# borgwang/tinynn-autograd

Measured on AMD Instinct MI355X. Metric: training samples/sec, MNIST 3-layer MLP (784-256-128-10), bs=128, at 1/2/4/8 GPUs, higher is better.
Workload: dtype f32; 1 GPU; configs[1]: Dense/ReLU MLP 784-256-128-10, 128 rows per GPU (global batch 128), whole-batch softmax NLL, Adam lr=1e-3; parallelism=dp1, global_batch=128, rows_per_rank=128, data_resident_in_hbm=True

## Files before the change

tinynn-autograd_amd/csrc/tnn_gemm.hip:

```cpp
#include <math.h>
#include <stdlib.h>

#include <algorithm>

#include "tnn_internal.h"
#include "tnn_dispatch.h"
#include "tnn_tile_order.h"
#include "tnn_p2p.h"
#include "tnn_head_stats.h"

namespace {

#include "tnn_gemm_args.h"
#include "tnn_gemm_tiled.h"
#include "tnn_gemm_adam.h"
#include "tnn_gemm_small.h"
#include "tnn_gemm_mid.h"
#include "tnn_gemm_step.h"
#include "tnn_gemm_f64.h"

GemmArgs gemm_args(const void* A, int64_t lda, const void* B, int64_t ldb, void* C, int64_t ldc, int64_t M, int64_t N, int64_t K,
                   int epi, float alpha = 1.f, float beta = 0.f) {
    GemmArgs g = {};
    g.A = (const float*)A; g.B = (const float*)B; g.C = (float*)C;
    g.M = M; g.N = N; g.K = K; g.lda = lda; g.ldb = ldb; g.ldc = ldc;
    g.alpha = alpha; g.beta = beta; g.epi = epi;
    return g;
}
void set_bias_act(GemmArgs& g, const void* bias, int act, int relu_sign) {
    g.bias = (const float*)bias; g.act = act; g.relu_sign = relu_sign;
}
void set_mask(GemmArgs& g, const void* Y, int64_t ldy) {
    g.Y = (const float*)Y; g.ldy = ldy;
}

bool vec_ok(const void* p, int64_t ld, int64_t contiguous, int64_t bytes = 0) {
    return tnn::aligned16(p) && ld % 4 == 0 && contiguous % 4 == 0 && bytes < (int64_t(1) << 32);
}

template <typename F>
auto with_layout(int transA, int transB, F&& f) {
    return tnn::with_flag(!transA, [&](auto akc) { return tnn::with_flag(transB != 0, [&](auto bkc) { return f(akc, bkc); }); });
}

GemmArgs dense_fwd_args(int64_t M, int64_t N, int64_t K, const void* A, int64_t lda, const void* B, int64_t ldb, const void* bias,
                        int act, int relu_sign, void* C, int64_t ldc) {
    GemmArgs g = gemm_args(A, lda, B, ldb, C, ldc, M, N, K, EPI_BIAS_ACT);
    set_bias_act(g, bias, act, relu_sign);
    g.vecA = vec_ok(A, lda, K);
    g.vecB = vec_ok(B, ldb, N);
    return g;
}
void set_head(GemmArgs& g, const void* head_w, void* head_z, int64_t head_c) {
    g.head_w = (const float*)head_w; g.head_z = (float*)head_z; g.head_c = (int)head_c;
}

void small_geometry(GemmArgs& g) {
    g.tiles_m = (int)((g.M + 15) / 16);
    g.tiles_n = (int)((g.N + 15) / 16);
    g.splits = 1;
    g.ws = nullptr;
    g.ord = tnn::tile_order(g.tiles_m, g.tiles_n, 0, 0);
}

inline bool tn_extents_ok(const GemmArgs& g) {
    return g.K * g.lda * 4 < (int64_t(1) << 31) && g.K * g.ldb * 4 < (int64_t(1) << 31);
}

void pick_xcd_cut(GemmArgs& g) {
    int xg_m = 0, xg_n = 0, best = 0;
    for (int xm = 1; xm <= 8; xm *= 2) {
        const int xn = 8 / xm;
        if (g.tiles_m % xm || g.tiles_n % xn) continue;
        const int cost = g.tiles_m / xm + g.tiles_n / xn;
        if (!best || cost < best) { best = cost; xg_m = xm; xg_n = xn; }
    }
    g.ord = tnn::tile_order(g.tiles_m, g.tiles_n, xg_m, xg_n);
}

bool mid_ok(const GemmArgs& g, int transA, int transB) {
    const bool akc = !transA, bkc = transB != 0;
    if (akc && !vec_ok(g.A, g.lda, g.K)) return false;
    if (bkc && !vec_ok(g.B, g.ldb, g.K)) return false;
    const int64_t a_bytes = ((akc ? g.M : g.K) * g.lda) * 4, b_bytes = ((bkc ? g.N : g.K) * g.ldb) * 4;
    return a_bytes < (int64_t(1) << 31) && b_bytes < (int64_t(1) << 31);
}

bool small_fast_ok(const GemmArgs& g, int transA, int transB) {
    const int64_t lim = int64_t(1) << 31;
    if (((g.M - 1) * g.ldc + g.N) * 4 >= lim || (g.epi == EPI_MASK && ((g.M - 1) * g.ldy + g.N) * 4 >= lim)) return false;
    return (!transA || transB) && mid_ok(g, transA, transB);
}

void fill_small_fast(GemmArgs& g, bool akc, bool bkc) {
    SmallFast& f = g.f;
    f.A = g.A; f.B = g.B;
    f.a_bytes = (uint32_t)(((akc ? g.M : g.K) - 1) * g.lda + (akc ? g.K : g.M)) * 4u;
    f.b_bytes = (uint32_t)(((bkc ? g.N : g.K) - 1) * g.ldb + (bkc ? g.K : g.N)) * 4u;
    f.lda4 = (uint32_t)g.lda * 4u; f.ldb4 = (uint32_t)g.ldb * 4u;
    f.M = (uint32_t)g.M; f.N = (uint32_t)g.N; f.K = (uint32_t)g.K;
    f.nchunks = (int)((g.K + 15) / 16);
    f.e_ptr = nullptr; f.e_bytes = 0u; f.e_ld4 = 0u;
    if (g.epi == EPI_BIAS_ACT) {
        f.e_ptr = g.bias; f.e_bytes = (uint32_t)g.N * 4u;
    } else if (g.epi == EPI_MASK) {
        f.e_ptr = g.Y; f.e_bytes = (uint32_t)((g.M - 1) * g.ldy + g.N) * 4u; f.e_ld4 = (uint32_t)g.ldy * 4u;
    } else if (g.beta != 0.f) {
        f.e_ptr = g.C; f.e_bytes = (uint32_t)((g.M - 1) * g.ldc + g.N) * 4u; f.e_ld4 = (uint32_t)g.ldc * 4u;
    }
    if (f.e_ptr == nullptr) f.e_bytes = 0u;
    const bool head = g.head_z != nullptr && g.head_w != nullptr;
    f.head_w = head ? g.head_w : nullptr;
    f.h_bytes = head ? (uint32_t)g.N * (uint32_t)g.head_c * 4u : 0u;
    f.hc4 = (uint32_t)g.head_c * 4u;
}

template <int WAVES>
int launch_small(GemmArgs& g, int transA, int transB, float* colsum) {
    small_geometry(g);
    dim3 grid((unsigned)(g.tiles_m * g.tiles_n));
    hipStream_t s = tnn::stream();
    const bool fast = small_fast_ok(g, transA, transB);
    pick_xcd_cut(g);
    if (fast) fill_small_fast(g, !transA, transB != 0);
    with_layout(transA, transB, [&](auto akc, auto bkc) {
        tnn::with_flag(fast, [&](auto f) {
            hipLaunchKernelGGL((gemm_small_f32_kernel<decltype(akc)::value, decltype(bkc)::value, WAVES, decltype(f)::value>), grid,
                               WAVES * 64, 0, s, g, colsum);
        });
    });
    TNN_LAUNCH_OK();
    return 0;
}

bool use_small_path(const GemmArgs& g) {
    int64_t tiles = ((g.M + 15) / 16) * ((g.N + 15) / 16);
    if (const char* e = getenv("TNN_GEMM_SMALL")) return atoi(e) != 0 && tiles <= tnn::kTileOrderMaxTiles;
    if (getenv("TNN_GEMM_CFG")) return false;
    double flop = 2.0 * (double)g.M * (double)g.N * (double)g.K;
    return flop <= 4.2e8 && tiles <= 8192;
}

int gemm_small(GemmArgs& g, int transA, int transB, float* colsum) {
    int nchunks = (int)((g.K + 15) / 16);
    if (nchunks <= 16) return launch_small<4>(g, transA, transB, colsum);
    if (nchunks <= 48) return launch_small<8>(g, transA, transB, colsum);
    return launch_small<16>(g, transA, transB, colsum);
}

bool use_mid_path(const GemmArgs& g, int transA, int transB) {
    const double flop = 2.0 * (double)g.M * (double)g.N * (double)g.K;
    const int64_t tiles = ((g.M + 31) / 32) * ((g.N + 31) / 32);
    return flop >= 1.5e8 && tiles >= 192 && mid_ok(g, transA, transB);
}

void mid_geometry(GemmArgs& g) {
    g.tiles_m = (int)((g.M + 31) / 32);
    g.tiles_n = (int)((g.N + 31) / 32);
    g.splits = 1;
    g.ws = nullptr;
    pick_xcd_cut(g);
}

int gemm_mid(GemmArgs& g, int transA, int transB, float* colsum) {
    mid_geometry(g);
    const int tiles = g.tiles_m * g.tiles_n;
    hipStream_t s = tnn::stream();
    AdamEpi none = {};
    with_layout(transA, transB, [&](auto akc, auto bkc) {
        hipLaunchKernelGGL((gemm_mid_f32_kernel<decltype(akc)::value, decltype(bkc)::value, false>), tiles, 512, 0, s, g, colsum,
                           none, tiles);
    });
    TNN_LAUNCH_OK();
    return 0;
}

template <int BM, int BN, int BK, int WM, int WN>
int launch_cfg(GemmArgs& g, int transA, int transB, int splits) {
    g.tiles_m = (int)((g.M + BM - 1) / BM);
    g.tiles_n = (int)((g.N + BN - 1) / BN);
    int64_t ktiles = (g.K + BK - 1) / BK;
    if (splits > ktiles) splits = (int)ktiles;
    if (splits < 1) splits = 1;
    int64_t tiles_per_split = (ktiles + splits - 1) / splits;
    if (tiles_per_split < 1) tiles_per_split = 1;
    splits = ktiles > 0 ? (int)((ktiles + tiles_per_split - 1) / tiles_per_split) : 1;
    g.k_per_split = tiles_per_split * BK;
    g.splits = splits;
    g.ws = nullptr;
    g.group_m = 8;
    if (const char* e = getenv("TNN_GEMM_GROUP_M")) g.group_m = atoi(e) > 0 ? atoi(e) : 8;
#ifdef TNN_GEMM_TRACE
    g.trace = nullptr;
    if (const char* e = getenv("TNN_GEMM_TRACE_PTR"))
        if (splits == 1) g.trace = reinterpret_cast<unsigned long long*>(strtoull(e, nullptr, 0));
#endif
    void* ws = nullptr;
    if (splits > 1) {
        if (tnn_malloc((size_t)splits * g.M * g.N * sizeof(float), &ws)) return 1;
        g.ws = (float*)ws;
    }
    dim3 grid((unsigned)(g.tiles_m * g.tiles_n), 1, (unsigned)splits);
    constexpr int NT = WM * WN * 64;
    hipStream_t s = tnn::stream();
    with_layout(transA, transB, [&](auto akc, auto bkc) {
        tnn::with_flag(g.vecA && g.vecB, [&](auto vec) {
            hipLaunchKernelGGL((gemm_f32_mfma_kernel<BM, BN, BK, WM, WN, decltype(akc)::value, decltype(bkc)::value, decltype(vec)::value>),
                               grid, NT, 0, s, g);
        });
    });
    if (splits > 1) {
        hipLaunchKernelGGL(splitk_reduce_kernel, tnn::stream_grid(g.M * g.N, 256), 256, 0, s, g);
        tnn_free(ws);
    }
    TNN_LAUNCH_OK();
    return 0;
}

int gemm_f32(GemmArgs& g, int transA, int transB, float* colsum = nullptr) {
    g.vecA = vec_ok(g.A, g.lda, transA ? g.M : g.K, (transA ? g.K : g.M) * g.lda * 4);
    g.vecB = vec_ok(g.B, g.ldb, transB ? g.K : g.N, (transB ? g.N : g.K) * g.ldb * 4);
    if (use_small_path(g)) return use_mid_path(g, transA, transB) ? gemm_mid(g, transA, transB, colsum)
                                                                    : gemm_small(g, transA, transB, colsum);
    if (colsum != nullptr) {
        if (int rc = tnn_reduce(TNN_RSUM, g.B, colsum, 1, g.K, g.N, TNN_F32)) return rc;
    }

    const int cus = tnn::num_cus();
    g.staged_c = 1;
    int cfg = -1, splits = 0;
    if (const char* e = getenv("TNN_GEMM_CFG")) cfg = atoi(e);
    if (const char* e = getenv("TNN_GEMM_SPLITK")) splits = atoi(e);
    int64_t t128x64 = ((g.M + 127) / 128) * ((g.N + 63) / 64);
    int64_t t64 = ((g.M + 63) / 64) * ((g.N + 63) / 64);
    if (cfg < 0) cfg = (t128x64 >= cus / 2) ? 3 : 2;
    const int64_t t64x128 = ((g.M + 63) / 64) * ((g.N + 127) / 128);
    if (cfg == 3 && !getenv("TNN_GEMM_CFG") && !transA && g.M <= 1024 && t64x128 >= cus / 2 && t64x128 <= 2 * cus) cfg = 1;
    if (splits <= 0) {
        splits = 1;
        int64_t tiles = cfg == 3 ? t128x64 : cfg == 2 ? t64 : cfg == 0 ? ((g.M + 127) / 128) * ((g.N + 127) / 128)
                                                              : ((g.M + 63) / 64) * ((g.N + 127) / 128);
        if (tiles < cus) {
            splits = (int)((cus + tiles - 1) / tiles);
            int64_t max_splits = g.K / 256;
            if (splits > max_splits) splits = (int)max_splits;
            if (splits < 1) splits = 1;
            if (splits > 16) splits = 16;
        }
    }
    switch (cfg) {
        case 0: return launch_cfg<128, 128, 32, 2, 2>(g, transA, transB, splits);
        case 1: return launch_cfg<64, 128, 32, 2, 2>(g, transA, transB, splits);
        case 2: return launch_cfg<64, 64, 32, 2, 2>(g, transA, transB, splits);
        case 3: return launch_cfg<128, 64, 32, 2, 2>(g, transA, transB, splits);
    }
    tnn::set_error("tnn_gemm: unknown tile configuration %d", cfg);
    return 2;
}

int gemm_f64(int transA, int transB, int64_t M, int64_t N, int64_t K, const void* A, int64_t lda,
             const void* B, int64_t ldb, void* C, int64_t ldc, double alpha, double beta, int epi,
             const void* bias, int act, int relu_sign, const void* Y, int64_t ldy) {
    GemmArgsD g;
    g.relu_sign = relu_sign;
    g.A = (const double*)A; g.B = (const double*)B; g.C = (double*)C;
    g.M = M; g.N = N; g.K = K;
    g.sam = transA ? 1 : lda; g.sak = transA ? lda : 1;
    g.sbk = transB ? 1 : ldb; g.sbn = transB ? ldb : 1;
    g.ldc = ldc; g.alpha = alpha; g.beta = beta; g.epi = epi;
    g.bias = (const double*)bias; g.act = act; g.Y = (const double*)Y; g.ldy = ldy;
    dim3 grid((unsigned)((N + 63) / 64), (unsigned)std::min<int64_t>((M + 63) / 64, 65535));
    hipLaunchKernelGGL(gemm_f64_kernel, grid, 256, 0, tnn::stream(), g);
    TNN_LAUNCH_OK();
    return 0;
}

int check_shapes(const char* fn, int transA, int transB, int64_t M, int64_t N, int64_t K,
                 int64_t lda, int64_t ldb, int64_t ldc) {
    TNN_REQUIRE(M >= 0 && N >= 0 && K >= 0, "%s: negative extent", fn);
    TNN_REQUIRE(lda >= (transA ? M : K), "%s: lda %lld too small", fn, (long long)lda);
    TNN_REQUIRE(ldb >= (transB ? K : N), "%s: ldb %lld too small", fn, (long long)ldb);
    TNN_REQUIRE(ldc >= N, "%s: ldc %lld too small", fn, (long long)ldc);
    TNN_REQUIRE(M < (1LL << 31) && N < (1LL << 31), "%s: extent exceeds 2^31", fn);
    return 0;
}

int rowpanel_args(const char* fn, bool merged, int64_t M, int64_t N, int64_t K, const void* A, int64_t lda, const void* B, int64_t ldb,
                  const void* bias, int act, int relu_sign, void* C, int64_t ldc, const void* head_w, int64_t head_c,
                  void* head_z_full, const void* head_b, void* pairs_f32, const void* ticket, const void* out_pair, int dtype,
                  RowPanelArgs& g) {
    TNN_NEED_INIT();
    if (int rc = check_shapes(fn, 0, 0, M, N, K, lda, ldb, ldc)) return rc;
    TNN_REQUIRE(dtype == TNN_F32 && M >= 1 && M <= 1024 && N == 128 && head_c == 10 && K >= 1,
                "%s: f32, 1 <= rows <= 1024, 128 hidden units, 10 classes", fn);
    TNN_REQUIRE(A && B && C && head_w && head_z_full && head_b && pairs_f32 && (!merged || (ticket && out_pair)),
                "%s: A, B, C, head_w, head_z_full, head_b%s are required", fn, merged ? ", pairs, ticket and out_pair" : " and pairs");
    TNN_REQUIRE(act == TNN_ACT_RELU, "%s: the hidden layer in front of the head is a ReLU layer (activation %d)", fn, act);
    TNN_REQUIRE(vec_ok(A, lda, K) && (M - 1) * lda + K < (int64_t)1 << 30 && (K - 1) * ldb + 128 < (int64_t)1 << 30,
                "%s: A must be 16-B aligned with lda and K multiples of 4, operands below 4 GiB", fn);
    g.A = (const float*)A; g.B = (const float*)B; g.bias = (const float*)bias; g.C = (float*)C;
    g.lda = lda; g.ldb = ldb; g.ldc = ldc;
    g.M = (int)M; g.K = (int)K; g.relu_sign = relu_sign;
    g.head_w = (const float*)head_w; g.head_b = (const float*)head_b;
    g.zfull = (float*)head_z_full; g.pairs = (float*)pairs_f32; g.bump = nullptr;
    return 0;
}
int launch_rowpanel_plain(const RowPanelArgs& g) {
    hipLaunchKernelGGL(dense_fwd_rowpanel_head_kernel<false>, dim3((unsigned)((g.M + 15) / 16)), 512, 0, tnn::stream(), g, HeadTail{},
                       tnn::p2p::LaunchCtx{});
    TNN_LAUNCH_OK();
    return 0;
}

}

extern "C" {

int tnn_gemm(int transA, int transB, int64_t M, int64_t N, int64_t K, double alpha, const void* A,
             int64_t lda, const void* B, int64_t ldb, double beta, void* C, int64_t ldc, int dtype) {
    TNN_NEED_INIT();
    if (int rc = check_shapes("tnn_gemm", transA, transB, M, N, K, lda, ldb, ldc)) return rc;
    if (M == 0 || N == 0) return 0;
    if (dtype == TNN_F64)
        return gemm_f64(transA, transB, M, N, K, A, lda, B, ldb, C, ldc, alpha, beta, EPI_AXPBY,
                        nullptr, 0, 0, nullptr, 0);
    TNN_REQUIRE(dtype == TNN_F32, "tnn_gemm: dtype %d is not a float type", dtype);
    GemmArgs g = gemm_args(A, lda, B, ldb, C, ldc, M, N, K, EPI_AXPBY, (float)alpha, (float)beta);
    return gemm_f32(g, transA, transB);
}

int tnn_gemm_tn_colsum(int64_t M, int64_t N, int64_t K, const void* A, int64_t lda, const void* G,
                       int64_t ldg, void* dW, int64_t ldc, void* db, int dtype) {
    TNN_NEED_INIT();
    if (int rc = check_shapes("tnn_gemm_tn_colsum", 1, 0, M, N, K, lda, ldg, ldc)) return rc;
    TNN_REQUIRE(ldg == N || db == nullptr, "tnn_gemm_tn_colsum: the column sum needs a dense G (ldg == N)");
    if (N == 0) return 0;
    if (dtype == TNN_F64) {
        if (M > 0)
            if (int rc = gemm_f64(1, 0, M, N, K, A, lda, G, ldg, dW, ldc, 1.0, 0.0, EPI_AXPBY, nullptr, 0, 0,
                                  nullptr, 0))
                return rc;
        return db ? tnn_reduce(TNN_RSUM, G, db, 1, K, N, TNN_F64) : 0;
    }
    TNN_REQUIRE(dtype == TNN_F32, "tnn_gemm_tn_colsum: dtype %d is not a float type", dtype);
    if (M == 0) return db ? tnn_reduce(TNN_RSUM, G, db, 1, K, N, TNN_F32) : 0;
    GemmArgs g = gemm_args(A, lda, G, ldg, dW, ldc, M, N, K, EPI_AXPBY);
    return gemm_f32(g, 1, 0, (float*)db);
}

int tnn_gemm_tn_adam(int64_t M, int64_t N, int64_t K, const void* A, int64_t lda, const void* G, int64_t ldg, void* g_out,
                     void* p, void* m, void* v, double lr, double b1, double b2, double eps, const void* pows_f64,
                     int dtype) {
    return tnn_gemm_tn_adam_bias(M, N, K, A, lda, G, ldg, g_out, p, m, v, nullptr, nullptr, nullptr, nullptr, lr, b1, b2, eps,
                                 pows_f64, dtype);
}

int tnn_gemm_tn_adam_bias(int64_t M, int64_t N, int64_t K, const void* A, int64_t lda, const void* G, int64_t ldg, void* g_out,
                          void* p, void* m, void* v, void* db, void* pb, void* mb, void* vb, double lr, double b1, double b2,
                          double eps, const void* pows_f64, int dtype) {
    TNN_NEED_INIT();
    if (int rc = check_shapes("tnn_gemm_tn_adam", 1, 0, M, N, K, lda, ldg, N)) return rc;
    TNN_REQUIRE((pb == nullptr) == (mb == nullptr) && (pb == nullptr) == (vb == nullptr) && (pb == nullptr || db != nullptr),
                "tnn_gemm_tn_adam_bias: pb / mb / vb go together and need db");
    TNN_REQUIRE(db == nullptr || ldg == N, "tnn_gemm_tn_adam_bias: the column sum needs a dense G (ldg == N)");
    TNN_REQUIRE(p && m && v && pows_f64, "tnn_gemm_tn_adam: p, m, v and pows are required");
    TNN_REQUIRE(dtype == TNN_F32 || dtype == TNN_F64, "tnn_gemm_tn_adam: dtype %d is not a float type", dtype);
    if (M == 0 || N == 0) return 0;
    using tnn::aligned16;
    GemmArgs g = gemm_args(A, lda, G, ldg, g_out, N, M, N, K, EPI_ADAM);
    const bool tiled = dtype == TNN_F32 && !use_small_path(g) && N % 4 == 0 && aligned16(p) && aligned16(m) && aligned16(v) && aligned16(g_out) &&
                       ((M + 127) / 128) * ((N + 63) / 64) >= tnn::num_cus() / 2 && getenv("TNN_GEMM_CFG") == nullptr &&
                       getenv("TNN_GEMM_SPLITK") == nullptr;
    if (tiled) {
        g.ad_p = (float*)p; g.ad_m = (float*)m; g.ad_v = (float*)v;
        g.ad_lr = (float)lr; g.ad_b1 = (float)b1; g.ad_b2 = (float)b2; g.ad_eps = (float)eps;
        g.ad_pows = (const double*)pows_f64;
        g.ad_guard = tnn::update_guard();
        const bool cs = db != nullptr;
        if (cs) { g.cs_db = (float*)db; g.cs_p = (float*)pb; g.cs_m = (float*)mb; g.cs_v = (float*)vb; }
        if (int rc = gemm_f32(g, 1, 0)) return rc;
        if (db != nullptr && !cs) {
            if (int rc = tnn_reduce(TNN_RSUM, G, db, 1, K, N, dtype)) return rc;
            if (pb) return tnn_adam_ex(pb, db, mb, vb, N, lr, b1, b2, eps, const_cast<void*>(pows_f64), nullptr, dtype, 0, nullptr, nullptr);
        }
        return 0;
    }
    void* scratch = nullptr;
    void* gw = g_out;
    const size_t esz = dtype == TNN_F64 ? 8 : 4;
    if (gw == nullptr) {
        if (tnn_malloc((size_t)(M * N) * esz, &scratch)) return 1;
        gw = scratch;
    }
    int rc = tnn_gemm_tn_colsum(M, N, K, A, lda, G, ldg, gw, N, db, dtype);
    if (!rc) rc = tnn_adam_ex(p, gw, m, v, M * N, lr, b1, b2, eps, const_cast<void*>(pows_f64), nullptr, dtype, 0, nullptr, nullptr);
    if (!rc && pb) rc = tnn_adam_ex(pb, db, mb, vb, N, lr, b1, b2, eps, const_cast<void*>(pows_f64), nullptr, dtype, 0, nullptr, nullptr);
    if (scratch) tnn_free(scratch);
    return rc;
}

int tnn_dense_bwd(int64_t rows, int64_t n_in, int64_t n_out, const void* x, const void* dz, const void* w,
                  void* dw, void* db, void* dx, const void* mask_src, int dtype) {
    TNN_NEED_INIT();
    TNN_REQUIRE(rows > 0 && n_in > 0 && n_out > 0, "tnn_dense_bwd: empty layer");
    TNN_REQUIRE(dx == nullptr || mask_src != nullptr, "tnn_dense_bwd: dx needs mask_src");
    if (dtype == TNN_F32 && dx != nullptr) {
        GemmArgs gw = gemm_args(x, n_in, dz, n_out, dw, n_out, n_in, n_out, rows, EPI_AXPBY);
        gw.vecA = vec_ok(x, n_in, n_in); gw.vecB = vec_ok(dz, n_out, n_out);
        GemmArgs gx = gemm_args(dz, n_out, w, n_out, dx, n_in, rows, n_in, n_out, EPI_MASK);
        set_mask(gx, mask_src, n_in);
        gx.vecA = vec_ok(dz, n_out, n_out); gx.vecB = vec_ok(w, n_out, n_out);
        if (use_small_path(gw) && use_small_path(gx)) {
            small_geometry(gw);
            small_geometry(gx);
            int n_dw = gw.tiles_m * gw.tiles_n, n_dx = gx.tiles_m * gx.tiles_n;
            if (n_dw % 8 == 0) {
                pick_xcd_cut(gw);
                pick_xcd_cut(gx);
            }
            int nchunks = (int)((std::max(gw.K, gx.K) + 15) / 16);
            hipStream_t s = tnn::stream();
            const bool fast = small_fast_ok(gw, 1, 0) && small_fast_ok(gx, 0, 1);
            if (fast) { fill_small_fast(gw, false, false); fill_small_fast(gx, true, true); }
#define TNN_BWD_SMALL(W)                                                                                             \
    do {                                                                                                             \
        if (fast) hipLaunchKernelGGL((dense_bwd_small_kernel<W, true>), n_dw + n_dx, W * 64, 0, s, gw, (float*)db, gx, n_dw); \
        else hipLaunchKernelGGL((dense_bwd_small_kernel<W, false>), n_dw + n_dx, W * 64, 0, s, gw, (float*)db, gx, n_dw);    \
    } while (0)
            if (nchunks <= 16)
                TNN_BWD_SMALL(4);
            else if (nchunks <= 48)
                TNN_BWD_SMALL(8);
            else
                TNN_BWD_SMALL(16);
#undef TNN_BWD_SMALL
            TNN_LAUNCH_OK();
            return 0;
        }
    }
    if (int rc = tnn_gemm_tn_colsum(n_in, n_out, rows, x, n_in, dz, n_out, dw, n_out, db, dtype)) return rc;
    if (dx != nullptr)
        return tnn_gemm_mask(0, 1, rows, n_in, n_out, dz, n_out, w, n_out, mask_src, n_in, dx, n_in, dtype);
    return 0;
}

static bool dw0_wide_ok(const GemmArgs& g) {
    static const bool off = getenv("TNN_DW0_WIDE") && atoi(getenv("TNN_DW0_WIDE")) == 0;
    return !off && g.N % 32 == 0 && ((g.M + 15) / 16) * (g.N / 32) >= 256 && g.epi == EPI_AXPBY && g.beta == 0.f;
}

int tnn_dense_bwd_first_adam(int64_t rows, int64_t n_in, int64_t n_out, const void* x, const void* dz, void* dw, void* db,
                             void* p_w, void* m_w, void* v_w, void* p_b, void* m_b, void* v_b, void* flat_p,
                             const void* flat_g, void* flat_m, void* flat_v, int64_t flat_n, double lr, double b1,
                             double b2, double eps, const void* pows_f64, int dtype) {
    TNN_NEED_INIT();
    TNN_REQUIRE(rows > 0 && n_in > 0 && n_out > 0, "tnn_dense_bwd_first_adam: empty layer");
    TNN_REQUIRE(pows_f64 && p_w && m_w && v_w && p_b && m_b && v_b, "tnn_dense_bwd_first_adam: optimizer state is required");
    if (dtype == TNN_F32) {
        GemmArgs gw = gemm_args(x, n_in, dz, n_out, dw, n_out, n_in, n_out, rows, EPI_AXPBY);
        if (use_small_path(gw) && tn_extents_ok(gw)) {
            const bool mid = use_mid_path(gw, 1, 0);
            if (mid) mid_geometry(gw);
            else { small_geometry(gw); pick_xcd_cut(gw); }
            const int n_dw = gw.tiles_m * gw.tiles_n;
            AdamEpi ad;
            ad.pw = (float*)p_w; ad.mw = (float*)m_w; ad.vw = (float*)v_w;
            ad.pb = (float*)p_b; ad.mb = (float*)m_b; ad.vb = (float*)v_b;
            ad.fp = (float*)flat_p; ad.fg = (const float*)flat_g; ad.fm = (float*)flat_m; ad.fv = (float*)flat_v;
            ad.fn = flat_n > 0 ? flat_n : 0;
            ad.lr = (float)lr; ad.b1 = (float)b1; ad.b2 = (float)b2; ad.eps = (float)eps;
            ad.pows = (const double*)pows_f64;
            const int nchunks = (int)((gw.K + 15) / 16);
            hipStream_t s = tnn::stream();
            if (mid) {
                const int extra = adam_flat_blocks(ad.fp, ad.fg, ad.fm, ad.fv, ad.fn, 512);
                hipLaunchKernelGGL((gemm_mid_f32_kernel<false, false, true>), n_dw + extra, 512, 0, s, gw, (float*)db, ad, n_dw);
                TNN_LAUNCH_OK();
                return 0;
            }
#define TNN_BWD0(W)                                                                                         \
    do {                                                                                                    \
        const int extra = adam_flat_blocks(ad.fp, ad.fg, ad.fm, ad.fv, ad.fn, W * 64);                      \
        hipLaunchKernelGGL((dense_bwd0_adam_kernel<W>), n_dw + extra, W * 64, 0, s, gw, (float*)db, ad, n_dw); \
    } while (0)
            if (nchunks <= 16 && dw0_wide_ok(gw)) {
                gw.tiles_n = (int)(gw.N / 32);
                pick_xcd_cut(gw);
                const int n_wide = gw.tiles_m * gw.tiles_n;
                const int extra = adam_flat_blocks(ad.fp, ad.fg, ad.fm, ad.fv, ad.fn, 256);
                hipLaunchKernelGGL((dense_bwd0_adam_kernel<4, true>), n_wide + extra, 256, 0, s, gw, (float*)db, ad, n_wide);
                TNN_LAUNCH_OK();
                return 0;
            }
            const int waves = nchunks <= 16 ? 4 : nchunks <= 48 ? 8 : 16;
            if (waves == 4) TNN_BWD0(4);
            else if (waves == 8) TNN_BWD0(8);
            else TNN_BWD0(16);
#undef TNN_BWD0
            TNN_LAUNCH_OK();
            return 0;
        }
    }
    void* pows = const_cast<void*>(pows_f64);
    if (int rc = tnn_gemm_tn_adam_bias(n_in, n_out, rows, x, n_in, dz, n_out, dw, p_w, m_w, v_w, db, p_b, m_b, v_b, lr, b1, b2, eps,
                                       pows, dtype))
        return rc;
    if (flat_n > 0)
        return tnn_adam_ex(flat_p, flat_g, flat_m, flat_v, flat_n, lr, b1, b2, eps, pows, nullptr, dtype, 0, nullptr, nullptr);
    return 0;
}

#ifdef TNN_STEP_TRACE
extern "C" __attribute__((visibility("default"))) int tnn_debug_step_trace(unsigned long long* out, int n) {
    TNN_CHECK_HIP(hipDeviceSynchronize());
    TNN_CHECK_HIP(hipMemcpyFromSymbol(out, HIP_SYMBOL(g_step_trace), (size_t)std::min(n, 4 * 1024 * 4) * 8));
    return 0;
}
extern "C" __attribute__((visibility("default"))) int tnn_debug_step_trace_first(unsigned long long* out, int n) {
    TNN_CHECK_HIP(hipDeviceSynchronize());
    TNN_CHECK_HIP(hipMemcpyFromSymbol(out, HIP_SYMBOL(g_step_trace_first), (size_t)std::min(n, 4 * 1024) * 8));
    return 0;
}
#endif
#ifdef TNN_AR_TRACE
__attribute__((visibility("default"))) int tnn_debug_fh_trace(unsigned long long* out, int n) {
    TNN_CHECK_HIP(hipDeviceSynchronize());
    TNN_CHECK_HIP(hipMemcpyFromSymbol(out, HIP_SYMBOL(g_fh_trace), (size_t)std::min(n, 1024) * 8));
    return 0;
}
__attribute__((visibility("default"))) int tnn_debug_ar_trace(unsigned long long* out, int n) {
    TNN_CHECK_HIP(hipDeviceSynchronize());
    TNN_CHECK_HIP(hipMemcpyFromSymbol(out, HIP_SYMBOL(g_ar_trace), (size_t)std::min(n, 4096) * 8));
    return 0;
}
#endif

int tnn_dense_bwd_first_allreduce_adam(int64_t rows, int64_t n_in, int64_t n_out, const void* x, const void* dz, void* grads,
                                       int64_t n_reduce, int64_t w_off, int64_t b_off, void* p, void* m, void* v,
                                       int64_t n_params, double lr, double b1, double b2, double eps, const void* pows_f64,
                                       int64_t scalar_index, void* scalar_dst, int dtype) {
    TNN_NEED_INIT();
    TNN_REQUIRE(rows > 0 && n_in > 0 && n_out > 0, "tnn_dense_bwd_first_allreduce_adam: empty layer");
    TNN_REQUIRE(grads && p && m && v && pows_f64, "tnn_dense_bwd_first_allreduce_adam: NULL argument");
    TNN_REQUIRE(n_params > 0 && n_reduce >= n_params && w_off >= 0 && b_off >= 0 && w_off + n_in * n_out <= n_params &&
                    b_off + n_out <= n_params,
                "tnn_dense_bwd_first_allreduce_adam: the layer's blocks do not lie inside the arena");
    TNN_REQUIRE(!scalar_dst || (scalar_index >= 0 && scalar_index < n_reduce), "tnn_dense_bwd_first_allreduce_adam: scalar_index");
    const size_t esz = dtype == TNN_F64 ? 8 : 4;
    if (dtype == TNN_F32) {
        GemmArgs gw = gemm_args(x, n_in, dz, n_out, nullptr, n_out, n_in, n_out, rows, EPI_AXPBY);
        using tnn::aligned16;
        const bool mid = use_mid_path(gw, 1, 0);
        tnn::p2p::LaunchCtx ctx;
        if (aligned16(grads) && aligned16(p) && aligned16(m) && aligned16(v) && use_small_path(gw) &&
            (mid || (tn_extents_ok(gw) && rows <= 256)) && n_out % 4 == 0 && w_off % 4 == 0 && b_off % 4 == 0 &&
            (!scalar_dst || scalar_index >= n_params) && tnn::p2p_can_allreduce(n_reduce, dtype, TNN_RSUM) && tnn::p2p_launch_ctx(&ctx)) {
            if (int rc = tnn::p2p_refuse_if_failed("tnn_dense_bwd_first_allreduce_adam")) return rc;
            if (mid) mid_geometry(gw);
            else { small_geometry(gw); pick_xcd_cut(gw); }
            const int W = ctx.peers.world;
            ArTileArgs f;
            f.buf = (float*)grads; f.n = n_reduce;
            f.slice = ((n_reduce + W - 1) / W + 3) / 4 * 4;
            f.w_off = w_off; f.b_off = b_off;
            f.n_dw = gw.tiles_m * gw.tiles_n;
            tnn::p2p::AdamTail t;
            t.p = (float*)p; t.m = (float*)m; t.v = (float*)v; t.n_params = n_params;
            t.lr = (float)lr; t.b1 = (float)b1; t.b2 = (float)b2; t.eps = (float)eps;
            t.pows = (const double*)pows_f64;
            t.scalar_index = scalar_dst ? scalar_index : -1;
            t.scalar_dst = (float*)scalar_dst;
            if (mid) {
                hipLaunchKernelGGL(dense_bwd0_mid_allreduce_adam_kernel, f.n_dw + ctx.ar_grid, 512, 0, tnn::stream(), gw, f, ctx, t);
            } else if (dw0_wide_ok(gw)) {
                gw.tiles_n = (int)(gw.N / 32);
                pick_xcd_cut(gw);
                f.n_dw = gw.tiles_m * gw.tiles_n;
                hipLaunchKernelGGL((dense_bwd0_allreduce_adam_kernel<4, true>), f.n_dw + ctx.ar_grid, 256, 0, tnn::stream(), gw, f, ctx, t);
            } else {
                hipLaunchKernelGGL((dense_bwd0_allreduce_adam_kernel<4>), f.n_dw + ctx.ar_grid, 256, 0, tnn::stream(), gw, f, ctx, t);
            }
            TNN_LAUNCH_OK();
            return 0;
        }
    }
    if (int rc = tnn_dense_bwd(rows, n_in, n_out, x, dz, nullptr, (char*)grads + (size_t)w_off * esz,
                               (char*)grads + (size_t)b_off * esz, nullptr, nullptr, dtype))
        return rc;
    return tnn_allreduce_adam(grads, n_reduce, p, m, v, n_params, lr, b1, b2, eps, const_cast<void*>(pows_f64), 0, dtype,
                              scalar_index, scalar_dst);
}

int tnn_gemm_bias_act(int transA, int transB, int64_t M, int64_t N, int64_t K, const void* A,
                      int64_t lda, const void* B, int64_t ldb, const void* bias, int act,
                      int relu_sign, void* C, int64_t ldc, int dtype) {
    TNN_NEED_INIT();
    if (int rc = check_shapes("tnn_gemm_bias_act", transA, transB, M, N, K, lda, ldb, ldc)) return rc;
    TNN_REQUIRE(act == TNN_ACT_NONE || act == TNN_ACT_RELU, "tnn_gemm_bias_act: activation %d", act);
    if (M == 0 || N == 0) return 0;
    if (dtype == TNN_F64)
        return gemm_f64(transA, transB, M, N, K, A, lda, B, ldb, C, ldc, 1.0, 0.0, EPI_BIAS_ACT, bias,
                        act, relu_sign, nullptr, 0);
    TNN_REQUIRE(dtype == TNN_F32, "tnn_gemm_bias_act: dtype %d is not a float type", dtype);
    GemmArgs g = gemm_args(A, lda, B, ldb, C, ldc, M, N, K, EPI_BIAS_ACT);
    set_bias_act(g, bias, act, relu_sign);
    return gemm_f32(g, transA, transB);
}

int tnn_dense_fwd_head_partials(int64_t M, int64_t N, int64_t K, const void* A, int64_t lda, const void* B,
                                           int64_t ldb, const void* bias, int act, int relu_sign, void* C, int64_t ldc,
                                           const void* head_w, int64_t head_c, void* head_z, int dtype) {
    TNN_NEED_INIT();
    if (int rc = check_shapes("tnn_dense_fwd_head_partials", 0, 0, M, N, K, lda, ldb, ldc)) return rc;
    TNN_REQUIRE(dtype == TNN_F32, "tnn_dense_fwd_head_partials: f32 only (dtype %d)", dtype);
    TNN_REQUIRE(head_w && head_z && head_c >= 1 && head_c <= 16, "tnn_dense_fwd_head_partials: head_w, head_z and 1 <= head_c <= 16");
    TNN_REQUIRE(act == TNN_ACT_NONE || act == TNN_ACT_RELU, "tnn_dense_fwd_head_partials: activation %d", act);
    if (M == 0 || N == 0) return 0;
    GemmArgs g = dense_fwd_args(M, N, K, A, lda, B, ldb, bias, act, relu_sign, C, ldc);
    if (use_small_path(g) && small_fast_ok(g, 0, 0)) {
        set_head(g, head_w, head_z, head_c);
        return gemm_small(g, 0, 0, nullptr);
    }
    if (int rc = gemm_f32(g, 0, 0)) return rc;
    const int64_t total = ((N + 15) / 16) * M * head_c;
    hipLaunchKernelGGL(head_partials_kernel, tnn::stream_grid(total, 256), 256, 0, tnn::stream(), (const float*)C, M, N, ldc,
                       (const float*)head_w, (int)head_c, (float*)head_z);
    TNN_LAUNCH_OK();
    return 0;
}

int tnn_dense_fwd_head_partials_stats(int64_t M, int64_t N, int64_t K, const void* A, int64_t lda, const void* B, int64_t ldb,
                                      const void* bias, int act, int relu_sign, void* C, int64_t ldc, const void* head_w,
                                      int64_t head_c, void* head_z, const void* head_b, const void* y, void* ticket_u32,
                                      void* out_pair_f32, int exchange, int dtype) {
    TNN_NEED_INIT();
    if (int rc = check_shapes("tnn_dense_fwd_head_partials_stats", 0, 0, M, N, K, lda, ldb, ldc)) return rc;
    TNN_REQUIRE(dtype == TNN_F32 && M >= 1 && M <= 1024 && N >= 16 && N <= 256 && N % 16 == 0 && head_c >= 1 && head_c <= 16,
                "tnn_dense_fwd_head_partials_stats: f32, rows <= 1024, hidden width a multiple of 16 up to 256, <= 16 classes");
    TNN_REQUIRE(head_w && head_z && head_b && y && ticket_u32 && out_pair_f32,
                "tnn_dense_fwd_head_partials_stats: head_w, head_z, head_b, y, ticket and out_pair are required");
    TNN_REQUIRE(act == TNN_ACT_NONE || act == TNN_ACT_RELU, "tnn_dense_fwd_head_partials_stats: activation %d", act);
    GemmArgs g = dense_fwd_args(M, N, K, A, lda, B, ldb, bias, act, relu_sign, C, ldc);
    TNN_REQUIRE(small_fast_ok(g, 0, 0), "tnn_dense_fwd_head_partials_stats: operands must be 16-B aligned with K %% 4 == 0");
    set_head(g, head_w, head_z, head_c);
    small_geometry(g);
    pick_xcd_cut(g);
    fill_small_fast(g, true, false);
    tnn::p2p::LaunchCtx ctx = {};
    if (exchange == 2) {
        TNN_REQUIRE(M <= 128, "tnn_dense_fwd_head_partials_stats: exchange = 2 is the <= 128-row form (rows %lld)", (long long)M);
        if (int rc = tnn::p2p_refuse_if_failed("tnn_dense_fwd_head_partials_stats")) return rc;
        TNN_REQUIRE(tnn::p2p_launch_ctx(&ctx), "tnn_dense_fwd_head_partials_stats: the peer-to-peer transport is not enabled");
        g.bump = ctx.xchg_seq;
        return gemm_small(g, 0, 0, nullptr);
    }
    HeadTail ta;
    ta.ticket = (unsigned int*)ticket_u32;
    ta.zpart = (const float*)head_z; ta.bias = (const float*)head_b; ta.y = (const float*)y;
    ta.out_pair = (float*)out_pair_f32; ta.m = (int)M; ta.exchange = exchange ? 1 : 0;
    if (exchange) {
        if (int rc = tnn::p2p_refuse_if_failed("tnn_dense_fwd_head_partials_stats")) return rc;
        TNN_REQUIRE(tnn::p2p_launch_ctx(&ctx), "tnn_dense_fwd_head_partials_stats: the peer-to-peer transport is not enabled");
    }
    if (N == 128 && head_c == 10)
        hipLaunchKernelGGL(dense_fwd_head_kernel<8>, dim3((unsigned)(g.tiles_m * g.tiles_n)), 512, 0, tnn::stream(), g, ta, ctx);
    else
        hipLaunchKernelGGL(dense_fwd_head_generic_kernel<8>, dim3((unsigned)(g.tiles_m * g.tiles_n)), 512, 0, tnn::stream(), g, ta, ctx);
    TNN_LAUNCH_OK();
    return 0;
}

int tnn_dense_fwd_rows_head_stats(int64_t M, int64_t N, int64_t K, const void* A, int64_t lda, const void* B, int64_t ldb,
                                  const void* bias, int act, int relu_sign, void* C, int64_t ldc, const void* head_w,
                                  int64_t head_c, void* head_z_full, const void* head_b, void* pairs_f32, int dtype) {
    RowPanelArgs g;
    if (int rc = rowpanel_args("tnn_dense_fwd_rows_head_stats", false, M, N, K, A, lda, B, ldb, bias, act, relu_sign, C, ldc, head_w, head_c,
                               head_z_full, head_b, pairs_f32, nullptr, nullptr, dtype, g))
        return rc;
    return launch_rowpanel_plain(g);
}

int tnn_dense_fwd_rows_head_stats_merged(int64_t M, int64_t N, int64_t K, const void* A, int64_t lda, const void* B, int64_t ldb,
                                         const void* bias, int act, int relu_sign, void* C, int64_t ldc, const void* head_w,
                                         int64_t head_c, void* head_z_full, const void* head_b, void* pairs_f32, void* ticket_u32,
                                         void* out_pair_f32, int exchange, int dtype) {
    RowPanelArgs g;
    if (int rc = rowpanel_args("tnn_dense_fwd_rows_head_stats_merged", true, M, N, K, A, lda, B, ldb, bias, act, relu_sign, C, ldc, head_w,
                               head_c, head_z_full, head_b, pairs_f32, ticket_u32, out_pair_f32, dtype, g))
        return rc;
    HeadTail ta = {};
    ta.ticket = (unsigned int*)ticket_u32;
    ta.out_pair = (float*)out_pair_f32; ta.m = (int)M; ta.exchange = exchange ? 1 : 0;
    tnn::p2p::LaunchCtx ctx = {};
    if (exchange) {
        if (int rc = tnn::p2p_refuse_if_failed("tnn_dense_fwd_rows_head_stats_merged")) return rc;
        TNN_REQUIRE(tnn::p2p_launch_ctx(&ctx), "tnn_dense_fwd_rows_head_stats_merged: the peer-to-peer transport is not enabled");
    }
    if (exchange == 2) {
        g.bump = ctx.xchg_seq;
        return launch_rowpanel_plain(g);
    }
    hipLaunchKernelGGL(dense_fwd_rowpanel_head_kernel<true>, dim3((unsigned)((M + 15) / 16)), 512, 0, tnn::stream(), g, ta, ctx);
    TNN_LAUNCH_OK();
    return 0;
}

int tnn_gemm_mask(int transA, int transB, int64_t M, int64_t N, int64_t K, const void* A, int64_t lda,
                  const void* B, int64_t ldb, const void* Y, int64_t ldy, void* C, int64_t ldc,
                  int dtype) {
    TNN_NEED_INIT();
    if (int rc = check_shapes("tnn_gemm_mask", transA, transB, M, N, K, lda, ldb, ldc)) return rc;
    TNN_REQUIRE(Y != nullptr && ldy >= N, "tnn_gemm_mask: bad mask operand");
    if (M == 0 || N == 0) return 0;
    if (dtype == TNN_F64)
        return gemm_f64(transA, transB, M, N, K, A, lda, B, ldb, C, ldc, 1.0, 0.0, EPI_MASK, nullptr, 0,
                        0, Y, ldy);
    TNN_REQUIRE(dtype == TNN_F32, "tnn_gemm_mask: dtype %d is not a float type", dtype);
    GemmArgs g = gemm_args(A, lda, B, ldb, C, ldc, M, N, K, EPI_MASK);
    set_mask(g, Y, ldy);
    return gemm_f32(g, transA, transB);
}

}
```

tinynn-autograd_amd/csrc/tnn_gemm_args.h:

```cpp
#pragma once

typedef float f32x16 __attribute__((ext_vector_type(16)));
typedef float f32x4 __attribute__((ext_vector_type(4)));

enum { EPI_AXPBY = 0, EPI_BIAS_ACT = 1, EPI_MASK = 2, EPI_ADAM = 3 };

struct SmallFast {
    uint32_t a_bytes, b_bytes;
    uint32_t lda4, ldb4;
    uint32_t M, N, K;
    int nchunks;
    uint32_t e_bytes, e_ld4;
    uint32_t h_bytes, hc4;
    const float *A, *B, *e_ptr, *head_w;
};

struct GemmArgs {
    const float* A;
    const float* B;
    float* C;
    int64_t M, N, K, lda, ldb, ldc;
    float alpha, beta;
    int epi;
    const float* bias;
    int act, relu_sign;
    const float* Y;
    int64_t ldy;
    int vecA, vecB;
    int64_t k_per_split;
    int splits;
    float* ws;
    int tiles_m, tiles_n;
    tnn::TileOrder ord;
    SmallFast f;
    const float* head_w;
    float* head_z;
    int head_c;
    unsigned int* bump;
    float *ad_p, *ad_m, *ad_v;
    float ad_lr, ad_b1, ad_b2, ad_eps;
    const double* ad_pows;
    const int* ad_guard;
    int staged_c;
    int group_m;
    float *cs_db, *cs_p, *cs_m, *cs_v;
#ifdef TNN_GEMM_TRACE
    unsigned long long* trace;
#endif
};

__device__ __forceinline__ float apply_epilogue(const GemmArgs& g, float acc, int64_t row,
                                                int64_t col) {
    if (g.epi == EPI_AXPBY) {
        float r = g.alpha * acc;
        if (g.beta != 0.f) r += g.beta * g.C[row * g.ldc + col];
        return r;
    } else if (g.epi == EPI_BIAS_ACT) {
        float v = acc + (g.bias ? g.bias[col] : 0.f);
        if (g.act == TNN_ACT_RELU) {
            if (g.relu_sign) v = v < 0.f ? -0.0f : fabsf(v);
            else v = v < 0.f ? 0.f : v;
        }
        return v;
    } else {
        float y = g.Y[row * g.ldy + col];
        return (__float_as_uint(y) >> 31) ? 0.f : acc;
    }
}

__device__ __forceinline__ int xcd_remap(int b, int nb) {
    const int nx = 8;
    if (nb < 2 * nx) return b;
    int q = nb / nx, r = nb % nx;
    int xcd = b % nx, local = b / nx;
    int base = xcd < r ? xcd * (q + 1) : r * (q + 1) + (xcd - r) * q;
    return base + local;
}

__device__ __forceinline__ float finish_epilogue(const GemmArgs& g, float acc, float pre) {
    if (g.epi == EPI_AXPBY) {
        float r = g.alpha * acc;
        if (g.beta != 0.f) r += g.beta * pre;
        return r;
    } else if (g.epi == EPI_BIAS_ACT) {
        float v = acc + pre;
        if (g.act == TNN_ACT_RELU) {
            if (g.relu_sign) v = v < 0.f ? -0.0f : fabsf(v);
            else v = v < 0.f ? 0.f : v;
        }
        return v;
    } else {
        return (__float_as_uint(pre) >> 31) ? 0.f : acc;
    }
}

__device__ __forceinline__ void small_tile_coords(const GemmArgs& g, const int block, int& tm, int& tn) {
    tnn::tile_coords(g.ord, block, tm, tn);
}

#ifdef TNN_STEP_TRACE
__device__ unsigned long long g_step_trace[4 * 1024 * 4];
__device__ unsigned long long g_step_trace_first[4 * 1024];
#endif
```

tinynn-autograd_amd/csrc/tnn_gemm_small.h:

```cpp
#pragma once


struct TnFrag {
    __amdgpu_buffer_rsrc_t rsrc;
    uint32_t K, ld4, lane, k0;
    bool ok;
    __device__ __forceinline__ TnFrag(const float* p, int64_t K_, int64_t ld, int64_t extent, int grp, int64_t col, bool ok_)
        : rsrc(__builtin_amdgcn_make_buffer_rsrc(const_cast<float*>(p), 0, (uint32_t)((K_ - 1) * ld + extent) * 4u, 0x00020000)),
          K((uint32_t)K_), ld4((uint32_t)ld * 4u), lane((uint32_t)grp * 4u * (uint32_t)ld * 4u + (uint32_t)col * 4u),
          k0((uint32_t)grp * 4u), ok(ok_) {}
    __device__ __forceinline__ float load(const uint32_t row, const uint32_t byte_off) const {
        uint32_t off = (ok & (row + k0 < K)) ? lane + row * ld4 + byte_off : 0xffffffffu;
        asm("" : "+v"(off));
        return __uint_as_float(__builtin_amdgcn_raw_buffer_load_b32(rsrc, off, 0, 0));
    }
};

template <int V> struct IntC { static constexpr int value = V; };
constexpr int TN_MAXC = 4;
__device__ __forceinline__ void tn_pin(float (&b)[4]) { asm volatile("" : "+v"(b[0]), "+v"(b[1]), "+v"(b[2]), "+v"(b[3])); }
template <int LIVE, int WAVES, class L, class K, class M>
__device__ __forceinline__ void tn_batch_body(const int c0, L&& load, K&& mma_mark, M&& mma) {
#pragma unroll
    for (int u = 0; u < LIVE; ++u) {
        load(u, c0 + u * WAVES);
        __builtin_amdgcn_sched_barrier(0);
    }
#pragma unroll
    for (int u = 0; u < LIVE; ++u) {
        mma_mark(u, LIVE);
        mma(u);
        __builtin_amdgcn_sched_barrier(0);
    }
}
template <int WAVES, bool SINGLE, class L, class K, class M>
__device__ __forceinline__ void tn_batches(const int wid, const int nchunks, L&& load, K&& mma_mark, M&& mma) {
    for (int c0 = wid; c0 < nchunks; c0 += WAVES * TN_MAXC) {
        const int live = (nchunks - c0 + WAVES - 1) / WAVES;
        auto mark = [&](const int u, const int n) { if (c0 == wid) mma_mark(u, n); };
        switch (live < TN_MAXC ? live : TN_MAXC) {
            case 1: tn_batch_body<1, WAVES>(c0, load, mark, mma); break;
            case 2: tn_batch_body<2, WAVES>(c0, load, mark, mma); break;
            case 3: tn_batch_body<3, WAVES>(c0, load, mark, mma); break;
            default: tn_batch_body<4, WAVES>(c0, load, mark, mma); break;
        }
        if constexpr (SINGLE) break;
    }
}

template <bool AKC, bool BKC, int WAVES, bool ADAM = false, bool TO_LDS = false>
__device__ __forceinline__ void small_tile(const GemmArgs& g, float* __restrict__ colsum, int block,
                                           float (*red)[4][64], float (*bsum)[64], const AdamEpi* ad = nullptr,
                                           float* out_lds = nullptr) {
    if constexpr (ADAM) TNN_STEP_STAMP(g_step_trace, 3, 0);
    const int tid = threadIdx.x, lane = tid & 63, wid = tid >> 6;
    const int i16 = lane & 15, grp = lane >> 4;
    int tm, tn;
    small_tile_coords(g, block, tm, tn);
    const int64_t m0 = (int64_t)tm * 16, n0 = (int64_t)tn * 16;
    const int64_t am = m0 + i16, bn = n0 + i16;
    const bool a_ok = am < g.M, b_ok = bn < g.N;
    const int nchunks = (int)((g.K + 15) / 16);
    f32x4 acc = {0.f, 0.f, 0.f, 0.f};
    float bs = 0.f;
    [[maybe_unused]] unsigned long long t_first = 0, t_last = 0;
    float a_p = 0.f, a_m = 0.f, a_v = 0.f, ab_p = 0.f, ab_m = 0.f, ab_v = 0.f, ic1 = 0.f, ic2 = 0.f;
    if constexpr (ADAM) {
        ic1 = (float)(1.0 / (1.0 - ad->pows[0]));
        ic2 = (float)(1.0 / (1.0 - ad->pows[1]));
        if (tid < 256) {
            const int64_t row = m0 + ((tid & 63) >> 4) * 4 + (tid >> 6), col = n0 + (tid & 15);
            if (row < g.M && col < g.N) {
                const int64_t i = row * g.ldc + col;
                a_p = ad->pw[i]; a_m = ad->mw[i]; a_v = ad->vw[i];
            }
        }
        if (tm == 0 && tid < 16 && n0 + tid < g.N) {
            ab_p = ad->pb[n0 + tid]; ab_m = ad->mb[n0 + tid]; ab_v = ad->vb[n0 + tid];
        }
    }
    if constexpr (ADAM) {
        static_assert(!AKC && !BKC, "the Adam epilogue belongs to dW = X^T dZ");
        const TnFrag fa(g.A, g.K, g.lda, g.M, grp, am, a_ok), fb(g.B, g.K, g.ldb, g.N, grp, bn, b_ok);
        const int swid = __builtin_amdgcn_readfirstlane(wid);
        float a[TN_MAXC][4], b[TN_MAXC][4];
        tn_batches<WAVES, false>(
            swid, nchunks,
            [&](const int u, const int c) {
#pragma unroll
                for (int j = 0; j < 4; ++j) {
                    a[u][j] = fa.load((uint32_t)c * 16u + (uint32_t)j, 0u);
                    b[u][j] = fb.load((uint32_t)c * 16u + (uint32_t)j, 0u);
                }
            },
            [&](const int u, const int n) {
                if (u == 0) TNN_STEP_CLOCK_HOME(t_first, a[0][3], b[0][3]);
                if (u == n - 1) TNN_STEP_CLOCK_HOME(t_last, a[u][3], b[u][3]);
            },
            [&](const int u) {
#pragma unroll
                for (int j = 0; j < 4; ++j) acc = __builtin_amdgcn_mfma_f32_16x16x4f32(a[u][j], b[u][j], acc, 0, 0, 0);
                tn_pin(b[u]);
                bs += (b[u][0] + b[u][1]) + (b[u][2] + b[u][3]);
            });
    } else {
        for (int c = wid; c < nchunks; c += WAVES) {
            const int64_t k = (int64_t)c * 16 + grp * 4;
            float a[4] = {0.f, 0.f, 0.f, 0.f}, b[4] = {0.f, 0.f, 0.f, 0.f};
            if constexpr (AKC) {
                const float* p = g.A + am * g.lda + k;
                if (a_ok) {
                    if (g.vecA && k + 3 < g.K) {
                        float4 v = *reinterpret_cast<const float4*>(p);
                        a[0] = v.x; a[1] = v.y; a[2] = v.z; a[3] = v.w;
                    } else {
#pragma unroll
                        for (int j = 0; j < 4; ++j) if (k + j < g.K) a[j] = p[j];
                    }
                }
            } else {
                if (a_ok) {
#pragma unroll
                    for (int j = 0; j < 4; ++j) if (k + j < g.K) a[j] = g.A[(k + j) * g.lda + am];
                }
            }
            if constexpr (BKC) {
                const float* p = g.B + bn * g.ldb + k;
                if (b_ok) {
                    if (g.vecB && k + 3 < g.K) {
                        float4 v = *reinterpret_cast<const float4*>(p);
                        b[0] = v.x; b[1] = v.y; b[2] = v.z; b[3] = v.w;
                    } else {
#pragma unroll
                        for (int j = 0; j < 4; ++j) if (k + j < g.K) b[j] = p[j];
                    }
                }
            } else {
                if (b_ok) {
#pragma unroll
                    for (int j = 0; j < 4; ++j) if (k + j < g.K) b[j] = g.B[(k + j) * g.ldb + bn];
                }
            }
#pragma unroll
            for (int j = 0; j < 4; ++j) acc = __builtin_amdgcn_mfma_f32_16x16x4f32(a[j], b[j], acc, 0, 0, 0);
            bs += (b[0] + b[1]) + (b[2] + b[3]);
        }
    }
#pragma unroll
    for (int r = 0; r < 4; ++r) red[wid][r][lane] = acc[r];
    bsum[wid][lane] = bs;
    __syncthreads();
    if constexpr (ADAM) TNN_STEP_STAMP(g_step_trace, 3, 2);
    if constexpr (ADAM) {
        TNN_STEP_STAMP_VALUE(g_step_trace_first, 3, 1, 0, t_first);
        TNN_STEP_STAMP_VALUE(g_step_trace, 3, 4, 1, t_last);
    }
    if (tid < 256) {
        const int r = tid >> 6, ln = tid & 63;
        float s = 0.f;
#pragma unroll
        for (int w = 0; w < WAVES; ++w) s += red[w][r][ln];
        const int64_t row = m0 + (ln >> 4) * 4 + r, col = n0 + (ln & 15);
        if (row < g.M && col < g.N) {
            const float gval = apply_epilogue(g, s, row, col);
            if constexpr (TO_LDS) out_lds[((ln >> 4) * 4 + r) * 16 + (ln & 15)] = gval;
            else if (!ADAM || g.C != nullptr) g.C[row * g.ldc + col] = gval;
            if constexpr (ADAM) {
                const int64_t i = row * g.ldc + col;
                ad->pw[i] = adam_apply(*ad, ic1, ic2, gval, a_m, a_v, a_p);
                ad->mw[i] = a_m;
                ad->vw[i] = a_v;
            }
        }
    }
    if ((TO_LDS || colsum != nullptr) && tm == 0 && tid < 16 && n0 + tid < g.N) {
        float s = 0.f;
#pragma unroll
        for (int w = 0; w < WAVES; ++w) s += (bsum[w][tid] + bsum[w][16 + tid]) + (bsum[w][32 + tid] + bsum[w][48 + tid]);
        if constexpr (TO_LDS) out_lds[256 + tid] = s;
        else colsum[n0 + tid] = s;
        if constexpr (ADAM) {
            ad->pb[n0 + tid] = adam_apply(*ad, ic1, ic2, s, ab_m, ab_v, ab_p);
            ad->mb[n0 + tid] = ab_m;
            ad->vb[n0 + tid] = ab_v;
        }
    }
    if constexpr (ADAM) TNN_STEP_STAMP_ACKED(g_step_trace, 3, 3);
}

template <int WAVES, bool ADAM, bool TO_LDS>
__device__ __forceinline__ void dw_tile_wide(const GemmArgs& g, float* __restrict__ colsum, const int block, float (*red)[8][64],
                                             float (*bsum)[2][64], const AdamEpi* ad = nullptr, float* out_lds = nullptr) {
    if constexpr (ADAM) TNN_STEP_STAMP(g_step_trace, 3, 0);
    const int tid = threadIdx.x, lane = tid & 63, wid = tid >> 6;
    const int i16 = lane & 15, grp = lane >> 4;
    int tm, tn;
    small_tile_coords(g, block, tm, tn);
    const int64_t m0 = (int64_t)tm * 16, n0 = (int64_t)tn * 32;
    const int64_t am = m0 + i16, bn = n0 + i16;
    const bool a_ok = am < g.M;
    const int nchunks = (int)((g.K + 15) / 16);
    const int e_r = tid >> 6, e_ln = tid & 63;
    const int64_t e_row = m0 + (e_ln >> 4) * 4 + e_r, e_col = n0 + (e_ln & 15);
    const bool e_live = tid < 256 && e_row < g.M;
    float a_p[2] = {0.f, 0.f}, a_m[2] = {0.f, 0.f}, a_v[2] = {0.f, 0.f}, ab_p = 0.f, ab_m = 0.f, ab_v = 0.f, ic1 = 0.f, ic2 = 0.f;
    if constexpr (ADAM) {
        ic1 = (float)(1.0 / (1.0 - ad->pows[0]));
        ic2 = (float)(1.0 / (1.0 - ad->pows[1]));
        if (e_live) {
#pragma unroll
            for (int u = 0; u < 2; ++u) {
                const int64_t i = e_row * g.ldc + e_col + 16 * u;
                a_p[u] = ad->pw[i]; a_m[u] = ad->mw[i]; a_v[u] = ad->vw[i];
            }
        }
        if (tm == 0 && tid < 32) { ab_p = ad->pb[n0 + tid]; ab_m = ad->mb[n0 + tid]; ab_v = ad->vb[n0 + tid]; }
    }
    f32x4 acc0 = {0.f, 0.f, 0.f, 0.f}, acc1 = {0.f, 0.f, 0.f, 0.f};
    float bs0 = 0.f, bs1 = 0.f;
    const TnFrag fa(g.A, g.K, g.lda, g.M, grp, am, a_ok), fb(g.B, g.K, g.ldb, g.N, grp, bn, true);
    const int swid = __builtin_amdgcn_readfirstlane(wid);
    float a[TN_MAXC][4], b0[TN_MAXC][4], b1[TN_MAXC][4];
    [[maybe_unused]] unsigned long long t_first = 0, t_last = 0;
    tn_batches<WAVES, true>(
        swid, nchunks,
        [&](const int u, const int c) {
#pragma unroll
            for (int j = 0; j < 4; ++j) {
                const uint32_t row = (uint32_t)c * 16u + (uint32_t)j;
                a[u][j] = fa.load(row, 0u);
                b0[u][j] = fb.load(row, 0u);
                b1[u][j] = fb.load(row, 64u);
            }
        },
        [&](const int u, const int n) {
            if constexpr (ADAM) {
                if (u == 0) TNN_STEP_CLOCK_HOME(t_first, a[0][3], b1[0][3]);
                if (u == n - 1) TNN_STEP_CLOCK_HOME(t_last, a[u][3], b1[u][3]);
            }
        },
        [&](const int u) {
#pragma unroll
            for (int j = 0; j < 4; ++j) {
                acc0 = __builtin_amdgcn_mfma_f32_16x16x4f32(a[u][j], b0[u][j], acc0, 0, 0, 0);
                acc1 = __builtin_amdgcn_mfma_f32_16x16x4f32(a[u][j], b1[u][j], acc1, 0, 0, 0);
            }
            tn_pin(b0[u]);
            tn_pin(b1[u]);
            bs0 += (b0[u][0] + b0[u][1]) + (b0[u][2] + b0[u][3]);
            bs1 += (b1[u][0] + b1[u][1]) + (b1[u][2] + b1[u][3]);
        });
#pragma unroll
    for (int r = 0; r < 4; ++r) { red[wid][r][lane] = acc0[r]; red[wid][4 + r][lane] = acc1[r]; }
    bsum[wid][0][lane] = bs0;
    bsum[wid][1][lane] = bs1;
    __syncthreads();
    if constexpr (ADAM) TNN_STEP_STAMP(g_step_trace, 3, 2);
    if constexpr (ADAM) {
        TNN_STEP_STAMP_VALUE(g_step_trace_first, 3, 1, 0, t_first);
        TNN_STEP_STAMP_VALUE(g_step_trace, 3, 4, 1, t_last);
    }
    if (e_live) {
#pragma unroll
        for (int u = 0; u < 2; ++u) {
            float sres = 0.f;
#pragma unroll
            for (int w = 0; w < WAVES; ++w) sres += red[w][4 * u + e_r][e_ln];
            const float gval = g.alpha * sres;
            const int64_t i = e_row * g.ldc + e_col + 16 * u;
            if constexpr (TO_LDS) out_lds[(int)(e_row - m0) * 32 + (int)(e_col - n0) + 16 * u] = gval;
            else if (!ADAM || g.C != nullptr) g.C[i] = gval;
            if constexpr (ADAM) {
                ad->pw[i] = adam_apply(*ad, ic1, ic2, gval, a_m[u], a_v[u], a_p[u]);
                ad->mw[i] = a_m[u];
                ad->vw[i] = a_v[u];
            }
        }
    }
    if ((TO_LDS || colsum != nullptr) && tm == 0 && tid < 32) {
        const int u = tid >> 4, t = tid & 15;
        float sres = 0.f;
#pragma unroll
        for (int w = 0; w < WAVES; ++w) sres += (bsum[w][u][t] + bsum[w][u][16 + t]) + (bsum[w][u][32 + t] + bsum[w][u][48 + t]);
        if constexpr (TO_LDS) out_lds[512 + tid] = sres;
        else colsum[n0 + tid] = sres;
        if constexpr (ADAM) {
            ad->pb[n0 + tid] = adam_apply(*ad, ic1, ic2, sres, ab_m, ab_v, ab_p);
            ad->mb[n0 + tid] = ab_m;
            ad->vb[n0 + tid] = ab_v;
        }
    }
    if constexpr (ADAM) TNN_STEP_STAMP_ACKED(g_step_trace, 3, 3);
}

template <bool AKC, bool BKC, int WAVES, bool SYS_HEADZ = false, bool HEAD = true>
__device__ __forceinline__ void small_tile_fast(const GemmArgs& g, float* __restrict__ colsum, int block,
                                                float (*red)[4][64], float (*bsum)[64], float* head_lds = nullptr) {
    typedef unsigned int u32x4_t __attribute__((ext_vector_type(4)));
    constexpr uint32_t OOB = 0xffffffffu;
    constexpr int KID = WAVES == 16 ? 0 : 1;
    TNN_STEP_STAMP(g_step_trace, KID, 0);
    const int tid = threadIdx.x, lane = tid & 63, wid = tid >> 6;
    const int i16 = lane & 15, grp = lane >> 4;
    const SmallFast& f = g.f;
    int tm, tn;
    small_tile_coords(g, block, tm, tn);
    const uint32_t m0 = (uint32_t)tm * 16u, n0 = (uint32_t)tn * 16u;
    const uint32_t am = m0 + (uint32_t)i16, bn = n0 + (uint32_t)i16;
    const bool a_ok = am < f.M, b_ok = bn < f.N;
    const int nchunks = f.nchunks;
    const uint32_t K = f.K, lda4 = f.lda4, ldb4 = f.ldb4;
    const __amdgpu_buffer_rsrc_t a_rsrc = __builtin_amdgcn_make_buffer_rsrc(const_cast<float*>(f.A), 0, f.a_bytes, 0x00020000);
    const __amdgpu_buffer_rsrc_t b_rsrc = __builtin_amdgcn_make_buffer_rsrc(const_cast<float*>(f.B), 0, f.b_bytes, 0x00020000);
    const uint32_t a_lane = AKC ? am * lda4 + (uint32_t)grp * 16u : (uint32_t)grp * 4u * lda4 + am * 4u;
    const uint32_t b_lane = BKC ? bn * ldb4 + (uint32_t)grp * 16u : (uint32_t)grp * 4u * ldb4 + bn * 4u;
    const uint32_t a_chunk = AKC ? 64u : 16u * lda4;
    const uint32_t b_chunk = BKC ? 64u : 16u * ldb4;

    const int e_r = tid >> 6, e_ln = tid & 63;
    const uint32_t e_row = m0 + (uint32_t)((e_ln >> 4) * 4 + e_r), e_col = n0 + (uint32_t)(e_ln & 15);
    const bool e_live = tid < 256 && e_row < f.M && e_col < f.N;
    const uint32_t e_off = e_row * f.e_ld4 + e_col * 4u;
    const __amdgpu_buffer_rsrc_t e_rsrc = __builtin_amdgcn_make_buffer_rsrc(const_cast<float*>(f.e_ptr), 0, f.e_bytes, 0x00020000);
    const bool head_on = f.h_bytes != 0u;
    const __amdgpu_buffer_rsrc_t h_rsrc = __builtin_amdgcn_make_buffer_rsrc(const_cast<float*>(f.head_w), 0, f.h_bytes, 0x00020000);
    const int swid = __builtin_amdgcn_readfirstlane(wid);
    float e_pre = 0.f;
    float head_pre[4] = {0.f, 0.f, 0.f, 0.f};
    auto request_epilogue = [&](auto role_c) {
        constexpr int ROLE = decltype(role_c)::value;
        if constexpr (ROLE >= 1) {
            uint32_t off = e_live ? e_off : OOB;
            asm("" : "+v"(off));
            e_pre = __uint_as_float(__builtin_amdgcn_raw_buffer_load_b32(e_rsrc, off, 0, 0));
        }
        if constexpr (ROLE == 2) {
            const uint32_t unit0 = n0 + 4u * (uint32_t)grp, hc4 = f.hc4;
            uint32_t unit_b = unit0 * hc4;
            asm("" : "+v"(unit_b));
            const uint32_t off0 = unit_b + (uint32_t)i16 * 4u;
            const bool cls_ok = (uint32_t)i16 * 4u < hc4;
#pragma unroll
            for (int j = 0; j < 4; ++j) {
                const bool ok = cls_ok & (unit0 + (uint32_t)j < f.N);
                uint32_t off = ok ? off0 + (uint32_t)j * hc4 : OOB;
                asm("" : "+v"(off));
                head_pre[j] = __uint_as_float(__builtin_amdgcn_raw_buffer_load_b32(h_rsrc, off, 0, 0));
            }
        }
    };

    f32x4 acc = {0.f, 0.f, 0.f, 0.f};
    float bs = 0.f;
    [[maybe_unused]] unsigned long long t_first = 0, t_last = 0;
    constexpr int MAXC = 4;
    auto load_chunk = [&](float (&a)[4], float (&b)[4], const uint32_t c) {
        const uint32_t k = c * 16u + (uint32_t)grp * 4u;
        if constexpr (AKC) {
            uint32_t off = (a_ok && k < K) ? a_lane + c * a_chunk : OOB;
            asm("" : "+v"(off));
            const u32x4_t v = __builtin_amdgcn_raw_buffer_load_b128(a_rsrc, off, 0, 0);
#pragma unroll
            for (int j = 0; j < 4; ++j) a[j] = __uint_as_float(v[j]);
        } else {
#pragma unroll
            for (int j = 0; j < 4; ++j) {
                uint32_t off = (a_ok && k + j < K) ? a_lane + c * a_chunk + (uint32_t)j * lda4 : OOB;
                asm("" : "+v"(off));
                a[j] = __uint_as_float(__builtin_amdgcn_raw_buffer_load_b32(a_rsrc, off, 0, 0));
            }
        }
        if constexpr (BKC) {
            uint32_t off = (b_ok && k < K) ? b_lane + c * b_chunk : OOB;
            asm("" : "+v"(off));
            const u32x4_t v = __builtin_amdgcn_raw_buffer_load_b128(b_rsrc, off, 0, 0);
#pragma unroll
            for (int j = 0; j < 4; ++j) b[j] = __uint_as_float(v[j]);
        } else {
#pragma unroll
            for (int j = 0; j < 4; ++j) {
                uint32_t off = (b_ok && k + j < K) ? b_lane + c * b_chunk + (uint32_t)j * ldb4 : OOB;
                asm("" : "+v"(off));
                b[j] = __uint_as_float(__builtin_amdgcn_raw_buffer_load_b32(b_rsrc, off, 0, 0));
            }
        }
    };
    auto mma_chunk = [&](const float (&a)[4], float (&b)[4]) {
#pragma unroll
        for (int j = 0; j < 4; ++j) acc = __builtin_amdgcn_mfma_f32_16x16x4f32(a[j], b[j], acc, 0, 0, 0);
        tn_pin(b);
        bs += (b[0] + b[1]) + (b[2] + b[3]);
    };
    auto first_batch = [&](auto live_c, auto role_c) {
        constexpr int LIVE = decltype(live_c)::value;
        float a[LIVE > 0 ? LIVE : 1][4], b[LIVE > 0 ? LIVE : 1][4];
#pragma unroll
        for (int u = 0; u < LIVE; ++u) {
            load_chunk(a[u], b[u], (uint32_t)(swid + u * WAVES));
            __builtin_amdgcn_sched_barrier(0);
        }
        request_epilogue(role_c);
        __builtin_amdgcn_sched_barrier(0);
#pragma unroll
        for (int u = 0; u < LIVE; ++u) {
            if (u == 0) TNN_STEP_CLOCK_HOME(t_first, a[0][3], b[0][3]);
            if (u == LIVE - 1) TNN_STEP_CLOCK_HOME(t_last, a[u][3], b[u][3]);
            mma_chunk(a[u], b[u]);
            __builtin_amdgcn_sched_barrier(0);
        }
    };
    auto by_live = [&](auto role_c) {
        const int live = swid < nchunks ? (nchunks - swid + WAVES - 1) / WAVES : 0;
        switch (live < MAXC ? live : MAXC) {
            case 0: first_batch(IntC<0>{}, role_c); break;
            case 1: first_batch(IntC<1>{}, role_c); break;
            case 2: first_batch(IntC<2>{}, role_c); break;
            case 3: first_batch(IntC<3>{}, role_c); break;
            default: first_batch(IntC<4>{}, role_c); break;
        }
    };
    if (HEAD && head_on && swid == 0) by_live(IntC<2>{});
    else if (WAVES <= 4 || swid < 4) by_live(IntC<1>{});
    else by_live(IntC<0>{});
    for (int c0 = swid + WAVES * MAXC; c0 < nchunks; c0 += WAVES * MAXC) {
        float a[MAXC][4], b[MAXC][4];
#pragma unroll
        for (int u = 0; u < MAXC; ++u) {
            const uint32_t c = (uint32_t)(c0 + u * WAVES);
            if ((int)c >= nchunks) {
#pragma unroll
                for (int j = 0; j < 4; ++j) { a[u][j] = 0.f; b[u][j] = 0.f; }
                continue;
            }
            load_chunk(a[u], b[u], c);
        }
#pragma unroll
        for (int u = 0; u < MAXC; ++u) mma_chunk(a[u], b[u]);
    }
#pragma unroll
    for (int r = 0; r < 4; ++r) red[wid][r][lane] = acc[r];
    bsum[wid][lane] = bs;
    __syncthreads();
    TNN_STEP_STAMP(g_step_trace, KID, 2);
    TNN_STEP_STAMP_VALUE(g_step_trace_first, KID, 1, 0, t_first);
    TNN_STEP_STAMP_VALUE(g_step_trace, KID, 4, 1, t_last);
    float e_val = 0.f;
    if (tid < 256) {
        float s = 0.f;
#pragma unroll
        for (int w = 0; w < WAVES; ++w) s += red[w][e_r][e_ln];
        if (e_live) {
            e_val = finish_epilogue(g, s, e_pre);
            g.C[(int64_t)e_row * g.ldc + e_col] = e_val;
        }
    }
    if (colsum != nullptr && tm == 0 && tid < 16 && n0 + (uint32_t)tid < f.N) {
        float s = 0.f;
#pragma unroll
        for (int w = 0; w < WAVES; ++w) s += (bsum[w][tid] + bsum[w][16 + tid]) + (bsum[w][32 + tid] + bsum[w][48 + tid]);
        colsum[n0 + tid] = s;
    }
    if (head_lds != nullptr && g.head_z != nullptr) {
        float* tile_s = head_lds;
        if (tid < 256) tile_s[((e_ln >> 4) * 4 + e_r) * 20 + (e_ln & 15)] = e_val;
        __syncthreads();
        if (wid == 0) {
            const f32x4 a4 = *reinterpret_cast<const f32x4*>(tile_s + i16 * 20 + 4 * grp);
            f32x4 hacc = {0.f, 0.f, 0.f, 0.f};
#pragma unroll
            for (int j = 0; j < 4; ++j) hacc = __builtin_amdgcn_mfma_f32_16x16x4f32(a4[j], head_pre[j], hacc, 0, 0, 0);
            if (i16 < g.head_c) {
#pragma unroll
                for (int q = 0; q < 4; ++q) {
                    const int64_t row = (int64_t)m0 + 4 * grp + q;
                    if (row < g.M) {
                        float* dst = g.head_z + ((int64_t)tn * g.M + row) * g.head_c + i16;
                        if constexpr (SYS_HEADZ) tnn::p2p::store_sys(reinterpret_cast<uint32_t*>(dst), __float_as_uint(hacc[q]));
                        else *dst = hacc[q];
                    }
                }
            }
        }
    }
    TNN_STEP_STAMP_ACKED(g_step_trace, KID, 3);
}

template <bool AKC, bool BKC, int WAVES, bool FAST>
__global__ __launch_bounds__(WAVES * 64) void gemm_small_f32_kernel(GemmArgs g, float* __restrict__ colsum) {
    __shared__ float red[WAVES][4][64];
    __shared__ float bsum[WAVES][64];
    if constexpr (FAST) {
        __shared__ __attribute__((aligned(16))) float head_lds[16 * 20];
        small_tile_fast<AKC, BKC, WAVES>(g, colsum, (int)blockIdx.x, red, bsum, head_lds);
        if (g.bump != nullptr && blockIdx.x == 0 && threadIdx.x == 0) *g.bump += 1u;
    } else {
        small_tile<AKC, BKC, WAVES>(g, colsum, (int)blockIdx.x, red, bsum);
    }
}
```

tinynn-autograd_amd/csrc/tnn_gemm_step.h:

```cpp
#pragma once

#ifdef TNN_AR_TRACE
__device__ unsigned long long g_fh_trace[128 * 8];
#endif
template <int WAVES>
__global__ __launch_bounds__(WAVES * 64) void dense_fwd_head_kernel(GemmArgs g, HeadTail ta, tnn::p2p::LaunchCtx ctx) {
    static_assert(WAVES == 8, "head_tail_stats is written for 512 threads");
    __shared__ float red[WAVES][4][64];
    __shared__ float bsum[WAVES][64];
    __shared__ __attribute__((aligned(16))) float head_lds[16 * 20];
    __shared__ __attribute__((aligned(16))) float zs[128 * 10], ys[128 * 10];
    __shared__ double dred[8][4];
    __shared__ int is_last;
    TNN_AR_STAMP(g_fh_trace, blockIdx.x, 8, 128, 0);
    small_tile_fast<true, false, WAVES, true>(g, nullptr, (int)blockIdx.x, red, bsum, head_lds);
    TNN_AR_STAMP(g_fh_trace, blockIdx.x, 8, 128, 1);
    using namespace tnn::p2p;
    int tm, tn;
    small_tile_coords(g, (int)blockIdx.x, tm, tn);
    const int nb = (ta.m + 127) / 128, rb = nb > 1 ? tm >> 3 : 0;
    const unsigned cnt = nb > 1 ? (unsigned)(min(8, g.tiles_m - 8 * rb) * g.tiles_n) : gridDim.x;
    unsigned int* const ctr = ta.ticket + (nb > 1 ? 1 + rb : 0);
    float* const pairs = reinterpret_cast<float*>(ta.ticket + 16);
    if (threadIdx.x < 64) {
        asm volatile("s_waitcnt vmcnt(0)" ::: "memory");
        TNN_AR_STAMP(g_fh_trace, blockIdx.x, 8, 128, 2);
        if (threadIdx.x == 0) {
            const unsigned prev = __hip_atomic_fetch_add(ctr, 1u, __ATOMIC_RELAXED, __HIP_MEMORY_SCOPE_AGENT);
            const int last = prev == cnt - 1 ? 1 : 0;
            if (last) __hip_atomic_store(ctr, 0u, __ATOMIC_RELAXED, __HIP_MEMORY_SCOPE_AGENT);
            is_last = last;
        }
    }
    __syncthreads();
#ifdef TNN_AR_TRACE
    if (threadIdx.x == 0 && blockIdx.x < 128) { g_fh_trace[blockIdx.x * 8 + 3] = wall_clock64(); g_fh_trace[blockIdx.x * 8 + 6] = is_last; }
#endif
    if (!is_last) return;
    float M, S;
    head_tail_stats<10, 8>(ta, 128 * rb, min(ta.m, 128 * rb + 128), zs, ys, dred, M, S);
    TNN_AR_STAMP(g_fh_trace, blockIdx.x, 8, 128, 4);
    if (nb > 1) {
        __syncthreads();
        if (threadIdx.x == 0) {
            __hip_atomic_store(pairs + 2 * rb, M, __ATOMIC_RELAXED, __HIP_MEMORY_SCOPE_SYSTEM);
            __hip_atomic_store(pairs + 2 * rb + 1, S, __ATOMIC_RELAXED, __HIP_MEMORY_SCOPE_SYSTEM);
            asm volatile("s_waitcnt vmcnt(0)" ::: "memory");
            const unsigned prev = __hip_atomic_fetch_add(ta.ticket, 1u, __ATOMIC_RELAXED, __HIP_MEMORY_SCOPE_AGENT);
            const int last = prev == (unsigned)nb - 1 ? 1 : 0;
            if (last) __hip_atomic_store(ta.ticket, 0u, __ATOMIC_RELAXED, __HIP_MEMORY_SCOPE_AGENT);
            is_last = last;
        }
        __syncthreads();
        if (!is_last) return;
        M = -INFINITY; S = 0.f;
        for (int q = 0; q < nb; ++q) {
            const float mq = __hip_atomic_load(pairs + 2 * q, __ATOMIC_RELAXED, __HIP_MEMORY_SCOPE_SYSTEM);
            const float sq = __hip_atomic_load(pairs + 2 * q + 1, __ATOMIC_RELAXED, __HIP_MEMORY_SCOPE_SYSTEM);
            const float nm = fmaxf(M, mq);
            S = S * expf(M - nm) + sq * expf(mq - nm);
            M = nm;
        }
    }
    head_tail_finish(ta, ctx, M, S);
    TNN_AR_STAMP(g_fh_trace, blockIdx.x, 8, 128, 5);
}

template <int WAVES>
__global__ __launch_bounds__(WAVES * 64) void dense_fwd_head_generic_kernel(GemmArgs g, HeadTail ta, tnn::p2p::LaunchCtx ctx) {
    static_assert(WAVES == 8, "512 threads");
    __shared__ float red[WAVES][4][64];
    __shared__ float bsum[WAVES][64];
    __shared__ __attribute__((aligned(16))) float head_lds[16 * 20];
    __shared__ float wred[WAVES][2];
    __shared__ int is_last;
    small_tile_fast<true, false, WAVES, true>(g, nullptr, (int)blockIdx.x, red, bsum, head_lds);
    using namespace tnn::p2p;
    if (threadIdx.x < 64) {
        asm volatile("s_waitcnt vmcnt(0)" ::: "memory");
        if (threadIdx.x == 0) {
            const unsigned prev = __hip_atomic_fetch_add(ta.ticket, 1u, __ATOMIC_RELAXED, __HIP_MEMORY_SCOPE_AGENT);
            const int last = prev == gridDim.x - 1 ? 1 : 0;
            if (last) __hip_atomic_store(ta.ticket, 0u, __ATOMIC_RELAXED, __HIP_MEMORY_SCOPE_AGENT);
            is_last = last;
        }
    }
    __syncthreads();
    if (!is_last) return;
    const int t = threadIdx.x, lane = t & 63, wid = t >> 6;
    const int C = g.head_c, NP = g.tiles_n, m = ta.m;
    float mx = -INFINITY, sx = 0.f;
    for (int r = t; r < m; r += WAVES * 64) {
        uint32_t u[16][1];
        float z[16];
#pragma unroll
        for (int k = 0; k < 16; ++k) z[k] = k < C ? ta.bias[k] : -INFINITY;
        for (int tn = 0; tn < NP; ++tn) {
            const uint32_t* src = reinterpret_cast<const uint32_t*>(ta.zpart) + ((size_t)tn * m + r) * C;
#pragma unroll
            for (int k = 0; k < 16; ++k) if (k < C) load_sys(u[k][0], src + k);
            asm volatile("s_waitcnt vmcnt(0)" ::: "memory");
#pragma unroll
            for (int k = 0; k < 16; ++k) {
                asm volatile("" : "+v"(u[k][0]));
                if (k < C) z[k] += __uint_as_float(u[k][0]);
            }
        }
        float rm = -INFINITY, rs = 0.f;
#pragma unroll
        for (int k = 0; k < 16; ++k) if (k < C) rm = fmaxf(rm, z[k]);
#pragma unroll
        for (int k = 0; k < 16; ++k) if (k < C) rs += expf(z[k] - rm);
        const float nm = fmaxf(mx, rm);
        sx = sx * expf(mx - nm) + rs * expf(rm - nm);
        mx = nm;
    }
    const float wm = tnn::wave_max_dpp(mx);
    const float ws = tnn::wave_sum_dpp(mx > -INFINITY ? sx * expf(mx - wm) : 0.f);
    if (lane == 0) { wred[wid][0] = wm; wred[wid][1] = ws; }
    __syncthreads();
    float M = -INFINITY, S = 0.f;
#pragma unroll
    for (int w = 0; w < WAVES; ++w) M = fmaxf(M, wred[w][0]);
#pragma unroll
    for (int w = 0; w < WAVES; ++w) S += wred[w][0] > -INFINITY ? wred[w][1] * expf(wred[w][0] - M) : 0.f;
    head_tail_finish(ta, ctx, M, S);
}

struct RowPanelArgs {
    const float *A, *B, *bias;
    float* C;
    int64_t lda, ldb, ldc;
    int M, K, relu_sign;
    const float *head_w, *head_b;
    float *zfull, *pairs;
    unsigned int* bump;
};

template <bool MERGE>
__global__ __launch_bounds__(512) void dense_fwd_rowpanel_head_kernel(RowPanelArgs g, HeadTail ta, tnn::p2p::LaunchCtx ctx) {
    typedef unsigned int u32x4_t __attribute__((ext_vector_type(4)));
    constexpr uint32_t OOB = 0xffffffffu;
    constexpr int C = 10;
    __shared__ __attribute__((aligned(16))) float tile_s[8][16 * 20];
    __shared__ float zred[8][16 * 16];
    __shared__ float wred[4][2];
    const int tid = threadIdx.x, lane = tid & 63, wid = tid >> 6;
    const int i16 = lane & 15, grp = lane >> 4;
    const int m0 = 16 * (int)blockIdx.x, n0 = 16 * wid;
    const uint32_t K = (uint32_t)g.K, lda4 = (uint32_t)g.lda * 4u, ldb4 = (uint32_t)g.ldb * 4u;
    const __amdgpu_buffer_rsrc_t a_rsrc = __builtin_amdgcn_make_buffer_rsrc(
        const_cast<float*>(g.A), 0, (uint32_t)(((int64_t)(g.M - 1) * g.lda + g.K) * 4), 0x00020000);
    const __amdgpu_buffer_rsrc_t b_rsrc = __builtin_amdgcn_make_buffer_rsrc(
        const_cast<float*>(g.B), 0, (uint32_t)(((int64_t)(g.K - 1) * g.ldb + 128) * 4), 0x00020000);
    const uint32_t b_lane = (uint32_t)grp * 4u * ldb4 + (uint32_t)(n0 + i16) * 4u;

    const float e_bias = g.bias ? g.bias[n0 + i16] : 0.f;
    float head_pre[4] = {0.f, 0.f, 0.f, 0.f};
    if (i16 < C) {
#pragma unroll
        for (int j = 0; j < 4; ++j) head_pre[j] = g.head_w[(n0 + 4 * grp + j) * C + i16];
    }
    const int zrow = tid >> 4, zcls = tid & 15;
    const float zb = (tid < 256 && zcls < C) ? g.head_b[zcls] : 0.f;

    constexpr int KB = 256, CH = KB / 16, AS = KB + 4;
    __shared__ __attribute__((aligned(16))) float a_s[16 * AS];
    f32x4 accq[4] = {{0.f, 0.f, 0.f, 0.f}, {0.f, 0.f, 0.f, 0.f}, {0.f, 0.f, 0.f, 0.f}, {0.f, 0.f, 0.f, 0.f}};
    for (int kb = 0; kb < g.K; kb += KB) {
        u32x4_t av[2];
#pragma unroll
        for (int i = 0; i < 2; ++i) {
            const int piece = tid + i * 512, row = piece >> 6, c4 = piece & 63;
            const uint32_t k = (uint32_t)kb + (uint32_t)c4 * 4u;
            const uint32_t aoff = (m0 + row < g.M && k < K) ? (uint32_t)(m0 + row) * lda4 + k * 4u : OOB;
            av[i] = __builtin_amdgcn_raw_buffer_load_b128(a_rsrc, aoff, 0, 0);
        }
        __builtin_amdgcn_sched_barrier(0);
        float b[CH][4];
#pragma unroll
        for (int c = 0; c < CH; ++c) {
            const uint32_t k = (uint32_t)kb + (uint32_t)c * 16u + (uint32_t)grp * 4u;
#pragma unroll
            for (int j = 0; j < 4; ++j) {
                const uint32_t boff = (k + j < K) ? b_lane + (uint32_t)(kb / 16 + c) * 16u * ldb4 + (uint32_t)j * ldb4 : OOB;
                b[c][j] = __uint_as_float(__builtin_amdgcn_raw_buffer_load_b32(b_rsrc, boff, 0, 0));
            }
        }
        if (kb) __syncthreads();
#pragma unroll
        for (int i = 0; i < 2; ++i) {
            const int piece = tid + i * 512, row = piece >> 6, c4 = piece & 63;
            *reinterpret_cast<u32x4_t*>(a_s + row * AS + 4 * c4) = av[i];
        }
        __syncthreads();
#pragma unroll
        for (int c = 0; c < CH; ++c) {
            const f32x4 a4 = *reinterpret_cast<const f32x4*>(a_s + i16 * AS + 16 * c + 4 * grp);
#pragma unroll
            for (int j = 0; j < 4; ++j) accq[j] = __builtin_amdgcn_mfma_f32_16x16x4f32(a4[j], b[c][j], accq[j], 0, 0, 0);
        }
    }
    const f32x4 acc = (accq[0] + accq[1]) + (accq[2] + accq[3]);

    float* ts = tile_s[wid];
#pragma unroll
    for (int r = 0; r < 4; ++r) {
        float v = acc[r] + e_bias;
        if (g.relu_sign) v = v < 0.f ? -0.0f : fabsf(v);
        else v = v < 0.f ? 0.f : v;
        const int row = m0 + 4 * grp + r;
        if (row < g.M) g.C[(int64_t)row * g.ldc + n0 + i16] = v;
        ts[(4 * grp + r) * 20 + i16] = v;
    }
    __builtin_amdgcn_fence(__ATOMIC_RELEASE, "wavefront");
    __builtin_amdgcn_wave_barrier();
    {
        const f32x4 a4 = *reinterpret_cast<const f32x4*>(ts + i16 * 20 + 4 * grp);
        f32x4 hacc = {0.f, 0.f, 0.f, 0.f};
#pragma unroll
        for (int j = 0; j < 4; ++j) hacc = __builtin_amdgcn_mfma_f32_16x16x4f32(a4[j], head_pre[j], hacc, 0, 0, 0);
#pragma unroll
        for (int q = 0; q < 4; ++q) zred[wid][(4 * grp + q) * 16 + i16] = hacc[q];
    }
    __syncthreads();
    if (tid < 256) {
        const float* zr = &zred[0][zrow * 16 + zcls];
        const float z_nb = ((zr[0] + zr[256]) + (zr[512] + zr[768])) + ((zr[1024] + zr[1280]) + (zr[1536] + zr[1792]));
        const int grow = m0 + zrow;
        const bool valid = zcls < C && grow < g.M;
        if (valid) g.zfull[(int64_t)grow * C + zcls] = z_nb;
        const float z = z_nb + zb;
        float mx = valid ? z : -INFINITY, w;
        w = tnn::dpp_move<0xB1, 0xf>(-INFINITY, mx); mx = w > mx ? w : mx;
        w = tnn::dpp_move<0x4E, 0xf>(-INFINITY, mx); mx = w > mx ? w : mx;
        w = tnn::dpp_move<0x141, 0xf>(-INFINITY, mx); mx = w > mx ? w : mx;
        w = tnn::dpp_move<0x140, 0xf>(-INFINITY, mx); mx = w > mx ? w : mx;
        float se = valid ? expf(z - mx) : 0.f;
        se += tnn::dpp_move<0xB1, 0xf>(0.f, se);
        se += tnn::dpp_move<0x4E, 0xf>(0.f, se);
        se += tnn::dpp_move<0x141, 0xf>(0.f, se);
        se += tnn::dpp_move<0x140, 0xf>(0.f, se);
        const bool speaks = zcls == 0 && grow < g.M;
        const float wm = tnn::wave_max_dpp(speaks ? mx : -INFINITY);
        const float ws = tnn::wave_sum_dpp(speaks ? se * expf(mx - wm) : 0.f);
        if (lane == 0) { wred[wid][0] = wm; wred[wid][1] = ws; }
    }
    __syncthreads();
    if (tid == 0) {
        float M = wred[0][0];
#pragma unroll
        for (int q = 1; q < 4; ++q) M = fmaxf(M, wred[q][0]);
        float S = 0.f;
#pragma unroll
        for (int q = 0; q < 4; ++q) S += wred[q][0] > -INFINITY ? wred[q][1] * expf(wred[q][0] - M) : 0.f;
        if constexpr (MERGE) {
            __hip_atomic_store(g.pairs + 2 * blockIdx.x, M, __ATOMIC_RELAXED, __HIP_MEMORY_SCOPE_SYSTEM);
            __hip_atomic_store(g.pairs + 2 * blockIdx.x + 1, S, __ATOMIC_RELAXED, __HIP_MEMORY_SCOPE_SYSTEM);
        } else {
            g.pairs[2 * blockIdx.x] = M;
            g.pairs[2 * blockIdx.x + 1] = S;
            if (g.bump != nullptr && blockIdx.x == 0) *g.bump += 1u;
        }
    }
    if constexpr (MERGE) {
        __shared__ int is_last;
        if (tid == 0) {
            asm volatile("s_waitcnt vmcnt(0)" ::: "memory");
            const unsigned prev = __hip_atomic_fetch_add(ta.ticket, 1u, __ATOMIC_RELAXED, __HIP_MEMORY_SCOPE_AGENT);
            const int last = prev == gridDim.x - 1 ? 1 : 0;
            if (last) __hip_atomic_store(ta.ticket, 0u, __ATOMIC_RELAXED, __HIP_MEMORY_SCOPE_AGENT);
            is_last = last;
        }
        __syncthreads();
        if (!is_last) return;
        const int n = (int)gridDim.x;
        const bool has = lane < n;
        const float mq = has ? __hip_atomic_load(g.pairs + 2 * lane, __ATOMIC_RELAXED, __HIP_MEMORY_SCOPE_SYSTEM) : -INFINITY;
        const float sq = has ? __hip_atomic_load(g.pairs + 2 * lane + 1, __ATOMIC_RELAXED, __HIP_MEMORY_SCOPE_SYSTEM) : 0.f;
        const float Mm = tnn::wave_max_dpp(mq);
        const float Sm = tnn::wave_sum_dpp(has ? sq * expf(mq - Mm) : 0.f);
        head_tail_finish(ta, ctx, Mm, Sm);
    }
}

template <int WAVES, bool FAST>
__global__ __launch_bounds__(WAVES * 64) void dense_bwd_small_kernel(GemmArgs gw, float* __restrict__ db,
                                                                     GemmArgs gx, int n_dw) {
    __shared__ float red[WAVES][4][64];
    __shared__ float bsum[WAVES][64];
    if constexpr (FAST) {
        if ((int)blockIdx.x < n_dw)
            small_tile_fast<false, false, WAVES, false, false>(gw, db, (int)blockIdx.x, red, bsum);
        else
            small_tile_fast<true, true, WAVES, false, false>(gx, nullptr, (int)blockIdx.x - n_dw, red, bsum);
    } else {
        if ((int)blockIdx.x < n_dw)
            small_tile<false, false, WAVES>(gw, db, (int)blockIdx.x, red, bsum);
        else
            small_tile<true, true, WAVES>(gx, nullptr, (int)blockIdx.x - n_dw, red, bsum);
    }
}

template <int WAVES, bool WIDE = false>
__global__ __launch_bounds__(WAVES * 64) void dense_bwd0_adam_kernel(GemmArgs gw, float* __restrict__ db, AdamEpi ad,
                                                                     int n_dw) {
    __shared__ float red[WAVES][WIDE ? 8 : 4][64];
    __shared__ float bsum[WAVES][WIDE ? 2 : 1][64];
    if ((int)blockIdx.x < n_dw) {
        if constexpr (WIDE) dw_tile_wide<WAVES, true, false>(gw, db, (int)blockIdx.x, red, bsum, &ad);
        else small_tile<false, false, WAVES, true>(gw, db, (int)blockIdx.x, red, reinterpret_cast<float(*)[64]>(bsum), &ad);
        return;
    }
    adam_flat_range<WAVES * 64, true>(ad, (int)blockIdx.x - n_dw, (int)gridDim.x - n_dw);
}

struct ArTileArgs {
    float* buf;
    int64_t n, slice;
    int64_t w_off, b_off;
    int n_dw;
};

#ifdef TNN_AR_TRACE
__device__ unsigned long long g_ar_trace[1024 * 4];
#endif

template <int WAVES, bool WIDE = false>
__global__ __launch_bounds__(WAVES * 64) void dense_bwd0_allreduce_adam_kernel(GemmArgs gw, ArTileArgs f,
                                                                               tnn::p2p::LaunchCtx ctx,
                                                                               tnn::p2p::AdamTail t) {
    using namespace tnn::p2p;
    constexpr int TW = WIDE ? 32 : 16;
    __shared__ float red[WAVES][WIDE ? 8 : 4][64];
    __shared__ float bsum[WAVES][WIDE ? 2 : 1][64];
    __shared__ __attribute__((aligned(16))) float tile[16 * TW + TW];
    const Peers& p = ctx.peers;
    const int tid = threadIdx.x, P = ctx.ar_grid;
    TNN_AR_STAMP(g_ar_trace, blockIdx.x, 4, 1024, 0);
    if ((int)blockIdx.x < f.n_dw) {
        const int b = (int)blockIdx.x % P;
        const uint32_t tag = ctx.ar_epoch[b] + 1;
        const int dead_at_entry = __hip_atomic_load(ctx.dead, __ATOMIC_RELAXED, __HIP_MEMORY_SCOPE_AGENT);
        if constexpr (WIDE) dw_tile_wide<WAVES, false, true>(gw, nullptr, (int)blockIdx.x, red, bsum, nullptr, tile);
        else small_tile<false, false, WAVES, false, true>(gw, nullptr, (int)blockIdx.x, red, reinterpret_cast<float(*)[64]>(bsum), nullptr, tile);
        __syncthreads();
        TNN_AR_STAMP(g_ar_trace, blockIdx.x, 4, 1024, 1);
        constexpr int Q = TW / 4;
        if (tid < 16 * Q + Q && dead_at_entry == 0) {
            int tm, tn;
            small_tile_coords(gw, (int)blockIdx.x, tm, tn);
            const int64_t m0 = (int64_t)tm * 16, n0 = (int64_t)tn * TW;
            int64_t e;
            bool live;
            f32x4 v;
            if (tid < 16 * Q) {
                const int row = tid / Q, c4 = tid % Q;
                live = m0 + row < gw.M && n0 + 4 * c4 < gw.N;
                e = f.w_off + (m0 + row) * gw.ldc + n0 + 4 * c4;
                v = *reinterpret_cast<const f32x4*>(tile + row * TW + 4 * c4);
            } else {
                const int c4 = tid - 16 * Q;
                live = tm == 0 && n0 + 4 * c4 < gw.N;
                e = f.b_off + n0 + 4 * c4;
                v = *reinterpret_cast<const f32x4*>(tile + 16 * TW + 4 * c4);
            }
            if (live) {
                const int q = f.n < (int64_t(1) << 31) ? (int)((uint32_t)e / (uint32_t)f.slice) : (int)(e / f.slice);
                ll_send(p.base[q] + ll_recv_off(p, p.rank, (e - (int64_t)q * f.slice) / 4), v, tag);
            }
        }
        __syncthreads();
        if (tid == 0) __hip_atomic_fetch_add(ctx.ar_gate + b * GATE_STRIDE, 1u, __ATOMIC_RELAXED, __HIP_MEMORY_SCOPE_AGENT);
        TNN_AR_STAMP(g_ar_trace, blockIdx.x, 4, 1024, 2);
        return;
    }
    const int b = (int)blockIdx.x - f.n_dw;
    const uint32_t tag = ctx.ar_epoch[b] + 1;
    unsigned* const gate = ctx.ar_gate + b * GATE_STRIDE;
    SkipRanges skip;
    skip.lo0 = f.w_off; skip.hi0 = f.w_off + gw.M * gw.N;
    skip.lo1 = f.b_off; skip.hi1 = f.b_off + gw.N;
#ifdef TNN_AR_TRACE
    if (blockIdx.x < 1024) skip.trace = g_ar_trace + blockIdx.x * 4;
#endif
    allreduce_body<true, 2>(p, f.buf, f.n, f.slice, tag, ctx.dead, ctx.timeout_ticks, t, (int64_t)b * (WAVES * 64) + tid,
                         (int64_t)P * (WAVES * 64), skip, gate, b < f.n_dw ? (unsigned)((f.n_dw - b + P - 1) / P) : 0u);
    __syncthreads();
    if (tid == 0) {
        __hip_atomic_store(gate, 0u, __ATOMIC_RELAXED, __HIP_MEMORY_SCOPE_AGENT);
        ctx.ar_epoch[b] = tag;
    }
}

__global__ __launch_bounds__(512) void dense_bwd0_mid_allreduce_adam_kernel(GemmArgs gw, ArTileArgs f, tnn::p2p::LaunchCtx ctx,
                                                                            tnn::p2p::AdamTail t) {
    using namespace tnn::p2p;
    __shared__ float red[8][16][64];
    __shared__ float bsum[8][64];
    __shared__ __attribute__((aligned(16))) float tile[32 * 32 + 32];
    const Peers& p = ctx.peers;
    const int tid = threadIdx.x, P = ctx.ar_grid;
    if ((int)blockIdx.x < f.n_dw) {
        const int b = (int)blockIdx.x % P;
        const uint32_t tag = ctx.ar_epoch[b] + 1;
        const AdamEpi none = {};
        const int dead_at_entry = __hip_atomic_load(ctx.dead, __ATOMIC_RELAXED, __HIP_MEMORY_SCOPE_AGENT);
        mid_tile<false, false, false, true>(gw, nullptr, none, (int)blockIdx.x, red, bsum, tile);
        __syncthreads();
        if (tid < 264 && dead_at_entry == 0) {
            int tm, tn;
            small_tile_coords(gw, (int)blockIdx.x, tm, tn);
            const int64_t m0 = (int64_t)tm * 32, n0 = (int64_t)tn * 32;
            int64_t e;
            bool live;
            f32x4 v;
            if (tid < 256) {
                const int row = tid >> 3, c4 = tid & 7;
                live = m0 + row < gw.M && n0 + 4 * c4 < gw.N;
                e = f.w_off + (m0 + row) * gw.ldc + n0 + 4 * c4;
                v = *reinterpret_cast<const f32x4*>(tile + row * 32 + 4 * c4);
            } else {
                const int c4 = tid - 256;
                live = tm == 0 && n0 + 4 * c4 < gw.N;
                e = f.b_off + n0 + 4 * c4;
                v = *reinterpret_cast<const f32x4*>(tile + 1024 + 4 * c4);
            }
            if (live) {
                const int q = f.n < (int64_t(1) << 31) ? (int)((uint32_t)e / (uint32_t)f.slice) : (int)(e / f.slice);
                ll_send(p.base[q] + ll_recv_off(p, p.rank, (e - (int64_t)q * f.slice) / 4), v, tag);
            }
        }
        __syncthreads();
        if (tid == 0) __hip_atomic_fetch_add(ctx.ar_gate + b * GATE_STRIDE, 1u, __ATOMIC_RELAXED, __HIP_MEMORY_SCOPE_AGENT);
        return;
    }
    const int b = (int)blockIdx.x - f.n_dw;
    const uint32_t tag = ctx.ar_epoch[b] + 1;
    unsigned* const gate = ctx.ar_gate + b * GATE_STRIDE;
    SkipRanges skip;
    skip.lo0 = f.w_off; skip.hi0 = f.w_off + gw.M * gw.N;
    skip.lo1 = f.b_off; skip.hi1 = f.b_off + gw.N;
    allreduce_body<true, 2>(p, f.buf, f.n, f.slice, tag, ctx.dead, ctx.timeout_ticks, t, (int64_t)b * 512 + tid, (int64_t)P * 512, skip,
                            gate, b < f.n_dw ? (unsigned)((f.n_dw - b + P - 1) / P) : 0u);
    __syncthreads();
    if (tid == 0) {
        __hip_atomic_store(gate, 0u, __ATOMIC_RELAXED, __HIP_MEMORY_SCOPE_AGENT);
        ctx.ar_epoch[b] = tag;
    }
}

__global__ __launch_bounds__(256) void head_partials_kernel(const float* __restrict__ out, int64_t M, int64_t N, int64_t ldc,
                                                            const float* __restrict__ hw, int hc, float* __restrict__ hz) {
    const int64_t tiles_n = (N + 15) / 16, total = tiles_n * M * hc;
    for (int64_t i = (int64_t)blockIdx.x * blockDim.x + threadIdx.x; i < total; i += (int64_t)gridDim.x * blockDim.x) {
        const int c = (int)(i % hc);
        const int64_t row = (i / hc) % M, tn = i / (hc * M);
        float acc = 0.f;
        for (int col = 0; col < 16 && tn * 16 + col < N; ++col)
            acc = fmaf(out[row * ldc + tn * 16 + col], hw[(tn * 16 + col) * hc + c], acc);
        hz[i] = acc;
    }
}
```

tinynn-autograd_amd/csrc/tnn_head.hip:

```cpp
#include <math.h>
#include <stdio.h>
#include <stdlib.h>

#include "tnn_internal.h"
#include "tnn_tile_order.h"
#include "tnn_p2p.h"
#include <mutex>
#include <unordered_map>

#include "tnn_head_stats.h"

namespace {

typedef float f32x4 __attribute__((ext_vector_type(4)));

struct HeadMArgs {
    int m, rpb;
    int vec;
    int nparts;
    int m_global;
    const float* ext_pairs;
    int ext_n;
    const tnn::p2p::XchgCtx* xc;
    int xw;
    const float *a, *w, *b, *y;
    const float* zpart;
    float *logits, *dz, *stats, *loss, *dw, *db, *da;
    double* tick;
    double b1, b2;
};

template <int C, int NP>
struct HeadStage {
    f32x4 v[NP], yv;
};
template <int C, int NP>
__device__ __forceinline__ void head_stage_request(const HeadMArgs& p, const int t, HeadStage<C, NP>& h) {
    const int n = p.m * C;
    if (p.vec && t < (n >> 2)) {
#pragma unroll
        for (int tn = 0; tn < NP; ++tn) h.v[tn] = *reinterpret_cast<const f32x4*>(p.zpart + (size_t)tn * n + 4 * t);
        h.yv = *reinterpret_cast<const f32x4*>(p.y + 4 * t);
    }
}
template <int C, int NP>
__device__ __forceinline__ f32x4 head_stage_bias(const HeadMArgs& p, const int t) {
    f32x4 b = {0.f, 0.f, 0.f, 0.f};
    if (p.vec) {
#pragma unroll
        for (int i = 0; i < 4; ++i) b[i] = p.b[(4 * t + i) % C];
    }
    return b;
}
template <int C, int NP>
__device__ __forceinline__ void head_stage_store(const HeadMArgs& p, const int t, const HeadStage<C, NP>& h, float* zs, float* ys,
                                                 const f32x4 bias4) {
    static_assert(NP == 8, "the partial-sum tree is written for 8 tiles");
    const int n = p.m * C;
    if (p.vec) {
        if (t < (n >> 2)) {
            f32x4 s = ((h.v[0] + h.v[1]) + (h.v[2] + h.v[3])) + ((h.v[4] + h.v[5]) + (h.v[6] + h.v[7]));
            s += bias4;
            *reinterpret_cast<f32x4*>(zs + 4 * t) = s;
            *reinterpret_cast<f32x4*>(ys + 4 * t) = h.yv;
        }
    } else {
        for (int e = t; e < n; e += 512) {
            float u[NP];
#pragma unroll
            for (int tn = 0; tn < NP; ++tn) u[tn] = p.zpart[(size_t)tn * n + e];
            zs[e] = (((u[0] + u[1]) + (u[2] + u[3])) + ((u[4] + u[5]) + (u[6] + u[7]))) + p.b[e % C];
            ys[e] = p.y[e];
        }
    }
}

template <int H, int C, bool PART, int CUT, bool DA, int SH = 0>
__device__ __forceinline__ void head_block(const HeadMArgs& p, const int g) {
    constexpr int ROWS = 128, ZS = C + 1, WS = 12, JPB = 8, G = H / JPB, KC = H / 16, NP = H / 16;
    static_assert(H == ROWS && C <= 12 && (H * C) % 4 == 0, "thread (t & 127) doubles as the hidden-unit index of the da phase");
    constexpr int TS = ROWS + 16;
    __shared__ float zs[ROWS * ZS];
    __shared__ __attribute__((aligned(16))) float ws[H * WS];
    __shared__ __attribute__((aligned(16))) float dzr[ROWS * WS];
    __shared__ __attribute__((aligned(16))) float dzT[C * TS];
    __shared__ __attribute__((aligned(16))) float asT[JPB * TS];
    __shared__ double red[8][4];
    const int t = threadIdx.x, lane = t & 63, wid = t >> 6;
    const int i16 = lane & 15, grp = lane >> 4;
    const int r = t & (ROWS - 1), kq = t >> 7;
    const int srow = t >> 2, sub = t & 3;
    const int m = p.m;
    const bool slive = srow < m;

    const int sr = min(srow, m - 1);
    float zc[3] = {0.f, 0.f, 0.f}, yc[3];
    __shared__ __attribute__((aligned(16))) float zst[PART ? ROWS * C : 4], yst[PART ? ROWS * C : 4];
    HeadStage<C, NP> stg;
    f32x4 av[PART ? 1 : KC];
    f32x4 bias4 = {0.f, 0.f, 0.f, 0.f};
    if constexpr (PART) {
        head_stage_request<C, NP>(p, t, stg);
        bias4 = head_stage_bias<C, NP>(p, t);
    } else {
        const float* arow = p.a + (size_t)min(16 * wid + i16, m - 1) * H + 4 * grp;
#pragma unroll
        for (int c = 0; c < KC; ++c) av[c] = *reinterpret_cast<const f32x4*>(arow + 16 * c);
    }
    if constexpr (!PART) {
#pragma unroll
        for (int i = 0; i < 3; ++i) yc[i] = p.y[(size_t)sr * C + min(sub + 4 * i, C - 1)];
    }
    constexpr int WV = H * C / 4;
    f32x4 w4 = {0.f, 0.f, 0.f, 0.f};
    if (t < WV) w4 = *reinterpret_cast<const f32x4*>(p.w + 4 * t);
    float am[2] = {0.f, 0.f};
    const int r0 = g * p.rpb, rend = min(m, r0 + p.rpb);
    if constexpr (DA) {
#pragma unroll
        for (int i = 0; i < 2; ++i) am[i] = p.a[(size_t)min(r0 + kq + 4 * i, m - 1) * H + r];
    }
    const f32x4 asl = *reinterpret_cast<const f32x4*>(p.a + (size_t)min((t & 255) >> 1, m - 1) * H + g * JPB + 4 * (t & 1));
    double pw0 = 0.0, pw1 = 0.0;
    if (g == 0 && t == 0 && p.tick) { pw0 = p.tick[0]; pw1 = p.tick[1]; }

    if (t < H) { ws[t * WS + 10] = 0.f; ws[t * WS + 11] = 0.f; }
    if (t < WV) {
#pragma unroll
        for (int i = 0; i < 4; ++i) { const int e = 4 * t + i; ws[(e / C) * WS + e % C] = w4[i]; }
    }
    if (t < 2 * ROWS) {
#pragma unroll
        for (int i = 0; i < 4; ++i) asT[(4 * (t & 1) + i) * TS + (t >> 1)] = (t >> 1) < m ? asl[i] : 0.f;
    }

    if constexpr (PART) {
        head_stage_store<C, NP>(p, t, stg, zst, yst, bias4);
        __syncthreads();
#pragma unroll
        for (int i = 0; i < 3; ++i) {
            zc[i] = zst[sr * C + min(sub + 4 * i, C - 1)];
            yc[i] = yst[sr * C + min(sub + 4 * i, C - 1)];
        }
    } else {
        __syncthreads();
        f32x4 acc0 = {0.f, 0.f, 0.f, 0.f}, acc1 = {0.f, 0.f, 0.f, 0.f};
        const float* wl = ws + (4 * grp) * WS + min(i16, WS - 1);
#pragma unroll
        for (int c = 0; c < KC; ++c) {
            acc0 = __builtin_amdgcn_mfma_f32_16x16x4f32(av[c][0], wl[(16 * c + 0) * WS], acc0, 0, 0, 0);
            acc1 = __builtin_amdgcn_mfma_f32_16x16x4f32(av[c][1], wl[(16 * c + 1) * WS], acc1, 0, 0, 0);
            acc0 = __builtin_amdgcn_mfma_f32_16x16x4f32(av[c][2], wl[(16 * c + 2) * WS], acc0, 0, 0, 0);
            acc1 = __builtin_amdgcn_mfma_f32_16x16x4f32(av[c][3], wl[(16 * c + 3) * WS], acc1, 0, 0, 0);
        }
        if (i16 < C) {
            const float bias = p.b[i16];
#pragma unroll
            for (int q = 0; q < 4; ++q) zs[(16 * wid + 4 * grp + q) * ZS + i16] = (acc0[q] + acc1[q]) + bias;
        }
        __syncthreads();
#pragma unroll
        for (int i = 0; i < 3; ++i) zc[i] = zs[srow * ZS + min(sub + 4 * i, C - 1)];
    }
    if constexpr (CUT == 1) {
        p.da[(size_t)g * 512 + t] = zc[0] + zc[1] + zc[2] + am[0] + am[1] + yc[0];
        return;
    }

    HeadStats st;
    if constexpr (SH == 2) head_stats<C, true, true>(zc, yc, slive, sub, lane, wid, red, st, g == 0, p.ext_pairs, p.ext_n);
    else head_stats<C>(zc, yc, slive, sub, lane, wid, red, st, g == 0);
    if constexpr (SH == 3) {
        __shared__ float xm[2];
        float Mx = st.M, Sx = (float)st.S;
        tnn::p2p::xchg_merge<512>(p.xc, p.xw, Mx, Sx, false, xm);
        st.M = Mx; st.S = (double)Sx;
    }
    const bool (&valid)[3] = st.valid;
    const float (&ec)[3] = st.ec, (&eyc)[3] = st.eyc;
    const float mx = st.mx, urow = st.urow;
    const float M = st.M;
    const double S = st.S;
    const double L = st.L;
    double inv_m = 1.0 / (double)m;
    if constexpr (SH != 0) inv_m = 1.0 / (double)p.m_global;
    if constexpr (CUT == 2) {
        p.da[(size_t)g * 512 + t] = (float)(S + L) + M + am[0] + am[1] + ec[0] + ec[1] + ec[2] + eyc[0];
        return;
    }
    float dzc[3];
    {
        const float sf = slive ? expf(mx - M) * __builtin_amdgcn_rcpf((float)S) : 0.f, uf = slive ? (float)inv_m * __builtin_amdgcn_rcpf(urow) : 0.f;
#pragma unroll
        for (int i = 0; i < 3; ++i) {
            dzc[i] = ec[i] * sf - eyc[i] * uf;
            if (valid[i]) {
                dzr[srow * WS + sub + 4 * i] = dzc[i];
                dzT[(sub + 4 * i) * TS + srow] = dzc[i];
            }
        }
        if (sub >= 2) dzr[srow * WS + 8 + sub] = 0.f;
    }
    __syncthreads();
    if constexpr (CUT == 3) {
        p.da[(size_t)g * 512 + t] = dzr[r * WS] + asT[r] + am[0] + am[1];
        return;
    }

    if (DA && p.da) {
        f32x4 wv[WS / 4];
#pragma unroll
        for (int i = 0; i < WS / 4; ++i) wv[i] = *reinterpret_cast<const f32x4*>(ws + r * WS + 4 * i);
#pragma unroll
        for (int i = 0; i < 2; ++i) {
            const int row = r0 + kq + 4 * i;
            if (row < rend) {
                float d = 0.f;
#pragma unroll
                for (int k = 0; k < WS / 4; ++k) {
                    const f32x4 dv = *reinterpret_cast<const f32x4*>(dzr + row * WS + 4 * k);
#pragma unroll
                    for (int e = 0; e < 4; ++e) d = fmaf(dv[e], wv[k][e], d);
                }
                p.da[(size_t)row * H + r] = (__float_as_uint(am[i]) >> 31) ? 0.f : d;
            }
        }
    }
    if constexpr (CUT == 4) return;
    if (t < JPB * C * 4) {
        const int q = t & 3, o = t >> 2, jl = o / C, c = o - jl * C;
        float s0 = 0.f, s1 = 0.f;
#pragma unroll
        for (int i = 0; i < ROWS / 16; ++i) {
            const f32x4 a4 = *reinterpret_cast<const f32x4*>(asT + jl * TS + 16 * i + 4 * q);
            const f32x4 d4 = *reinterpret_cast<const f32x4*>(dzT + c * TS + 16 * i + 4 * q);
            s0 = fmaf(a4[0], d4[0], s0); s1 = fmaf(a4[1], d4[1], s1);
            s0 = fmaf(a4[2], d4[2], s0); s1 = fmaf(a4[3], d4[3], s1);
        }
        float s = s0 + s1;
        s += tnn::dpp_move<0xB1, 0xf>(0.f, s);
        s += tnn::dpp_move<0x4E, 0xf>(0.f, s);
        if (q == 0) p.dw[(size_t)(g * JPB + jl) * C + c] = s;
    }
    if constexpr (CUT == 5) return;
    if (g == 0) {
        if (wid == 7) {
            const int c = min(lane & 15, C - 1), rq = lane >> 4;
            f32x4 acc = {0.f, 0.f, 0.f, 0.f};
#pragma unroll
            for (int i = 0; i < ROWS / 16; ++i) acc += *reinterpret_cast<const f32x4*>(dzT + c * TS + 32 * rq + 4 * i);
            float s = (acc[0] + acc[1]) + (acc[2] + acc[3]);
            s += __shfl_xor(s, 16, 64);
            s += __shfl_xor(s, 32, 64);
            if (lane < C) p.db[lane] = s;
        }
        if (t == 0) {
            if (p.loss) p.loss[0] = SH != 0 ? (float)((((double)logf((float)S) + (double)M) * (double)m - L) * inv_m)
                                       : (float)((double)logf((float)S) + (double)M - L * inv_m);
            if (p.stats) { p.stats[0] = M; p.stats[1] = (float)S; }
            if (p.tick) { p.tick[0] = pw0 * p.b1; p.tick[1] = pw1 * p.b2; }
        }
    }
    if (g == G - 1 && slive) {
#pragma unroll
        for (int i = 0; i < 3; ++i)
            if (valid[i]) {
                if (p.logits) p.logits[(size_t)srow * C + sub + 4 * i] = zc[i];
                if (p.dz) p.dz[(size_t)srow * C + sub + 4 * i] = dzc[i];
            }
    }
}

template <int H, int C, bool PART, int CUT = 0>
__global__ __launch_bounds__(512) void mlp_head_multi_kernel(HeadMArgs p) {
    head_block<H, C, PART, CUT, true>(p, (int)blockIdx.x);
}

struct HeadBwdArgs {
    const float* x;
    const float* w1;
    float *dw1, *db1, *dx;
    int n_in, tiles_in;
    int n_dw;
    tnn::TileOrder ord_dw, ord_dx;
    int dx_wide;
};

#ifdef TNN_STEP_TRACE
__device__ unsigned long long g_step_trace_head[1024 * 4];
#endif

template <int H, int C, int CUT = 0, int SH = 0>
__global__ __launch_bounds__(512) void mlp_head_bwd_kernel(HeadMArgs p, HeadBwdArgs q) {
    constexpr int ROWS = 128, WS = 12, NP = H / 16, G = H / 8, TH = H / 16, PS = H + 4;
    static_assert(H == 128 && NP == 8, "one 16-deep K chunk per wave, 8 waves");
    TNN_STEP_STAMP(g_step_trace_head, 0, 0);
    if ((int)blockIdx.x < G) {
        head_block<H, C, true, 0, false, SH>(p, (int)blockIdx.x);
        TNN_STEP_STAMP_ACKED(g_step_trace_head, 0, 3);
        return;
    }
    __shared__ __attribute__((aligned(16))) float zs[ROWS * C], ys[ROWS * C];
    __shared__ __attribute__((aligned(16))) float dzr[ROWS * WS];
    __shared__ __attribute__((aligned(16))) float pan[16 * PS];
    __shared__ float redm[8][8][64];
    __shared__ float bsum[8][64];
    __shared__ double red[8][4];
    const int t = threadIdx.x, lane = t & 63, wid = t >> 6;
    const int i16 = lane & 15, grp = lane >> 4;
    const int srow = t >> 2, sub = t & 3;
    const int m = p.m;
    const bool slive = srow < m;
    const int sr = min(srow, m - 1);
    const int n_dw = q.n_dw;
    const int blk = (int)blockIdx.x - G;
    const bool is_dw = blk < n_dw;
    const bool wide = q.dx_wide != 0;
    const int n_in = q.n_in;
    int tm, tn;
    tnn::tile_coords(is_dw ? q.ord_dw : q.ord_dx, is_dw ? blk : blk - n_dw, tm, tn);
    const int m0 = tm * 16, n0 = tn * ((!is_dw && wide) ? 32 : 16);

    HeadStage<C, NP> stg;
    head_stage_request<C, NP>(p, t, stg);
    const f32x4 bias4 = head_stage_bias<C, NP>(p, t);
    const int urow = (is_dw ? n0 : 16 * wid) + i16;
    const int prow0 = (is_dw ? 16 * wid : m0) + 4 * grp;
    float w2f[3], a1m[4];
#pragma unroll
    for (int s3 = 0; s3 < 3; ++s3) w2f[s3] = p.w[(size_t)urow * C + min(4 * s3 + grp, C - 1)];
#pragma unroll
    for (int r = 0; r < 4; ++r) a1m[r] = p.a[(size_t)min(prow0 + r, m - 1) * H + urow];
    const int e_r = (t >> 6) & 3, e_ln = t & 63;
    float xq[4];
#pragma unroll
    for (int j = 0; j < 4; ++j) {
        const int xrow = is_dw ? 16 * wid + 4 * grp + j : m0 + 4 * grp + e_r;
        const int xcol = (is_dw ? m0 : n0 + ((j == 1 && wide) ? 16 : 0)) + i16;
        xq[j] = q.x[(size_t)min(xrow, m - 1) * n_in + xcol];
    }
    const int wrow = (is_dw ? 0 : n0) + i16, wrow1 = wrow + ((!is_dw && wide) ? 16 : 0);
    const f32x4 bf = *reinterpret_cast<const f32x4*>(q.w1 + (size_t)wrow * H + 16 * wid + 4 * grp);
    const f32x4 bf1 = *reinterpret_cast<const f32x4*>(q.w1 + (size_t)wrow1 * H + 16 * wid + 4 * grp);
    float af[4] = {xq[0], xq[1], xq[2], xq[3]};
    float e_pre = xq[0], e_pre1 = xq[1];
    if (grp >= 2) w2f[2] = 0.f;
    static_assert(C == 10, "the zero columns of the K = 12 product are written for 10 classes");

    TNN_STEP_STAMP_ACKED(g_step_trace_head, 0, 1);
    head_stage_store<C, NP>(p, t, stg, zs, ys, bias4);
    __syncthreads();
    float zc[3], yc[3];
#pragma unroll
    for (int i = 0; i < 3; ++i) {
        zc[i] = zs[sr * C + min(sub + 4 * i, C - 1)];
        yc[i] = ys[sr * C + min(sub + 4 * i, C - 1)];
    }
    if constexpr (CUT == 1) {
        q.dx[(size_t)(blk % 64) * 512 + t] = zc[0] + zc[1] + zc[2] + yc[0] + w2f[0] + w2f[1] + w2f[2] + a1m[0] + a1m[1] + a1m[2] + a1m[3] + af[0] + af[1] + af[2] + af[3] + bf[0] + e_pre;
        return;
    }
    HeadStats st;
    if constexpr (SH == 2) head_stats<C, false, true>(zc, yc, slive, sub, lane, wid, red, st, false, p.ext_pairs, p.ext_n);
    else head_stats<C, false>(zc, yc, slive, sub, lane, wid, red, st);
    if constexpr (SH == 3) {
        __shared__ float xm[2];
        float Mx = st.M, Sx = (float)st.S;
        tnn::p2p::xchg_merge<512>(p.xc, p.xw, Mx, Sx, blk == 0, xm);
        st.M = Mx; st.S = (double)Sx;
    }
    if constexpr (CUT == 2) {
        q.dx[(size_t)(blk % 64) * 512 + t] = (float)st.S + st.M + st.ec[0] + st.eyc[1] + w2f[0] + w2f[1] + w2f[2] + a1m[0] + a1m[1] + a1m[2] + a1m[3] + af[0] + af[1] + af[2] + af[3] + bf[0] + e_pre;
        return;
    }
    float m_norm = (float)m;
    if constexpr (SH != 0) m_norm = (float)p.m_global;
    {
        const float sf = slive ? expf(st.mx - st.M) * __builtin_amdgcn_rcpf((float)st.S) : 0.f;
        const float uf = slive ? __builtin_amdgcn_rcpf(m_norm * st.urow) : 0.f;
#pragma unroll
        for (int i = 0; i < 3; ++i)
            if (st.valid[i]) dzr[srow * WS + sub + 4 * i] = st.ec[i] * sf - st.eyc[i] * uf;
        if (sub >= 2) dzr[srow * WS + 8 + sub] = 0.f;
    }
    if (is_dw) { __builtin_amdgcn_fence(__ATOMIC_RELEASE, "wavefront"); __builtin_amdgcn_wave_barrier(); }
    else __syncthreads();
    if constexpr (CUT == 3) {
        q.dx[(size_t)(blk % 64) * 512 + t] = dzr[t] + w2f[0] + w2f[1] + w2f[2] + a1m[0] + a1m[1] + a1m[2] + a1m[3] + af[0] + af[1] + af[2] + af[3] + bf[0] + e_pre;
        return;
    }

    f32x4 pz = {0.f, 0.f, 0.f, 0.f};
    {
        const float* drow = dzr + ((is_dw ? 16 * wid : m0) + i16) * WS + grp;
#pragma unroll
        for (int s3 = 0; s3 < 3; ++s3) pz = __builtin_amdgcn_mfma_f32_16x16x4f32(drow[4 * s3], w2f[s3], pz, 0, 0, 0);
#pragma unroll
        for (int r = 0; r < 4; ++r) pz[r] = (__float_as_uint(a1m[r]) >> 31) ? 0.f : pz[r];
    }
    f32x4 acc = {0.f, 0.f, 0.f, 0.f}, acc1 = {0.f, 0.f, 0.f, 0.f};
    float bs = 0.f;
    if (is_dw) {
        if constexpr (CUT == 4) {
            q.dx[(size_t)(blk % 64) * 512 + t] = pz[0] + pz[1] + pz[2] + pz[3] + af[0] + af[1] + af[2] + af[3];
            return;
        }
#pragma unroll
        for (int j = 0; j < 4; ++j) acc = __builtin_amdgcn_mfma_f32_16x16x4f32(af[j], pz[j], acc, 0, 0, 0);
        bs = (pz[0] + pz[1]) + (pz[2] + pz[3]);
    } else {
#pragma unroll
        for (int r = 0; r < 4; ++r) pan[(4 * grp + r) * PS + 16 * wid + i16] = pz[r];
        __syncthreads();
        if constexpr (CUT == 4) {
            q.dx[(size_t)(blk % 64) * 512 + t] = pan[t] + bf[0] + e_pre;
            return;
        }
        const f32x4 a4 = *reinterpret_cast<const f32x4*>(pan + i16 * PS + 16 * wid + 4 * grp);
#pragma unroll
        for (int j = 0; j < 4; ++j) acc = __builtin_amdgcn_mfma_f32_16x16x4f32(a4[j], bf[j], acc, 0, 0, 0);
        if (wide) {
#pragma unroll
            for (int j = 0; j < 4; ++j) acc1 = __builtin_amdgcn_mfma_f32_16x16x4f32(a4[j], bf1[j], acc1, 0, 0, 0);
        }
    }
#pragma unroll
    for (int r = 0; r < 4; ++r) redm[wid][r][lane] = acc[r];
    if (!is_dw && wide) {
#pragma unroll
        for (int r = 0; r < 4; ++r) redm[wid][4 + r][lane] = acc1[r];
    }
    bsum[wid][lane] = bs;
    __syncthreads();
    TNN_STEP_STAMP(g_step_trace_head, 0, 2);
    asm volatile("" : "+v"(e_pre), "+v"(e_pre1));
    if (t < 256) {
        float s = 0.f;
#pragma unroll
        for (int w = 0; w < 8; ++w) s += redm[w][e_r][e_ln];
        const int row = m0 + (e_ln >> 4) * 4 + e_r, col = n0 + (e_ln & 15);
        if (is_dw) q.dw1[(size_t)row * H + col] = s;
        else if (row < m) {
            q.dx[(size_t)row * n_in + col] = (__float_as_uint(e_pre) >> 31) ? 0.f : s;
            if (wide) {
                float s1 = 0.f;
#pragma unroll
                for (int w = 0; w < 8; ++w) s1 += redm[w][4 + e_r][e_ln];
                q.dx[(size_t)row * n_in + col + 16] = (__float_as_uint(e_pre1) >> 31) ? 0.f : s1;
            }
        }
    }
    if (is_dw && tm == 0 && t < 16) {
        float s = 0.f;
#pragma unroll
        for (int w = 0; w < 8; ++w) s += (bsum[w][t] + bsum[w][16 + t]) + (bsum[w][32 + t] + bsum[w][48 + t]);
        q.db1[n0 + t] = s;
    }
    TNN_STEP_STAMP_ACKED(g_step_trace_head, 0, 3);
}

template <int C, int NP>
__device__ __forceinline__ void head_stage_request_rb(const HeadMArgs& p, const int t, HeadStage<C, NP>& h, const int mb, const int row0) {
    const int n = mb * C, stride = p.m * C, base = row0 * C;
    if (p.vec && t < (n >> 2)) {
#pragma unroll
        for (int tn = 0; tn < NP; ++tn) {
            h.v[tn] = f32x4{0.f, 0.f, 0.f, 0.f};
            if (tn < p.nparts) h.v[tn] = *reinterpret_cast<const f32x4*>(p.zpart + (size_t)tn * stride + base + 4 * t);
        }
        h.yv = *reinterpret_cast<const f32x4*>(p.y + base + 4 * t);
    }
}
template <int C, int NP>
__device__ __forceinline__ void head_stage_store_rb(const HeadMArgs& p, const int t, const HeadStage<C, NP>& h, float* zs, float* ys,
                                                 const int mb, const int row0, const f32x4 bias4) {
    static_assert(NP == 8, "the partial-sum tree is written for 8 tiles");
    const int n = mb * C, stride = p.m * C, base = row0 * C;
    if (p.vec) {
        if (t < (n >> 2)) {
            f32x4 s = ((h.v[0] + h.v[1]) + (h.v[2] + h.v[3])) + ((h.v[4] + h.v[5]) + (h.v[6] + h.v[7]));
            s += bias4;
            *reinterpret_cast<f32x4*>(zs + 4 * t) = s;
            *reinterpret_cast<f32x4*>(ys + 4 * t) = h.yv;
        }
    } else {
#pragma unroll 1
        for (int e = t; e < n; e += 512) {
            float u[NP];
#pragma unroll
            for (int tn = 0; tn < NP; ++tn) u[tn] = tn < p.nparts ? p.zpart[(size_t)tn * stride + base + e] : 0.f;
            zs[e] = (((u[0] + u[1]) + (u[2] + u[3])) + ((u[4] + u[5]) + (u[6] + u[7]))) + p.b[e % C];
            ys[e] = p.y[base + e];
        }
    }
}

template <int H, int C, bool PART, int CUT, bool DA, int SH = 0, bool RB = false>
__device__ __forceinline__ void head_block_rb(const HeadMArgs& p, const int g) {
    constexpr int ROWS = 128, ZS = C + 1, WS = 12, JPB = 8, G = H / JPB, KC = H / 16, NP = H / 16;
    static_assert(H == ROWS && C <= 12 && (H * C) % 4 == 0, "thread (t & 127) doubles as the hidden-unit index of the da phase");
    static_assert(!RB || (SH >= 2 && PART && !DA && CUT == 0), "row blocks exist in the form that takes the statistics from memory only");
    constexpr int TS = ROWS + 16;
    __shared__ float zs[ROWS * ZS];
    __shared__ __attribute__((aligned(16))) float ws[H * WS];
    __shared__ __attribute__((aligned(16))) float dzr[ROWS * WS];
    __shared__ __attribute__((aligned(16))) float dzT[C * TS];
    __shared__ __attribute__((aligned(16))) float asT[JPB * TS];
    __shared__ double red[8][4];
    __shared__ __attribute__((aligned(16))) float zst[PART ? ROWS * C : 4], yst[PART ? ROWS * C : 4];
    const int t = threadIdx.x, lane = t & 63, wid = t >> 6;
    const int i16 = lane & 15, grp = lane >> 4;
    const int r = t & (ROWS - 1), kq = t >> 7;
    const int srow = t >> 2, sub = t & 3;
    const int nb = RB ? (p.m + ROWS - 1) / ROWS : 1;

    constexpr int WV = H * C / 4;
    f32x4 w4 = {0.f, 0.f, 0.f, 0.f};
    if (t < WV) w4 = *reinterpret_cast<const f32x4*>(p.w + 4 * t);
    double pw0 = 0.0, pw1 = 0.0;
    if (g == 0 && t == 0 && p.tick) { pw0 = p.tick[0]; pw1 = p.tick[1]; }

    f32x4 bias4 = {0.f, 0.f, 0.f, 0.f};
    if constexpr (PART) bias4 = head_stage_bias<C, NP>(p, t);
    float ext_ms[2] = {0.f, 0.f};
    if constexpr (SH >= 2) head_merge_pairs(p.ext_pairs, p.ext_n, lane, ext_ms[0], ext_ms[1]);
    if constexpr (SH == 3) {
        __shared__ float xm[2];
        tnn::p2p::xchg_merge<512>(p.xc, p.xw, ext_ms[0], ext_ms[1], false, xm);
    }
    float dws0 = 0.f, dws1 = 0.f;
    f32x4 dbacc = {0.f, 0.f, 0.f, 0.f};
    double Lsum = 0.0;
    float M = 0.f;
    double S = 0.0;
    HeadStage<C, NP> stg_nx;
    f32x4 asl_nx = {0.f, 0.f, 0.f, 0.f};
    constexpr bool PF = true;
    if constexpr (RB && PF) {
        const int m0b = min(ROWS, p.m);
        head_stage_request_rb<C, NP>(p, t, stg_nx, m0b, 0);
        asl_nx = *reinterpret_cast<const f32x4*>(p.a + (size_t)min((t & 255) >> 1, m0b - 1) * H + g * JPB + 4 * (t & 1));
    }
    for (int rb = 0; rb < nb; ++rb) {
    int row0 = rb * ROWS;
    if constexpr (RB) asm volatile("" : "+s"(row0));
    const int m = RB ? min(ROWS, p.m - row0) : p.m;
    const float* const a_rb = p.a + (size_t)row0 * H;
    const bool slive = srow < m;
    if (rb) __syncthreads();
    int tt = t;
    if constexpr (RB) asm volatile("" : "+v"(tt));

    const int sr = min(srow, m - 1);
    float zc[3] = {0.f, 0.f, 0.f}, yc[3];
    HeadStage<C, NP> stg;
    f32x4 av[PART ? 1 : KC];
    if constexpr (PART) {
        if constexpr (RB && PF) stg = stg_nx;
        else head_stage_request_rb<C, NP>(p, tt, stg, m, row0);
    } else {
        const float* arow = a_rb + (size_t)min(16 * wid + i16, m - 1) * H + 4 * grp;
#pragma unroll
        for (int c = 0; c < KC; ++c) av[c] = *reinterpret_cast<const f32x4*>(arow + 16 * c);
    }
    if constexpr (!PART) {
#pragma unroll
        for (int i = 0; i < 3; ++i) yc[i] = p.y[(size_t)(row0 + sr) * C + min(sub + 4 * i, C - 1)];
    }
    float am[2] = {0.f, 0.f};
    const int r0 = g * p.rpb, rend = min(m, r0 + p.rpb);
    if constexpr (DA) {
#pragma unroll
        for (int i = 0; i < 2; ++i) am[i] = a_rb[(size_t)min(r0 + kq + 4 * i, m - 1) * H + r];
    }
    f32x4 asl;
    if constexpr (RB && PF) asl = asl_nx;
    else asl = *reinterpret_cast<const f32x4*>(a_rb + (size_t)min((t & 255) >> 1, m - 1) * H + g * JPB + 4 * (t & 1));

    if (rb == 0) {
        if (t < H) { ws[t * WS + 10] = 0.f; ws[t * WS + 11] = 0.f; }
        if (t < WV) {
#pragma unroll
            for (int i = 0; i < 4; ++i) { const int e = 4 * t + i; ws[(e / C) * WS + e % C] = w4[i]; }
        }
    }
    if (t < 2 * ROWS) {
#pragma unroll
        for (int i = 0; i < 4; ++i) asT[(4 * (t & 1) + i) * TS + (t >> 1)] = (t >> 1) < m ? asl[i] : 0.f;
    }

    if constexpr (PART) {
        head_stage_store_rb<C, NP>(p, t, stg, zst, yst, m, row0, bias4);
        if constexpr (RB && PF) {
            if (rb + 1 < nb) {
                const int m1 = min(ROWS, p.m - row0 - ROWS);
                head_stage_request_rb<C, NP>(p, tt, stg_nx, m1, row0 + ROWS);
                asl_nx = *reinterpret_cast<const f32x4*>(a_rb + (size_t)(ROWS + min((tt & 255) >> 1, m1 - 1)) * H + g * JPB + 4 * (tt & 1));
            }
        }
        __syncthreads();
#pragma unroll
        for (int i = 0; i < 3; ++i) {
            zc[i] = zst[sr * C + min(sub + 4 * i, C - 1)];
            yc[i] = yst[sr * C + min(sub + 4 * i, C - 1)];
        }
    } else {
        __syncthreads();
        f32x4 acc0 = {0.f, 0.f, 0.f, 0.f}, acc1 = {0.f, 0.f, 0.f, 0.f};
        const float* wl = ws + (4 * grp) * WS + min(i16, WS - 1);
#pragma unroll
        for (int c = 0; c < KC; ++c) {
            acc0 = __builtin_amdgcn_mfma_f32_16x16x4f32(av[c][0], wl[(16 * c + 0) * WS], acc0, 0, 0, 0);
            acc1 = __builtin_amdgcn_mfma_f32_16x16x4f32(av[c][1], wl[(16 * c + 1) * WS], acc1, 0, 0, 0);
            acc0 = __builtin_amdgcn_mfma_f32_16x16x4f32(av[c][2], wl[(16 * c + 2) * WS], acc0, 0, 0, 0);
            acc1 = __builtin_amdgcn_mfma_f32_16x16x4f32(av[c][3], wl[(16 * c + 3) * WS], acc1, 0, 0, 0);
        }
        if (i16 < C) {
            const float bias = p.b[i16];
#pragma unroll
            for (int q = 0; q < 4; ++q) zs[(16 * wid + 4 * grp + q) * ZS + i16] = (acc0[q] + acc1[q]) + bias;
        }
        __syncthreads();
#pragma unroll
        for (int i = 0; i < 3; ++i) zc[i] = zs[srow * ZS + min(sub + 4 * i, C - 1)];
    }
    if constexpr (CUT == 1) {
        p.da[(size_t)g * 512 + t] = zc[0] + zc[1] + zc[2] + am[0] + am[1] + yc[0];
        return;
    }

    HeadStats st;
    if constexpr (SH >= 2) head_stats<C, true, true>(zc, yc, slive, sub, lane, wid, red, st, !RB && g == 0, ext_ms, 0);
    else head_stats<C>(zc, yc, slive, sub, lane, wid, red, st, g == 0);
    const bool (&valid)[3] = st.valid;
    const float (&ec)[3] = st.ec, (&eyc)[3] = st.eyc;
    const float mx = st.mx, urow = st.urow;
    M = st.M;
    S = st.S;
    if constexpr (RB) { if (g == 0 && slive && sub == 0) Lsum += (double)logf(urow) + (double)mx; }
    else Lsum += st.L;
    double inv_m = 1.0 / (double)m;
    if constexpr (SH != 0) inv_m = 1.0 / (double)p.m_global;
    if constexpr (CUT == 2) {
        p.da[(size_t)g * 512 + t] = (float)(S + st.L) + M + am[0] + am[1] + ec[0] + ec[1] + ec[2] + eyc[0];
        return;
    }
    float dzc[3];
    {
        const float sf = slive ? expf(mx - M) * __builtin_amdgcn_rcpf((float)S) : 0.f, uf = slive ? (float)inv_m * __builtin_amdgcn_rcpf(urow) : 0.f;
#pragma unroll
        for (int i = 0; i < 3; ++i) {
            dzc[i] = ec[i] * sf - eyc[i] * uf;
            if (valid[i]) {
                dzr[srow * WS + sub + 4 * i] = dzc[i];
                dzT[(sub + 4 * i) * TS + srow] = dzc[i];
            }
        }
        if (sub >= 2) dzr[srow * WS + 8 + sub] = 0.f;
    }
    __syncthreads();
    if constexpr (CUT == 3) {
        p.da[(size_t)g * 512 + t] = dzr[r * WS] + asT[r] + am[0] + am[1];
        return;
    }

    if (DA && p.da) {
        f32x4 wv[WS / 4];
#pragma unroll
        for (int i = 0; i < WS / 4; ++i) wv[i] = *reinterpret_cast<const f32x4*>(ws + r * WS + 4 * i);
#pragma unroll
        for (int i = 0; i < 2; ++i) {
            const int row = r0 + kq + 4 * i;
            if (row < rend) {
                float d = 0.f;
#pragma unroll
                for (int k = 0; k < WS / 4; ++k) {
                    const f32x4 dv = *reinterpret_cast<const f32x4*>(dzr + row * WS + 4 * k);
#pragma unroll
                    for (int e = 0; e < 4; ++e) d = fmaf(dv[e], wv[k][e], d);
                }
                p.da[(size_t)row * H + r] = (__float_as_uint(am[i]) >> 31) ? 0.f : d;
            }
        }
    }
    if constexpr (CUT == 4) return;
    if (t < JPB * C * 4) {
        const int q = t & 3, o = t >> 2, jl = o / C, c = o - jl * C;
#pragma unroll
        for (int i = 0; i < ROWS / 16; ++i) {
            const f32x4 a4 = *reinterpret_cast<const f32x4*>(asT + jl * TS + 16 * i + 4 * q);
            const f32x4 d4 = *reinterpret_cast<const f32x4*>(dzT + c * TS + 16 * i + 4 * q);
            dws0 = fmaf(a4[0], d4[0], dws0); dws1 = fmaf(a4[1], d4[1], dws1);
            dws0 = fmaf(a4[2], d4[2], dws0); dws1 = fmaf(a4[3], d4[3], dws1);
        }
    }
    if (g == 0 && wid == 7) {
        const int c = min(lane & 15, C - 1), rq = lane >> 4;
#pragma unroll
        for (int i = 0; i < ROWS / 16; ++i) dbacc += *reinterpret_cast<const f32x4*>(dzT + c * TS + 32 * rq + 4 * i);
    }
    if (g == G - 1 && slive) {
#pragma unroll
        for (int i = 0; i < 3; ++i)
            if (valid[i]) {
                if (p.logits) p.logits[(size_t)(row0 + srow) * C + sub + 4 * i] = zc[i];
                if (p.dz) p.dz[(size_t)(row0 + srow) * C + sub + 4 * i] = dzc[i];
            }
    }
    }

    if (t < JPB * C * 4) {
        const int q = t & 3, o = t >> 2, jl = o / C, c = o - jl * C;
        float s = dws0 + dws1;
        s += tnn::dpp_move<0xB1, 0xf>(0.f, s);
        s += tnn::dpp_move<0x4E, 0xf>(0.f, s);
        if (q == 0) p.dw[(size_t)(g * JPB + jl) * C + c] = s;
    }
    if constexpr (CUT == 5) return;
    if constexpr (RB) {
        if (g == 0) {
            const double wl = tnn::wave_sum_dpp(Lsum);
            __syncthreads();
            if (lane == 0) red[wid][2] = wl;
            __syncthreads();
            Lsum = ((red[0][2] + red[1][2]) + (red[2][2] + red[3][2])) + ((red[4][2] + red[5][2]) + (red[6][2] + red[7][2]));
        }
    }
    if (g == 0) {
        if (wid == 7) {
            float s = (dbacc[0] + dbacc[1]) + (dbacc[2] + dbacc[3]);
            s += __shfl_xor(s, 16, 64);
            s += __shfl_xor(s, 32, 64);
            if (lane < C) p.db[lane] = s;
        }
        if (t == 0) {
            const double inv_all = 1.0 / (double)(SH != 0 ? p.m_global : p.m);
            if (p.loss) p.loss[0] = SH != 0 ? (float)((((double)logf((float)S) + (double)M) * (double)p.m - Lsum) * inv_all)
                                       : (float)((double)logf((float)S) + (double)M - Lsum * inv_all);
            if (p.stats) { p.stats[0] = M; p.stats[1] = (float)S; }
            if (p.tick) { p.tick[0] = pw0 * p.b1; p.tick[1] = pw1 * p.b2; }
        }
    }
}

template <int H, int C, int CUT = 0, int SH = 0, bool RB = false>
__global__ __launch_bounds__(512, RB ? 4 : 2) void mlp_head_bwd_rb_kernel(HeadMArgs p, HeadBwdArgs q) {
    constexpr int ROWS = 128, WS = 12, NP = H / 16, G = H / 8, TH = H / 16, PS = H + 4;
    static_assert(H == 128 && NP == 8, "one 16-deep K chunk per wave, 8 waves");
    TNN_STEP_STAMP(g_step_trace_head, 0, 0);
    if ((int)blockIdx.x < G) {
        head_block_rb<H, C, true, 0, false, SH, RB>(p, (int)blockIdx.x);
        TNN_STEP_STAMP_ACKED(g_step_trace_head, 0, 3);
        return;
    }
    __shared__ __attribute__((aligned(16))) float zs[ROWS * C], ys[ROWS * C];
    __shared__ __attribute__((aligned(16))) float dzr[ROWS * WS];
    __shared__ __attribute__((aligned(16))) float pan[16 * PS];
    __shared__ float redm[8][8][64];
    __shared__ float bsum[8][64];
    __shared__ double red[8][4];
    const int t = threadIdx.x, lane = t & 63, wid = t >> 6;
// ... 287 lines not shown
                tnn::p2p::xchg_merge<256>(p.xc, p.xw, M, Sx, blk == 0, xm);
                S = (double)Sx;
            }
        }
        if (t < n) {
            const float sf = live ? expf(mx - M) / (float)S : 0.f, uf = live ? (float)inv_m / qy : 0.f;
#pragma unroll
            for (int k = 0; k < CMAX; ++k) {
                const float d = live ? e[k] * sf - e[k] * yv[k] * uf : 0.f;
                dzs[t * CS + k] = d;
                if (write_out && p.dz && live && k < C) p.dz[(size_t)r * C + k] = d;
            }
        }
        __syncthreads();
        return live ? mx + logf(qy) : 0.f;
    };
    const int nblk = ext ? (m + ROWS - 1) / ROWS : 1;
    const bool par = p.ws != nullptr && nblk > 1;
    const int units = G + n_dw, role_blocks = par ? units * nblk : units;
    constexpr int SLOT = 288;
    __shared__ int last_flag;
    auto publish = [&](const int unit, const int rb, const float mine, const int n_main, const float bsum, const int n_b,
                       const double lsum_total) -> bool {
        float* slot = p.ws + ((size_t)unit * nblk + rb) * SLOT;
        if (t < n_main) __hip_atomic_store(slot + t, mine, __ATOMIC_RELAXED, __HIP_MEMORY_SCOPE_SYSTEM);
        if (t < n_b) __hip_atomic_store(slot + 256 + t, bsum, __ATOMIC_RELAXED, __HIP_MEMORY_SCOPE_SYSTEM);
        if (t == 0) __hip_atomic_store(reinterpret_cast<double*>(slot + 272), lsum_total, __ATOMIC_RELAXED, __HIP_MEMORY_SCOPE_SYSTEM);
        asm volatile("s_waitcnt vmcnt(0)" ::: "memory");
        __syncthreads();
        if (t == 0) {
            const unsigned prev = __hip_atomic_fetch_add(p.tickets + unit, 1u, __ATOMIC_RELAXED, __HIP_MEMORY_SCOPE_AGENT);
            const int last = prev == (unsigned)nblk - 1 ? 1 : 0;
            if (last) __hip_atomic_store(p.tickets + unit, 0u, __ATOMIC_RELAXED, __HIP_MEMORY_SCOPE_AGENT);
            last_flag = last;
        }
        __syncthreads();
        return last_flag != 0;
    };
    auto gather = [&](const int unit, const int off) -> float {
        float acc = 0.f;
        for (int rb = 0; rb < nblk; ++rb)
            acc += __hip_atomic_load(p.ws + ((size_t)unit * nblk + rb) * SLOT + off, __ATOMIC_RELAXED, __HIP_MEMORY_SCOPE_SYSTEM);
        return acc;
    };

    if (blk < role_blocks && (par ? blk / nblk : blk) < G) {
        const int g = par ? blk / nblk : blk, rb_lo = par ? blk % nblk : 0, rb_hi = par ? rb_lo + 1 : nblk;
        const int j = t / C, c = t - j * C;
        float s0 = 0.f, s1 = 0.f, dbs = 0.f;
        double lsum = 0.0;
        for (int rb = rb_lo; rb < rb_hi; ++rb) {
            const int row0 = rb * ROWS;
            const float lq = block_dz(row0, ROWS, g == G - 1);
            if (ext && g == 0) lsum += (double)lq;
#pragma unroll
            for (int i = t; i < ROWS * 16; i += 256) {
                const int r = i >> 4, jj = i & 15;
                pan[r * CS + jj] = row0 + r < m ? p.a[(size_t)(row0 + r) * H + 16 * g + jj] : 0.f;
            }
            __syncthreads();
            if (t < 16 * C) {
#pragma unroll 8
                for (int r = 0; r < ROWS; r += 2) {
                    s0 = fmaf(pan[r * CS + j], dzs[r * CS + c], s0);
                    s1 = fmaf(pan[(r + 1) * CS + j], dzs[(r + 1) * CS + c], s1);
                }
            }
            if (g == 0 && t < C)
                for (int r = 0; r < ROWS; ++r) dbs += dzs[r * CS + t];
            if (rb + 1 < rb_hi) __syncthreads();
        }
        if (g == 0 && ext) {
            lsum = tnn::wave_sum(lsum);
            __syncthreads();
            if (lane == 0) red[wid] = lsum;
            __syncthreads();
            L = (red[0] + red[1]) + (red[2] + red[3]);
        }
        float dw_v = s0 + s1;
        if (par) {
            if (!publish(g, rb_lo, dw_v, 16 * C, dbs, g == 0 ? C : 0, g == 0 ? L : 0.0)) return;
            if (t < 16 * C) dw_v = gather(g, t);
            if (g == 0) {
                if (t < C) dbs = gather(g, 256 + t);
                L = 0.0;
                for (int rb = 0; rb < nblk; ++rb)
                    L += __hip_atomic_load(reinterpret_cast<const double*>(p.ws + ((size_t)g * nblk + rb) * SLOT + 272), __ATOMIC_RELAXED,
                                           __HIP_MEMORY_SCOPE_SYSTEM);
            }
        }
        if (t < 16 * C) p.dw[(size_t)(16 * g + j) * C + c] = dw_v;
        if (g == 0) {
            if (t < C) p.db[t] = dbs;
            if (t == 0) {
                if (p.loss) p.loss[0] = dp ? (float)((((double)logf((float)S) + (double)M) * (double)m - L) * inv_m)
                                           : (float)((double)logf((float)S) + (double)M - L * inv_m);
                if (p.stats) { p.stats[0] = M; p.stats[1] = (float)S; }
                if (p.tick) {
                    if (par) { pw0 = p.tick[0]; pw1 = p.tick[1]; }
                    p.tick[0] = pw0 * p.b1;
                    p.tick[1] = pw1 * p.b2;
                }
            }
        }
        return;
    }
    if (blk < role_blocks) {
        const int unit = par ? blk / nblk : blk, rb_lo = par ? blk % nblk : 0, rb_hi = par ? rb_lo + 1 : nblk;
        const int b2 = unit - G, tm = b2 % tiles_in, tn = b2 / tiles_in, m0 = tm * 16, n0 = tn * 16;
        const int ti = t >> 4, tj = t & 15;
        float s0 = 0.f, s1 = 0.f, dbs = 0.f;
        for (int rb = rb_lo; rb < rb_hi; ++rb) {
            const int row0 = rb * ROWS;
            block_dz(row0, ROWS, false);
            float av8[8], xv8[8];
#pragma unroll
            for (int u = 0; u < 8; ++u) {
                const int i = t + 256 * u, r = i >> 4, j = i & 15;
                const bool ok = row0 + r < m;
                av8[u] = ok ? p.a[(size_t)(row0 + r) * H + n0 + j] : 0.f;
                xv8[u] = ok ? p.x[(size_t)(row0 + r) * n_in + m0 + j] : 0.f;
            }
#pragma unroll
            for (int u = 0; u < 8; ++u) {
                const int i = t + 256 * u, r = i >> 4, j = i & 15;
                float acc = 0.f;
                for (int c = 0; c < C; ++c) acc = fmaf(dzs[r * CS + c], w2s[(n0 + j) * C + c], acc);
                pan[r * CS + j] = (row0 + r < m && !(__float_as_uint(av8[u]) >> 31)) ? acc : 0.f;
                xs[r * CS + j] = xv8[u];
            }
            __syncthreads();
#pragma unroll 8
            for (int r = 0; r < ROWS; r += 2) {
                s0 = fmaf(xs[r * CS + ti], pan[r * CS + tj], s0);
                s1 = fmaf(xs[(r + 1) * CS + ti], pan[(r + 1) * CS + tj], s1);
            }
            if (tm == 0 && t < 16)
                for (int r = 0; r < ROWS; ++r) dbs += pan[r * CS + t];
            if (rb + 1 < rb_hi) __syncthreads();
        }
        float dw_v = s0 + s1;
        if (par) {
            if (!publish(unit, rb_lo, dw_v, 256, dbs, tm == 0 ? 16 : 0, 0.0)) return;
            dw_v = gather(unit, t);
            if (tm == 0 && t < 16) dbs = gather(unit, 256 + t);
        }
        p.dw1[(size_t)(m0 + ti) * H + n0 + tj] = dw_v;
        if (tm == 0 && t < 16) p.db1[n0 + t] = dbs;
        return;
    }
    {
        const int b3 = blk - role_blocks, tr = (m + 15) / 16, tm = b3 % tr, tn = b3 / tr, m0 = tm * 16, n0 = tn * 16;
        const int HS = H + 1;
        const int dz0 = ext ? m0 : 0;
        block_dz(dz0, ext ? 16 : ROWS, false);
        for (int i = t; i < 16 * H; i += 256) {
            const int rr = i / H, j = i - rr * H, r = m0 + rr;
            float d1 = 0.f;
            if (r < m) {
                const float av = p.a[(size_t)r * H + j];
                float acc = 0.f;
                for (int c = 0; c < C; ++c) acc = fmaf(dzs[(r - dz0) * CS + c], w2s[j * C + c], acc);
                d1 = (__float_as_uint(av) >> 31) ? 0.f : acc;
            }
            pz[rr * HS + j] = d1;
            w1s[rr * HS + j] = p.w1[(size_t)(n0 + rr) * H + j];
        }
        __syncthreads();
        const int rr = t >> 4, i = t & 15, r = m0 + rr;
        float s0 = 0.f, s1 = 0.f;
#pragma unroll 8
        for (int j = 0; j < H; j += 2) {
            s0 = fmaf(pz[rr * HS + j], w1s[i * HS + j], s0);
            s1 = fmaf(pz[rr * HS + j + 1], w1s[i * HS + j + 1], s1);
        }
        if (r < m) {
            const float xv = p.x[(size_t)r * n_in + n0 + i];
            p.dx[(size_t)r * n_in + n0 + i] = (__float_as_uint(xv) >> 31) ? 0.f : s0 + s1;
        }
    }
}

struct HeadWs {
    float* slots = nullptr;
    unsigned* tickets = nullptr;
    size_t slot_floats = 0;
    int units = 0;
};
std::mutex g_head_ws_mu;
std::unordered_map<hipStream_t, HeadWs> g_head_ws;

bool head_workspace(hipStream_t st, int units, int nblk, HeadWs* out) {
    std::lock_guard<std::mutex> lk(g_head_ws_mu);
    HeadWs& w = g_head_ws[st];
    constexpr size_t CAP_FLOATS = ((size_t)16 << 20) / 4;
    constexpr int MAX_UNITS = (int)(CAP_FLOATS / (2 * 288));
    const size_t need = (size_t)units * nblk * 288;
    if (need > CAP_FLOATS || units > MAX_UNITS) return false;
    if (w.slots != nullptr) { *out = w; return true; }
    hipStreamCaptureStatus cs = hipStreamCaptureStatusNone;
    if (hipStreamIsCapturing(st, &cs) != hipSuccess || cs != hipStreamCaptureStatusNone) return false;
    if (hipMalloc(&w.slots, CAP_FLOATS * 4) != hipSuccess) { (void)hipGetLastError(); w = HeadWs(); return false; }
    if (hipMalloc(&w.tickets, (size_t)MAX_UNITS * 4) != hipSuccess || hipMemset(w.tickets, 0, (size_t)MAX_UNITS * 4) != hipSuccess) {
        (void)hipGetLastError();
        (void)hipFree(w.slots);
        w = HeadWs();
        return false;
    }
    w.slot_floats = CAP_FLOATS;
    w.units = MAX_UNITS;
    *out = w;
    return true;
}

bool head_bwd_generic_fits(int64_t rows, int64_t n_in, int64_t n_hidden, int64_t n_classes, int dtype, bool ext = false) {
    return dtype == TNN_F32 && rows >= 1 && rows <= (ext ? 1024 : 128) && n_hidden % 16 == 0 && n_hidden >= 16 &&
           n_hidden <= 256 && n_classes >= 1 && n_classes <= 16 && n_in >= 16 && n_in % 16 == 0;
}

constexpr int kHeadBwdMaxIn = 16 * (tnn::kTileOrderMaxTiles / 64);

bool head_multi_fits(int64_t rows, int64_t n_hidden, int64_t n_classes, int dtype) {
    return dtype == TNN_F32 && n_classes == 10 && n_hidden == 128 && rows >= 1 && rows <= 128;
}

int head_bwd_orders(HeadBwdArgs& q, const int tr) {
    q.n_dw = tnn::head_tile_orders(q.tiles_in, tr, q.dx_wide != 0, q.ord_dw, q.ord_dx);
    return q.n_dw + tr * (q.dx_wide ? q.tiles_in / 2 : q.tiles_in);
}

int head_bwd_launch(const char* fn, const float* ext_pairs, int ext_n, bool whole_logits, int64_t m_global, int64_t rows, int64_t n_in, int64_t n_hidden, int64_t n_classes, const void* x, const void* w1,
                          const tnn::p2p::XchgCtx* xc, const int xw,
                          const void* a, const void* w, const void* b, const void* y, const void* logit_partials,
                          void* logits, void* dz, void* stats, void* loss, void* dw, void* db, void* dw1, void* db1,
                          void* dx, int dtype, void* adam_pows_f64, double b1, double b2) {
    TNN_NEED_INIT();
    TNN_REQUIRE(rows > 0 && n_in > 0 && n_hidden > 0 && n_classes > 0, "%s: empty head", fn);
    TNN_REQUIRE(x && w1 && a && w && b && y && logit_partials && dw && db && dw1 && db1 && dx,
                "%s: x, w1, a, w, b, y, logit_partials, dw, db, dw1, db1 and dx are required", fn);
    auto al = [](const void* ptr) { return (reinterpret_cast<uintptr_t>(ptr) & 15) == 0; };
    if (!head_multi_fits(1, n_hidden, n_classes, dtype) && !whole_logits &&
        head_bwd_generic_fits(rows, n_in, n_hidden, n_classes, dtype, ext_pairs != nullptr)) {
        TNN_REQUIRE(ext_pairs == nullptr || (m_global >= rows && ext_n >= 1 && ext_n <= 64), "%s: m_global < rows or bad pair count", fn);
        HeadGenArgs ga;
        ga.m = (int)rows; ga.H = (int)n_hidden; ga.C = (int)n_classes; ga.n_in = (int)n_in;
        ga.m_global = (int)m_global; ga.ext_n = ext_n; ga.ext_pairs = ext_pairs; ga.xc = xc; ga.xw = xw;
        TNN_REQUIRE(xc == nullptr || (ext_pairs == nullptr && m_global >= rows),
                    "%s: the deferred exchange of a generic head is the <= 128-row form (statistics inside)", fn);
        ga.a = (const float*)a; ga.w = (const float*)w; ga.b = (const float*)b; ga.y = (const float*)y;
        ga.zpart = (const float*)logit_partials; ga.x = (const float*)x; ga.w1 = (const float*)w1;
        ga.logits = (float*)logits; ga.dz = (float*)dz; ga.stats = (float*)stats; ga.loss = (float*)loss;
        ga.dw = (float*)dw; ga.db = (float*)db; ga.dw1 = (float*)dw1; ga.db1 = (float*)db1; ga.dx = (float*)dx;
        ga.tick = (double*)adam_pows_f64; ga.b1 = b1; ga.b2 = b2;
        const int gh = (int)(n_hidden / 16), ti = (int)(n_in / 16);
        const int units = gh + ti * gh, nblk = ext_pairs != nullptr ? (int)((rows + 127) / 128) : 1;
        ga.ws = nullptr; ga.tickets = nullptr;
        HeadWs hw;
        if (nblk > 1 && head_workspace(tnn::stream(), units, nblk, &hw)) { ga.ws = hw.slots; ga.tickets = hw.tickets; }
        const int grid = units * (ga.ws ? nblk : 1) + (int)((rows + 15) / 16) * ti;
        hipLaunchKernelGGL(mlp_head_bwd_generic_kernel, grid, 256, 0, tnn::stream(), ga);
        TNN_LAUNCH_OK();
        return 0;
    }
    TNN_REQUIRE(head_multi_fits(ext_pairs ? (rows <= 1024 ? 1 : rows) : rows, n_hidden, n_classes, dtype) && n_in % 16 == 0 &&
                    n_in <= kHeadBwdMaxIn && al(a) && al(w) && al(w1),
                "%s: this head does not fit the merged form (tnn_mlp_head_fits, n_in %% 16 == 0 up to %d, 16-B aligned a / w / w1)", fn,
                kHeadBwdMaxIn);
    HeadMArgs p;
    p.m = (int)rows;
    p.rpb = (int)((rows + 15) / 16);
    p.a = (const float*)a; p.w = (const float*)w; p.b = (const float*)b; p.y = (const float*)y;
    p.zpart = (const float*)logit_partials;
    p.vec = (rows % 2 == 0 && ((reinterpret_cast<uintptr_t>(y) | reinterpret_cast<uintptr_t>(logit_partials)) & 15) == 0) ? 1 : 0;
    p.m_global = (int)m_global;
    p.ext_pairs = ext_pairs; p.ext_n = ext_n; p.xc = xc; p.xw = xw;
    TNN_REQUIRE(!whole_logits || rows > 128, "%s: whole logits (n_pairs < 0) come from the row-panel forward, i.e. with more than 128 rows", fn);
    p.nparts = whole_logits ? 1 : 8;
    p.logits = (float*)logits; p.dz = (float*)dz; p.stats = (float*)stats; p.loss = (float*)loss;
    p.dw = (float*)dw; p.db = (float*)db; p.da = nullptr;
    p.tick = (double*)adam_pows_f64; p.b1 = b1; p.b2 = b2;
    HeadBwdArgs q;
    q.x = (const float*)x; q.w1 = (const float*)w1;
    q.dw1 = (float*)dw1; q.db1 = (float*)db1; q.dx = (float*)dx;
    q.n_in = (int)n_in; q.tiles_in = (int)(n_in / 16);
    static const bool dx_wide_off = getenv("TNN_HEAD_DX_WIDE") && atoi(getenv("TNN_HEAD_DX_WIDE")) == 0;
    static const bool dx_wide_rb_off = getenv("TNN_HEAD_DX_WIDE_RB") && atoi(getenv("TNN_HEAD_DX_WIDE_RB")) == 0;
    q.dx_wide = (q.tiles_in % 2 == 0 && !dx_wide_off && (rows <= 128 || !dx_wide_rb_off)) ? 1 : 0;
    const int grid = 16 + head_bwd_orders(q, (int)((rows + 15) / 16));
    if (xc != nullptr) {
        TNN_REQUIRE(m_global >= rows && (rows <= 128 ? ext_pairs == nullptr : (ext_pairs != nullptr && ext_n >= 1 && ext_n <= 64)),
                    "%s: m_global < rows, or the pairs do not match the row count", fn);
        if (rows > 128) hipLaunchKernelGGL((mlp_head_bwd_rb_kernel<128, 10, 0, 3, true>), grid, 512, 0, tnn::stream(), p, q);
        else hipLaunchKernelGGL((mlp_head_bwd_kernel<128, 10, 0, 3>), grid, 512, 0, tnn::stream(), p, q);
        TNN_LAUNCH_OK();
        return 0;
    }
    if (ext_pairs != nullptr) {
        TNN_REQUIRE(m_global >= rows && ext_n >= 1 && ext_n <= 64, "%s: m_global < rows or bad pair count", fn);
        if (rows > 128) hipLaunchKernelGGL((mlp_head_bwd_rb_kernel<128, 10, 0, 2, true>), grid, 512, 0, tnn::stream(), p, q);
        else hipLaunchKernelGGL((mlp_head_bwd_kernel<128, 10, 0, 2>), grid, 512, 0, tnn::stream(), p, q);
        TNN_LAUNCH_OK();
        return 0;
    }
    hipLaunchKernelGGL((mlp_head_bwd_kernel<128, 10>), grid, 512, 0, tnn::stream(), p, q);
    TNN_LAUNCH_OK();
    return 0;
}


}

extern "C" {

#ifdef TNN_STEP_TRACE
__attribute__((visibility("default"))) int tnn_debug_step_trace_head(unsigned long long* out, int n) {
    TNN_CHECK_HIP(hipDeviceSynchronize());
    TNN_CHECK_HIP(hipMemcpyFromSymbol(out, HIP_SYMBOL(g_step_trace_head), (size_t)(n < 4096 ? n : 4096) * 8));
    return 0;
}
#endif

int tnn_mlp_head(int64_t rows, int64_t n_hidden, int64_t n_classes, const void* a, const void* w,
                 const void* b, const void* y, void* logits, void* dz, void* stats, void* loss, void* dw,
                 void* db, void* da, int dtype) {
    TNN_NEED_INIT();
    TNN_REQUIRE(rows > 0 && n_hidden > 0 && n_classes > 0, "tnn_mlp_head: empty head");
    TNN_REQUIRE(logits != nullptr && dz != nullptr && dw != nullptr && db != nullptr,
                "tnn_mlp_head: logits, dz, dw and db buffers are required");
    if (int rc = tnn_gemm_bias_act(0, 0, rows, n_classes, n_hidden, a, n_hidden, w, n_classes, b, TNN_ACT_NONE, 0,
                                   logits, n_classes, dtype))
        return rc;
    if (int rc = tnn_softmax_nll_fused(logits, y, rows, n_classes, stats, loss, dz, dtype)) return rc;
    return tnn_dense_bwd(rows, n_hidden, n_classes, a, dz, w, dw, db, da, a, dtype);
}

int tnn_mlp_head_fits(int64_t rows, int64_t n_hidden, int64_t n_classes, int dtype, int* fits) {
    TNN_REQUIRE(fits != nullptr, "tnn_mlp_head_fits: fits is NULL");
    *fits = head_multi_fits(rows, n_hidden, n_classes, dtype) ? 1 : 0;
    return 0;
}

int tnn_mlp_head_bwd_fits(int64_t rows, int64_t n_in, int64_t n_hidden, int64_t n_classes, int dtype, int* fits) {
    TNN_REQUIRE(fits != nullptr, "tnn_mlp_head_bwd_fits: fits is NULL");
    *fits = ((head_multi_fits(rows, n_hidden, n_classes, dtype) && n_in % 16 == 0 && n_in >= 16 && n_in <= kHeadBwdMaxIn) ||
             head_bwd_generic_fits(rows, n_in, n_hidden, n_classes, dtype)) ? 1 : 0;
    return 0;
}

int tnn_mlp_head_bwd_reserve(int64_t max_rows, int64_t n_in, int64_t n_hidden, int64_t n_classes) {
    TNN_NEED_INIT();
    if (head_multi_fits(1, n_hidden, n_classes, TNN_F32) || !head_bwd_generic_fits(max_rows < 1024 ? max_rows : 1024, n_in, n_hidden, n_classes, TNN_F32, true))
        return 0;
    const int nblk = (int)(((max_rows < 1024 ? max_rows : 1024) + 127) / 128);
    HeadWs hw;
    if (nblk > 1) (void)head_workspace(tnn::stream(), (int)(n_hidden / 16 + n_in / 16 * (n_hidden / 16)), nblk, &hw);
    return 0;
}

int tnn_mlp_head_tick(int64_t rows, int64_t n_hidden, int64_t n_classes, const void* a, const void* w,
                      const void* b, const void* y, const void* logit_partials, void* logits, void* dz, void* stats,
                      void* loss, void* dw, void* db, void* da, int dtype, void* adam_pows_f64, double b1, double b2) {
    TNN_NEED_INIT();
    TNN_REQUIRE(rows > 0 && n_hidden > 0 && n_classes > 0, "tnn_mlp_head_tick: empty head");
    TNN_REQUIRE(a && w && b && y && dw && db, "tnn_mlp_head_tick: a, w, b, y, dw and db are required");
    TNN_REQUIRE(head_multi_fits(rows, n_hidden, n_classes, dtype) && (reinterpret_cast<uintptr_t>(a) & 15) == 0,
                "tnn_mlp_head_tick: this head does not fit the one-launch form (ask tnn_mlp_head_fits first)");
    HeadMArgs p;
    p.m = (int)rows;
    p.rpb = (int)((rows + 15) / 16);
    p.a = (const float*)a; p.w = (const float*)w; p.b = (const float*)b; p.y = (const float*)y;
    p.zpart = (const float*)logit_partials;
    p.vec = (rows % 2 == 0 && ((reinterpret_cast<uintptr_t>(y) | reinterpret_cast<uintptr_t>(logit_partials)) & 15) == 0) ? 1 : 0;
    p.m_global = 0;
    p.ext_pairs = nullptr; p.ext_n = 0; p.xc = nullptr; p.xw = 1;
    p.nparts = 8;
    p.logits = (float*)logits; p.dz = (float*)dz; p.stats = (float*)stats; p.loss = (float*)loss;
    p.dw = (float*)dw; p.db = (float*)db; p.da = (float*)da;
    p.tick = (double*)adam_pows_f64; p.b1 = b1; p.b2 = b2;
    hipStream_t st = tnn::stream();
    if (p.zpart) hipLaunchKernelGGL((mlp_head_multi_kernel<128, 10, true>), 16, 512, 0, st, p);
    else hipLaunchKernelGGL((mlp_head_multi_kernel<128, 10, false>), 16, 512, 0, st, p);
    TNN_LAUNCH_OK();
    return 0;
}

int tnn_mlp_head_bwd_tick(int64_t rows, int64_t n_in, int64_t n_hidden, int64_t n_classes, const void* x, const void* w1,
                          const void* a, const void* w, const void* b, const void* y, const void* logit_partials,
                          void* logits, void* dz, void* stats, void* loss, void* dw, void* db, void* dw1, void* db1,
                          void* dx, int dtype, void* adam_pows_f64, double b1, double b2) {
    return head_bwd_launch("tnn_mlp_head_bwd_tick", nullptr, 0, false, 0, rows, n_in, n_hidden, n_classes, x, w1, nullptr, 1, a, w, b, y, logit_partials, logits,
                           dz, stats, loss, dw, db, dw1, db1, dx, dtype, adam_pows_f64, b1, b2);
}

int tnn_mlp_head_bwd_tick_ext(int64_t rows, int64_t m_global, int64_t n_in, int64_t n_hidden, int64_t n_classes,
                              const void* x, const void* w1, const void* a, const void* w, const void* b, const void* y,
                              const void* logit_partials, const void* stats_pairs, int n_pairs, void* logits, void* dz,
                              void* stats, void* loss, void* dw, void* db, void* dw1, void* db1, void* dx, int dtype,
                              void* adam_pows_f64, double b1, double b2) {
    TNN_REQUIRE(stats_pairs != nullptr && m_global >= 1, "tnn_mlp_head_bwd_tick_ext: stats_pairs and m_global are required");
    return head_bwd_launch("tnn_mlp_head_bwd_tick_ext", (const float*)stats_pairs, n_pairs < 0 ? -n_pairs : n_pairs, n_pairs < 0, m_global, rows, n_in, n_hidden,
                           n_classes, x, w1, nullptr, 1, a, w, b, y, logit_partials, logits, dz, stats, loss, dw, db, dw1, db1, dx, dtype,
                           adam_pows_f64, b1, b2);
}

int tnn_mlp_head_bwd_xchg_fits(int64_t rows, int64_t n_in, int64_t n_hidden, int64_t n_classes, int dtype, int* fits) {
    TNN_REQUIRE(fits != nullptr, "tnn_mlp_head_bwd_xchg_fits: fits is NULL");
    *fits = 0;
    if (!tnn::initialised() || tnn::p2p_xchg_ctx() == nullptr || dtype != TNN_F32 || rows < 1 || n_in < 16 || n_in % 16) return 0;
    const bool tuned = head_multi_fits(1, n_hidden, n_classes, dtype);
    int grid = 0, per_cu = 0;
    if (tuned && rows <= 1024) {
        static const bool dx_wide_off = getenv("TNN_HEAD_DX_WIDE") && atoi(getenv("TNN_HEAD_DX_WIDE")) == 0;
        static const bool dx_wide_rb_off = getenv("TNN_HEAD_DX_WIDE_RB") && atoi(getenv("TNN_HEAD_DX_WIDE_RB")) == 0;
        const int ti = (int)(n_in / 16), dx_cols = (ti % 2 == 0 && !dx_wide_off && (rows <= 128 || !dx_wide_rb_off)) ? ti / 2 : ti;
        grid = 16 + ti * 8 + (int)((rows + 15) / 16) * dx_cols;
        static int per_cu_small = -1, per_cu_rb = -1;
        if (per_cu_small < 0) {
            if (hipOccupancyMaxActiveBlocksPerMultiprocessor(&per_cu_small, mlp_head_bwd_kernel<128, 10, 0, 3>, 512, 0) != hipSuccess) per_cu_small = 0;
            if (hipOccupancyMaxActiveBlocksPerMultiprocessor(&per_cu_rb, mlp_head_bwd_rb_kernel<128, 10, 0, 3, true>, 512, 0) != hipSuccess) per_cu_rb = 0;
            (void)hipGetLastError();
        }
        per_cu = rows <= 128 ? per_cu_small : per_cu_rb;
    } else if (!tuned && head_bwd_generic_fits(rows, n_in, n_hidden, n_classes, dtype, false)) {
        const int gh = (int)(n_hidden / 16), ti = (int)(n_in / 16);
        grid = gh + ti * gh + (int)((rows + 15) / 16) * ti;
        static int per_cu_gen = -1;
        if (per_cu_gen < 0) {
            if (hipOccupancyMaxActiveBlocksPerMultiprocessor(&per_cu_gen, mlp_head_bwd_generic_kernel, 256, 0) != hipSuccess) per_cu_gen = 0;
            (void)hipGetLastError();
        }
        per_cu = per_cu_gen;
    } else {
        return 0;
    }
    const int shared = tnn::p2p_ranks_on_my_device();
    static const bool force = getenv("TNN_DP_XCHG") && atoi(getenv("TNN_DP_XCHG")) == 2;
    if (shared <= 1 || force || (int64_t)shared * grid <= (int64_t)per_cu * tnn::num_cus()) *fits = 1;
    return 0;
}

int tnn_mlp_head_bwd_tick_xchg(int64_t rows, int64_t m_global, int64_t n_in, int64_t n_hidden, int64_t n_classes,
                               const void* x, const void* w1, const void* a, const void* w, const void* b, const void* y,
                               const void* logit_partials, const void* shard_pairs, int n_pairs, void* logits, void* dz,
                               void* stats, void* loss, void* dw, void* db, void* dw1, void* db1, void* dx, int dtype,
                               void* adam_pows_f64, double b1, double b2) {
    TNN_NEED_INIT();
    TNN_REQUIRE(m_global >= 1 && n_pairs <= 0 && (n_pairs == 0 || shard_pairs != nullptr),
                "tnn_mlp_head_bwd_tick_xchg: m_global >= 1, n_pairs = 0 (statistics inside) or < 0 (row-panel pairs of this shard)");
    if (int rc = tnn::p2p_refuse_if_failed("tnn_mlp_head_bwd_tick_xchg")) return rc;
    const tnn::p2p::XchgCtx* xc = tnn::p2p_xchg_ctx();
    TNN_REQUIRE(xc != nullptr, "tnn_mlp_head_bwd_tick_xchg: the peer-to-peer transport is not enabled");
    int rank = 0, world = 1;
    (void)tnn::p2p_world(&rank, &world);
    return head_bwd_launch("tnn_mlp_head_bwd_tick_xchg", n_pairs < 0 ? (const float*)shard_pairs : nullptr, -n_pairs, n_pairs < 0, m_global,
                           rows, n_in, n_hidden, n_classes, x, w1, xc, world, a, w, b, y, logit_partials, logits, dz, stats, loss, dw, db, dw1,
                           db1, dx, dtype, adam_pows_f64, b1, b2);
}

}
```

tinynn-autograd_amd/csrc/tnn_tile_order.h:

```cpp
#pragma once
#include <stdint.h>

#if defined(__HIPCC__) || defined(__CUDACC__)
#define TNN_TILE_ORDER_HD __host__ __device__ __forceinline__
#else
#define TNN_TILE_ORDER_HD inline
#endif

namespace tnn {

constexpr int kTileOrderMaxTiles = 65535;

struct TileOrder {
    uint64_t magic;
    uint32_t pm, pn;
    uint32_t xcd_mask, xcd_shift;
    uint32_t xm_mask, xm_shift;
};

inline TileOrder tile_order(int tiles_m, int tiles_n, int xg_m, int xg_n) {
    TileOrder o = {};
    const bool cut = xg_m != 0;
    o.pm = (uint32_t)(cut ? tiles_m / xg_m : tiles_m);
    o.pn = (uint32_t)(cut ? tiles_n / xg_n : 0);
    if (o.pm == 0) o.pm = 1;
    o.magic = (uint64_t(1) << 32) / o.pm + 1;
    o.xcd_mask = cut ? 7u : 0u;
    o.xcd_shift = cut ? 3u : 0u;
    o.xm_mask = cut ? (uint32_t)xg_m - 1u : 0u;
    for (int x = xg_m; x > 1; x >>= 1) ++o.xm_shift;
    return o;
}

inline int head_tile_orders(int tiles_in, int tr, bool dx_wide, TileOrder& ord_dw, TileOrder& ord_dx) {
    constexpr int TH = 8;
    const int tcols = dx_wide ? tiles_in / 2 : tiles_in, n_dw = tiles_in * TH;
    const bool cut_dw = tiles_in % 2 == 0, cut_dx = tr % 2 == 0 && tcols % 4 == 0 && n_dw % 8 == 0;
    ord_dw = tile_order(tiles_in, TH, cut_dw ? 2 : 0, cut_dw ? 4 : 0);
    ord_dx = tile_order(tr, tcols, cut_dx ? 2 : 0, cut_dx ? 4 : 0);
    return n_dw;
}

TNN_TILE_ORDER_HD uint32_t tile_div(uint32_t n, uint64_t magic) {
    return (uint32_t)(((uint64_t)n * magic) >> 32);
}

TNN_TILE_ORDER_HD void tile_coords(const TileOrder& o, const int block, int& tm, int& tn) {
    const uint32_t b = (uint32_t)block, xcd = b & o.xcd_mask, idx = b >> o.xcd_shift;
    const uint32_t q = tile_div(idx, o.magic), r = idx - q * o.pm;
    tm = (int)((xcd & o.xm_mask) * o.pm + r);
    tn = (int)((xcd >> o.xm_shift) * o.pn + q);
}

}
```

Before: 7.615 million samples/s.

## Pass first-needed kernel args as leading scalars and move late loads after GEMM start

```diff
diff --git a/tinynn-autograd_amd/csrc/tnn_gemm.hip b/tinynn-autograd_amd/csrc/tnn_gemm.hip
--- a/tinynn-autograd_amd/csrc/tnn_gemm.hip
+++ b/tinynn-autograd_amd/csrc/tnn_gemm.hip
@@ -1,5 +1,6 @@
 #include <math.h>
 #include <stdlib.h>
+#include <string.h>
 
 #include <algorithm>
 
@@ -115,6 +116,17 @@
     f.hc4 = (uint32_t)g.head_c * 4u;
 }
 
+int g_small_args_form = -1;
+int g_bwd0_args_form = -1;
+
+bool step_args_struct_forced(const char* part) {
+    const char* e = getenv("TNN_STEP_ARGS");
+    if (e == nullptr || strncmp(e, "struct", 6) != 0) return false;
+    return e[6] == 0 || (e[6] == ':' && strstr(e + 7, part) != nullptr);
+}
+
+bool placed_at_once(int64_t workgroups) { return workgroups <= tnn::num_cus(); }
+
 template <int WAVES>
 int launch_small(GemmArgs& g, int transA, int transB, float* colsum) {
     small_geometry(g);
@@ -123,6 +135,20 @@
     const bool fast = small_fast_ok(g, transA, transB);
     pick_xcd_cut(g);
     if (fast) fill_small_fast(g, !transA, transB != 0);
+    tnn::PackedTileOrder po;
+    const char* part = WAVES == 4 ? "fwd4" : WAVES == 8 ? "fwd8" : "fwd16";
+    if (fast && placed_at_once(grid.x) && !step_args_struct_forced(part) && tnn::pack_tile_order(g.ord, po)) {
+        const SmallFast& f = g.f;
+        po.w[2] |= (f.h_bytes != 0u ? FAST_FLAG_HEAD : 0u) << tnn::kPackedOrderFlagShift;
+        with_layout(transA, transB, [&](auto akc, auto bkc) {
+            hipLaunchKernelGGL((gemm_small_pre_f32_kernel<decltype(akc)::value, decltype(bkc)::value, WAVES>), grid, WAVES * 64, 0, s,
+                               f.A, f.B, f.a_bytes, f.b_bytes, f.lda4, f.ldb4, f.M, f.N, f.K, po.w[0], po.w[1], po.w[2], g, colsum);
+        });
+        g_small_args_form = 1;
+        TNN_LAUNCH_OK();
+        return 0;
+    }
+    g_small_args_form = 0;
     with_layout(transA, transB, [&](auto akc, auto bkc) {
         tnn::with_flag(fast, [&](auto f) {
             hipLaunchKernelGGL((gemm_small_f32_kernel<decltype(akc)::value, decltype(bkc)::value, WAVES, decltype(f)::value>), grid,
@@ -449,6 +475,13 @@
     return !off && g.N % 32 == 0 && ((g.M + 15) / 16) * (g.N / 32) >= 256 && g.epi == EPI_AXPBY && g.beta == 0.f;
 }
 
+static bool pack_dw_dims(const GemmArgs& g, uint32_t& dims) {
+    if (g.M < 1 || g.M > 0xffff || g.N < 32 || g.N % 32 != 0 || g.N / 32 > 0xff || g.K < 1 || g.K > 256) return false;
+    if (g.lda != g.M || g.ldb != g.N || g.ldc != g.N) return false;
+    dims = (uint32_t)g.M | (uint32_t)(g.N / 32) << 16 | (uint32_t)(g.K - 1) << 24;
+    return true;
+}
+
 int tnn_dense_bwd_first_adam(int64_t rows, int64_t n_in, int64_t n_out, const void* x, const void* dz, void* dw, void* db,
                              void* p_w, void* m_w, void* v_w, void* p_b, void* m_b, void* v_b, void* flat_p,
                              const void* flat_g, void* flat_m, void* flat_v, int64_t flat_n, double lr, double b1,
@@ -456,6 +489,7 @@
     TNN_NEED_INIT();
     TNN_REQUIRE(rows > 0 && n_in > 0 && n_out > 0, "tnn_dense_bwd_first_adam: empty layer");
     TNN_REQUIRE(pows_f64 && p_w && m_w && v_w && p_b && m_b && v_b, "tnn_dense_bwd_first_adam: optimizer state is required");
+    g_bwd0_args_form = 0;
     if (dtype == TNN_F32) {
         GemmArgs gw = gemm_args(x, n_in, dz, n_out, dw, n_out, n_in, n_out, rows, EPI_AXPBY);
         if (use_small_path(gw) && tn_extents_ok(gw)) {
@@ -488,6 +522,16 @@
                 pick_xcd_cut(gw);
                 const int n_wide = gw.tiles_m * gw.tiles_n;
                 const int extra = adam_flat_blocks(ad.fp, ad.fg, ad.fm, ad.fv, ad.fn, 256);
+                tnn::PackedTileOrder po;
+                uint32_t dims;
+                if (!step_args_struct_forced("bwd0") && tnn::pack_tile_order(gw.ord, po) && n_wide <= 0xffff && pack_dw_dims(gw, dims)) {
+                    po.w[2] |= (uint32_t)n_wide << tnn::kPackedOrderFlagShift;
+                    hipLaunchKernelGGL((dense_bwd0_adam_pre_kernel<4>), n_wide + extra, 256, 0, s, ad.pw, ad.mw, ad.vw, gw.A, gw.B, po.w[0],
+                                       po.w[1], po.w[2], dims, gw, (float*)db, ad, ad);
+                    g_bwd0_args_form = 1;
+                    TNN_LAUNCH_OK();
+                    return 0;
+                }
                 hipLaunchKernelGGL((dense_bwd0_adam_kernel<4, true>), n_wide + extra, 256, 0, s, gw, (float*)db, ad, n_wide);
                 TNN_LAUNCH_OK();
                 return 0;
@@ -509,6 +553,8 @@
         return tnn_adam_ex(flat_p, flat_g, flat_m, flat_v, flat_n, lr, b1, b2, eps, pows, nullptr, dtype, 0, nullptr, nullptr);
     return 0;
 }
+
+__attribute__((visibility("default"))) int tnn_step_args_form(int which) { return which == 1 ? g_bwd0_args_form : g_small_args_form; }
 
 #ifdef TNN_STEP_TRACE
 extern "C" __attribute__((visibility("default"))) int tnn_debug_step_trace(unsigned long long* out, int n) {
@@ -623,8 +669,8 @@
     }
     if (int rc = gemm_f32(g, 0, 0)) return rc;
     const int64_t total = ((N + 15) / 16) * M * head_c;
-    hipLaunchKernelGGL(head_partials_kernel, tnn::stream_grid(total, 256), 256, 0, tnn::stream(), (const float*)C, M, N, ldc,
-                       (const float*)head_w, (int)head_c, (float*)head_z);
+    hipLaunchKernelGGL(head_partials_kernel, tnn::stream_grid(total, 256), 256, 0, tnn::stream(),
+                       HeadPartialsArgs{(const float*)C, M, N, ldc, (const float*)head_w, (int)head_c, (float*)head_z});
     TNN_LAUNCH_OK();
     return 0;
 }
diff --git a/tinynn-autograd_amd/csrc/tnn_gemm_args.h b/tinynn-autograd_amd/csrc/tnn_gemm_args.h
--- a/tinynn-autograd_amd/csrc/tnn_gemm_args.h
+++ b/tinynn-autograd_amd/csrc/tnn_gemm_args.h
@@ -22,6 +22,7 @@
     int64_t M, N, K, lda, ldb, ldc;
     float alpha, beta;
     int epi;
+    int epi_hole;
     const float* bias;
     int act, relu_sign;
     const float* Y;
@@ -48,6 +49,26 @@
     unsigned long long* trace;
 #endif
 };
+
+struct FastFirst {
+    const float *A, *B;
+    uint32_t a_bytes, b_bytes, lda4, ldb4, M, N, K;
+    int nchunks;
+    tnn::TileOrder ord;
+    bool head_on;
+};
+constexpr uint32_t FAST_FLAG_HEAD = 1u << 15;
+
+__device__ __forceinline__ FastFirst fast_first(const GemmArgs& g) {
+    const SmallFast& f = g.f;
+    return FastFirst{f.A, f.B, f.a_bytes, f.b_bytes, f.lda4, f.ldb4, f.M, f.N, f.K, f.nchunks, g.ord, f.h_bytes != 0u};
+}
+__device__ __forceinline__ FastFirst fast_first_sgprs(const float* A, const float* B, uint32_t a_bytes, uint32_t b_bytes, uint32_t lda4,
+                                                      uint32_t ldb4, uint32_t M, uint32_t N, uint32_t K, uint32_t o0, uint32_t o1,
+                                                      uint32_t o2) {
+    return FastFirst{A, B, a_bytes, b_bytes, lda4, ldb4, M, N, K, (int)((K + 15u) >> 4), tnn::unpack_tile_order(o0, o1, o2),
+                     (o2 >> tnn::kPackedOrderFlagShift & FAST_FLAG_HEAD) != 0u};
+}
 
 __device__ __forceinline__ float apply_epilogue(const GemmArgs& g, float acc, int64_t row,
                                                 int64_t col) {
diff --git a/tinynn-autograd_amd/csrc/tnn_gemm_small.h b/tinynn-autograd_amd/csrc/tnn_gemm_small.h
--- a/tinynn-autograd_amd/csrc/tnn_gemm_small.h
+++ b/tinynn-autograd_amd/csrc/tnn_gemm_small.h
@@ -188,37 +188,63 @@
     if constexpr (ADAM) TNN_STEP_STAMP_ACKED(g_step_trace, 3, 3);
 }
 
+struct DwFirst {
+    const float *A, *B;
+    float *pw, *mw, *vw;
+    int64_t M, N, K, lda, ldb, ldc;
+    tnn::TileOrder ord;
+};
+__device__ __forceinline__ DwFirst dw_first(const GemmArgs& g, const AdamEpi* ad) {
+    return DwFirst{g.A, g.B, ad ? ad->pw : nullptr, ad ? ad->mw : nullptr, ad ? ad->vw : nullptr, g.M, g.N, g.K, g.lda, g.ldb, g.ldc, g.ord};
+}
+__device__ __forceinline__ DwFirst dw_first_sgprs(float* pw, float* mw, float* vw, const float* A, const float* B, uint32_t o0, uint32_t o1,
+                                                  uint32_t o2, uint32_t dims) {
+    const int64_t M = dims & 0xffffu, N = (dims >> 16 & 0xffu) * 32u, K = (dims >> 24) + 1u;
+    return DwFirst{A, B, pw, mw, vw, M, N, K, M, N, N, tnn::unpack_tile_order(o0, o1, o2)};
+}
+
 template <int WAVES, bool ADAM, bool TO_LDS>
-__device__ __forceinline__ void dw_tile_wide(const GemmArgs& g, float* __restrict__ colsum, const int block, float (*red)[8][64],
-                                             float (*bsum)[2][64], const AdamEpi* ad = nullptr, float* out_lds = nullptr) {
+__device__ __forceinline__ void dw_tile_wide(const DwFirst& q, const GemmArgs& g, float* __restrict__ colsum, const int block,
+                                             float (*red)[8][64], float (*bsum)[2][64], const AdamEpi* ad = nullptr,
+                                             float* out_lds = nullptr) {
     if constexpr (ADAM) TNN_STEP_STAMP(g_step_trace, 3, 0);
     const int tid = threadIdx.x, lane = tid & 63, wid = tid >> 6;
     const int i16 = lane & 15, grp = lane >> 4;
     int tm, tn;
-    small_tile_coords(g, block, tm, tn);
+    tnn::tile_coords(q.ord, block, tm, tn);
     const int64_t m0 = (int64_t)tm * 16, n0 = (int64_t)tn * 32;
     const int64_t am = m0 + i16, bn = n0 + i16;
-    const bool a_ok = am < g.M;
-    const int nchunks = (int)((g.K + 15) / 16);
+    const bool a_ok = am < q.M;
+    const int nchunks = (int)((q.K + 15) / 16);
     const int e_r = tid >> 6, e_ln = tid & 63;
     const int64_t e_row = m0 + (e_ln >> 4) * 4 + e_r, e_col = n0 + (e_ln & 15);
-    const bool e_live = tid < 256 && e_row < g.M;
-    float a_p[2] = {0.f, 0.f}, a_m[2] = {0.f, 0.f}, a_v[2] = {0.f, 0.f}, ab_p = 0.f, ab_m = 0.f, ab_v = 0.f, ic1 = 0.f, ic2 = 0.f;
-    if constexpr (ADAM) {
-        ic1 = (float)(1.0 / (1.0 - ad->pows[0]));
-        ic2 = (float)(1.0 / (1.0 - ad->pows[1]));
+    const bool e_live = tid < 256 && e_row < q.M;
+    float a_p[2] = {0.f, 0.f}, a_m[2] = {0.f, 0.f}, a_v[2] = {0.f, 0.f}, ab_p = 0.f, ab_m = 0.f, ab_v = 0.f;
+    double pow1 = 0.0, pow2 = 0.0;
+    if constexpr (ADAM) {
         if (e_live) {
 #pragma unroll
             for (int u = 0; u < 2; ++u) {
-                const int64_t i = e_row * g.ldc + e_col + 16 * u;
-                a_p[u] = ad->pw[i]; a_m[u] = ad->mw[i]; a_v[u] = ad->vw[i];
-            }
-        }
-        if (tm == 0 && tid < 32) { ab_p = ad->pb[n0 + tid]; ab_m = ad->mb[n0 + tid]; ab_v = ad->vb[n0 + tid]; }
-    }
+                const int64_t i = e_row * q.ldc + e_col + 16 * u;
+                a_p[u] = q.pw[i]; a_m[u] = q.mw[i]; a_v[u] = q.vw[i];
+            }
+        }
+    }
+    [[maybe_unused]] auto request_late = [&]() {
+        if constexpr (ADAM) {
+            const uint32_t bytes = (uint32_t)q.N * 4u;
+            uint32_t off = (tm == 0 && tid < 32) ? ((uint32_t)n0 + (uint32_t)tid) * 4u : 0xffffffffu;
+            asm("" : "+v"(off));
+            ab_p = __uint_as_float(__builtin_amdgcn_raw_buffer_load_b32(__builtin_amdgcn_make_buffer_rsrc(ad->pb, 0, bytes, 0x00020000), off, 0, 0));
+            ab_m = __uint_as_float(__builtin_amdgcn_raw_buffer_load_b32(__builtin_amdgcn_make_buffer_rsrc(ad->mb, 0, bytes, 0x00020000), off, 0, 0));
+            ab_v = __uint_as_float(__builtin_amdgcn_raw_buffer_load_b32(__builtin_amdgcn_make_buffer_rsrc(ad->vb, 0, bytes, 0x00020000), off, 0, 0));
+            pow1 = ad->pows[0];
+            pow2 = ad->pows[1];
+        }
+    };
     f32x4 acc0 = {0.f, 0.f, 0.f, 0.f}, acc1 = {0.f, 0.f, 0.f, 0.f};
     float bs0 = 0.f, bs1 = 0.f;
-    const TnFrag fa(g.A, g.K, g.lda, g.M, grp, am, a_ok), fb(g.B, g.K, g.ldb, g.N, grp, bn, true);
+    const TnFrag fa(q.A, q.K, q.lda, q.M, grp, am, a_ok), fb(q.B, q.K, q.ldb, q.N, grp, bn, true);
     const int swid = __builtin_amdgcn_readfirstlane(wid);
     float a[TN_MAXC][4], b0[TN_MAXC][4], b1[TN_MAXC][4];
     [[maybe_unused]] unsigned long long t_first = 0, t_last = 0;
@@ -235,7 +261,11 @@
         },
         [&](const int u, const int n) {
             if constexpr (ADAM) {
-                if (u == 0) TNN_STEP_CLOCK_HOME(t_first, a[0][3], b1[0][3]);
+                if (u == 0) {
+                    request_late();
+                    __builtin_amdgcn_sched_barrier(0);
+                    TNN_STEP_CLOCK_HOME(t_first, a[0][3], b1[0][3]);
+                }
                 if (u == n - 1) TNN_STEP_CLOCK_HOME(t_last, a[u][3], b1[u][3]);
             }
         },
@@ -250,10 +280,18 @@
             bs0 += (b0[u][0] + b0[u][1]) + (b0[u][2] + b0[u][3]);
             bs1 += (b1[u][0] + b1[u][1]) + (b1[u][2] + b1[u][3]);
         });
+    if constexpr (ADAM) {
+        if (swid >= nchunks) request_late();
+    }
 #pragma unroll
     for (int r = 0; r < 4; ++r) { red[wid][r][lane] = acc0[r]; red[wid][4 + r][lane] = acc1[r]; }
     bsum[wid][0][lane] = bs0;
     bsum[wid][1][lane] = bs1;
+    float ic1 = 0.f, ic2 = 0.f;
+    if constexpr (ADAM) {
+        ic1 = (float)(1.0 / (1.0 - pow1));
+        ic2 = (float)(1.0 / (1.0 - pow2));
+    }
     __syncthreads();
     if constexpr (ADAM) TNN_STEP_STAMP(g_step_trace, 3, 2);
     if constexpr (ADAM) {
@@ -267,13 +305,13 @@
 #pragma unroll
             for (int w = 0; w < WAVES; ++w) sres += red[w][4 * u + e_r][e_ln];
             const float gval = g.alpha * sres;
-            const int64_t i = e_row * g.ldc + e_col + 16 * u;
+            const int64_t i = e_row * q.ldc + e_col + 16 * u;
             if constexpr (TO_LDS) out_lds[(int)(e_row - m0) * 32 + (int)(e_col - n0) + 16 * u] = gval;
             else if (!ADAM || g.C != nullptr) g.C[i] = gval;
             if constexpr (ADAM) {
-                ad->pw[i] = adam_apply(*ad, ic1, ic2, gval, a_m[u], a_v[u], a_p[u]);
-                ad->mw[i] = a_m[u];
-                ad->vw[i] = a_v[u];
+                q.pw[i] = adam_apply(*ad, ic1, ic2, gval, a_m[u], a_v[u], a_p[u]);
+                q.mw[i] = a_m[u];
+                q.vw[i] = a_v[u];
             }
         }
     }
@@ -294,7 +332,7 @@
 }
 
 template <bool AKC, bool BKC, int WAVES, bool SYS_HEADZ = false, bool HEAD = true>
-__device__ __forceinline__ void small_tile_fast(const GemmArgs& g, float* __restrict__ colsum, int block,
+__device__ __forceinline__ void small_tile_fast(const FastFirst& q, const GemmArgs& g, float* __restrict__ colsum, int block,
                                                 float (*red)[4][64], float (*bsum)[64], float* head_lds = nullptr) {
     typedef unsigned int u32x4_t __attribute__((ext_vector_type(4)));
     constexpr uint32_t OOB = 0xffffffffu;
@@ -304,14 +342,14 @@
     const int i16 = lane & 15, grp = lane >> 4;
     const SmallFast& f = g.f;
     int tm, tn;
-    small_tile_coords(g, block, tm, tn);
+    tnn::tile_coords(q.ord, block, tm, tn);
     const uint32_t m0 = (uint32_t)tm * 16u, n0 = (uint32_t)tn * 16u;
     const uint32_t am = m0 + (uint32_t)i16, bn = n0 + (uint32_t)i16;
-    const bool a_ok = am < f.M, b_ok = bn < f.N;
-    const int nchunks = f.nchunks;
-    const uint32_t K = f.K, lda4 = f.lda4, ldb4 = f.ldb4;
-    const __amdgpu_buffer_rsrc_t a_rsrc = __builtin_amdgcn_make_buffer_rsrc(const_cast<float*>(f.A), 0, f.a_bytes, 0x00020000);
-    const __amdgpu_buffer_rsrc_t b_rsrc = __builtin_amdgcn_make_buffer_rsrc(const_cast<float*>(f.B), 0, f.b_bytes, 0x00020000);
+    const bool a_ok = am < q.M, b_ok = bn < q.N;
+    const int nchunks = q.nchunks;
+    const uint32_t K = q.K, lda4 = q.lda4, ldb4 = q.ldb4;
+    const __amdgpu_buffer_rsrc_t a_rsrc = __builtin_amdgcn_make_buffer_rsrc(const_cast<float*>(q.A), 0, q.a_bytes, 0x00020000);
+    const __amdgpu_buffer_rsrc_t b_rsrc = __builtin_amdgcn_make_buffer_rsrc(const_cast<float*>(q.B), 0, q.b_bytes, 0x00020000);
     const uint32_t a_lane = AKC ? am * lda4 + (uint32_t)grp * 16u : (uint32_t)grp * 4u * lda4 + am * 4u;
     const uint32_t b_lane = BKC ? bn * ldb4 + (uint32_t)grp * 16u : (uint32_t)grp * 4u * ldb4 + bn * 4u;
     const uint32_t a_chunk = AKC ? 64u : 16u * lda4;
@@ -319,30 +357,33 @@
 
     const int e_r = tid >> 6, e_ln = tid & 63;
     const uint32_t e_row = m0 + (uint32_t)((e_ln >> 4) * 4 + e_r), e_col = n0 + (uint32_t)(e_ln & 15);
-    const bool e_live = tid < 256 && e_row < f.M && e_col < f.N;
-    const uint32_t e_off = e_row * f.e_ld4 + e_col * 4u;
-    const __amdgpu_buffer_rsrc_t e_rsrc = __builtin_amdgcn_make_buffer_rsrc(const_cast<float*>(f.e_ptr), 0, f.e_bytes, 0x00020000);
-    const bool head_on = f.h_bytes != 0u;
-    const __amdgpu_buffer_rsrc_t h_rsrc = __builtin_amdgcn_make_buffer_rsrc(const_cast<float*>(f.head_w), 0, f.h_bytes, 0x00020000);
+    const bool e_live = tid < 256 && e_row < q.M && e_col < q.N;
+    const uint32_t e_ld4 = f.e_ld4, e_bytes = f.e_bytes, h_bytes = f.h_bytes, h_hc4 = f.hc4;
+    const float *const e_ptr = f.e_ptr, *const h_ptr = f.head_w;
+    const bool head_on = q.head_on;
     const int swid = __builtin_amdgcn_readfirstlane(wid);
     float e_pre = 0.f;
     float head_pre[4] = {0.f, 0.f, 0.f, 0.f};
     auto request_epilogue = [&](auto role_c) {
         constexpr int ROLE = decltype(role_c)::value;
         if constexpr (ROLE >= 1) {
-            uint32_t off = e_live ? e_off : OOB;
+            const __amdgpu_buffer_rsrc_t e_rsrc = __builtin_amdgcn_make_buffer_rsrc(const_cast<float*>(e_ptr), 0, e_bytes, 0x00020000);
+            uint32_t row_b = e_row * e_ld4;
+            asm("" : "+v"(row_b));
+            uint32_t off = e_live ? row_b + e_col * 4u : OOB;
             asm("" : "+v"(off));
             e_pre = __uint_as_float(__builtin_amdgcn_raw_buffer_load_b32(e_rsrc, off, 0, 0));
         }
         if constexpr (ROLE == 2) {
-            const uint32_t unit0 = n0 + 4u * (uint32_t)grp, hc4 = f.hc4;
+            const __amdgpu_buffer_rsrc_t h_rsrc = __builtin_amdgcn_make_buffer_rsrc(const_cast<float*>(h_ptr), 0, h_bytes, 0x00020000);
+            const uint32_t unit0 = n0 + 4u * (uint32_t)grp, hc4 = h_hc4;
             uint32_t unit_b = unit0 * hc4;
             asm("" : "+v"(unit_b));
             const uint32_t off0 = unit_b + (uint32_t)i16 * 4u;
             const bool cls_ok = (uint32_t)i16 * 4u < hc4;
 #pragma unroll
             for (int j = 0; j < 4; ++j) {
-                const bool ok = cls_ok & (unit0 + (uint32_t)j < f.N);
+                const bool ok = cls_ok & (unit0 + (uint32_t)j < q.N);
                 uint32_t off = ok ? off0 + (uint32_t)j * hc4 : OOB;
                 asm("" : "+v"(off));
                 head_pre[j] = __uint_as_float(__builtin_amdgcn_raw_buffer_load_b32(h_rsrc, off, 0, 0));
@@ -441,6 +482,7 @@
     for (int r = 0; r < 4; ++r) red[wid][r][lane] = acc[r];
     bsum[wid][lane] = bs;
     __syncthreads();
+    asm volatile("" ::"s"(g.epi_hole));
     TNN_STEP_STAMP(g_step_trace, KID, 2);
     TNN_STEP_STAMP_VALUE(g_step_trace_first, KID, 1, 0, t_first);
     TNN_STEP_STAMP_VALUE(g_step_trace, KID, 4, 1, t_last);
@@ -454,7 +496,7 @@
             g.C[(int64_t)e_row * g.ldc + e_col] = e_val;
         }
     }
-    if (colsum != nullptr && tm == 0 && tid < 16 && n0 + (uint32_t)tid < f.N) {
+    if (colsum != nullptr && tm == 0 && tid < 16 && n0 + (uint32_t)tid < q.N) {
         float s = 0.f;
 #pragma unroll
         for (int w = 0; w < WAVES; ++w) s += (bsum[w][tid] + bsum[w][16 + tid]) + (bsum[w][32 + tid] + bsum[w][48 + tid]);
@@ -491,9 +533,22 @@
     __shared__ float bsum[WAVES][64];
     if constexpr (FAST) {
         __shared__ __attribute__((aligned(16))) float head_lds[16 * 20];
-        small_tile_fast<AKC, BKC, WAVES>(g, colsum, (int)blockIdx.x, red, bsum, head_lds);
+        small_tile_fast<AKC, BKC, WAVES>(fast_first(g), g, colsum, (int)blockIdx.x, red, bsum, head_lds);
         if (g.bump != nullptr && blockIdx.x == 0 && threadIdx.x == 0) *g.bump += 1u;
     } else {
         small_tile<AKC, BKC, WAVES>(g, colsum, (int)blockIdx.x, red, bsum);
     }
 }
+
+template <bool AKC, bool BKC, int WAVES>
+__global__ __launch_bounds__(WAVES * 64) void gemm_small_pre_f32_kernel(const float* A, const float* B, uint32_t a_bytes, uint32_t b_bytes,
+                                                                        uint32_t lda4, uint32_t ldb4, uint32_t M, uint32_t N, uint32_t K,
+                                                                        uint32_t o0, uint32_t o1, uint32_t o2, GemmArgs g,
+                                                                        float* __restrict__ colsum) {
+    __shared__ float red[WAVES][4][64];
+    __shared__ float bsum[WAVES][64];
+    __shared__ __attribute__((aligned(16))) float head_lds[16 * 20];
+    small_tile_fast<AKC, BKC, WAVES>(fast_first_sgprs(A, B, a_bytes, b_bytes, lda4, ldb4, M, N, K, o0, o1, o2), g, colsum,
+                                     (int)blockIdx.x, red, bsum, head_lds);
+    if (g.bump != nullptr && blockIdx.x == 0 && threadIdx.x == 0) *g.bump += 1u;
+}
diff --git a/tinynn-autograd_amd/csrc/tnn_gemm_step.h b/tinynn-autograd_amd/csrc/tnn_gemm_step.h
--- a/tinynn-autograd_amd/csrc/tnn_gemm_step.h
+++ b/tinynn-autograd_amd/csrc/tnn_gemm_step.h
@@ -13,7 +13,7 @@
     __shared__ double dred[8][4];
     __shared__ int is_last;
     TNN_AR_STAMP(g_fh_trace, blockIdx.x, 8, 128, 0);
-    small_tile_fast<true, false, WAVES, true>(g, nullptr, (int)blockIdx.x, red, bsum, head_lds);
+    small_tile_fast<true, false, WAVES, true>(fast_first(g), g, nullptr, (int)blockIdx.x, red, bsum, head_lds);
     TNN_AR_STAMP(g_fh_trace, blockIdx.x, 8, 128, 1);
     using namespace tnn::p2p;
     int tm, tn;
@@ -74,7 +74,7 @@
     __shared__ __attribute__((aligned(16))) float head_lds[16 * 20];
     __shared__ float wred[WAVES][2];
     __shared__ int is_last;
-    small_tile_fast<true, false, WAVES, true>(g, nullptr, (int)blockIdx.x, red, bsum, head_lds);
+    small_tile_fast<true, false, WAVES, true>(fast_first(g), g, nullptr, (int)blockIdx.x, red, bsum, head_lds);
     using namespace tnn::p2p;
     if (threadIdx.x < 64) {
         asm volatile("s_waitcnt vmcnt(0)" ::: "memory");
@@ -291,9 +291,9 @@
     __shared__ float bsum[WAVES][64];
     if constexpr (FAST) {
         if ((int)blockIdx.x < n_dw)
-            small_tile_fast<false, false, WAVES, false, false>(gw, db, (int)blockIdx.x, red, bsum);
+            small_tile_fast<false, false, WAVES, false, false>(fast_first(gw), gw, db, (int)blockIdx.x, red, bsum);
         else
-            small_tile_fast<true, true, WAVES, false, false>(gx, nullptr, (int)blockIdx.x - n_dw, red, bsum);
+            small_tile_fast<true, true, WAVES, false, false>(fast_first(gx), gx, nullptr, (int)blockIdx.x - n_dw, red, bsum);
     } else {
         if ((int)blockIdx.x < n_dw)
             small_tile<false, false, WAVES>(gw, db, (int)blockIdx.x, red, bsum);
@@ -308,8 +308,22 @@
     __shared__ float red[WAVES][WIDE ? 8 : 4][64];
     __shared__ float bsum[WAVES][WIDE ? 2 : 1][64];
     if ((int)blockIdx.x < n_dw) {
-        if constexpr (WIDE) dw_tile_wide<WAVES, true, false>(gw, db, (int)blockIdx.x, red, bsum, &ad);
+        if constexpr (WIDE) dw_tile_wide<WAVES, true, false>(dw_first(gw, &ad), gw, db, (int)blockIdx.x, red, bsum, &ad);
         else small_tile<false, false, WAVES, true>(gw, db, (int)blockIdx.x, red, reinterpret_cast<float(*)[64]>(bsum), &ad);
+        return;
+    }
+    adam_flat_range<WAVES * 64, true>(ad, (int)blockIdx.x - n_dw, (int)gridDim.x - n_dw);
+}
+
+template <int WAVES>
+__global__ __launch_bounds__(WAVES * 64) void dense_bwd0_adam_pre_kernel(float* pw, float* mw, float* vw, const float* A, const float* B,
+                                                                         uint32_t o0, uint32_t o1, uint32_t o2, uint32_t dims, GemmArgs gw,
+                                                                         float* __restrict__ db, AdamEpi adt, AdamEpi ad) {
+    __shared__ float red[WAVES][8][64];
+    __shared__ float bsum[WAVES][2][64];
+    const int n_dw = (int)(o2 >> tnn::kPackedOrderFlagShift);
+    if ((int)blockIdx.x < n_dw) {
+        dw_tile_wide<WAVES, true, false>(dw_first_sgprs(pw, mw, vw, A, B, o0, o1, o2, dims), gw, db, (int)blockIdx.x, red, bsum, &adt);
         return;
     }
     adam_flat_range<WAVES * 64, true>(ad, (int)blockIdx.x - n_dw, (int)gridDim.x - n_dw);
@@ -342,7 +356,7 @@
         const int b = (int)blockIdx.x % P;
         const uint32_t tag = ctx.ar_epoch[b] + 1;
         const int dead_at_entry = __hip_atomic_load(ctx.dead, __ATOMIC_RELAXED, __HIP_MEMORY_SCOPE_AGENT);
-        if constexpr (WIDE) dw_tile_wide<WAVES, false, true>(gw, nullptr, (int)blockIdx.x, red, bsum, nullptr, tile);
+        if constexpr (WIDE) dw_tile_wide<WAVES, false, true>(dw_first(gw, nullptr), gw, nullptr, (int)blockIdx.x, red, bsum, nullptr, tile);
         else small_tile<false, false, WAVES, false, true>(gw, nullptr, (int)blockIdx.x, red, reinterpret_cast<float(*)[64]>(bsum), nullptr, tile);
         __syncthreads();
         TNN_AR_STAMP(g_ar_trace, blockIdx.x, 4, 1024, 1);
@@ -450,8 +464,19 @@
     }
 }
 
-__global__ __launch_bounds__(256) void head_partials_kernel(const float* __restrict__ out, int64_t M, int64_t N, int64_t ldc,
-                                                            const float* __restrict__ hw, int hc, float* __restrict__ hz) {
+struct HeadPartialsArgs {
+    const float* out;
+    int64_t M, N, ldc;
+    const float* hw;
+    int hc;
+    float* hz;
+};
+__global__ __launch_bounds__(256) void head_partials_kernel(HeadPartialsArgs a) {
+    const float* __restrict__ out = a.out;
+    const float* __restrict__ hw = a.hw;
+    float* __restrict__ hz = a.hz;
+    const int64_t M = a.M, N = a.N, ldc = a.ldc;
+    const int hc = a.hc;
     const int64_t tiles_n = (N + 15) / 16, total = tiles_n * M * hc;
     for (int64_t i = (int64_t)blockIdx.x * blockDim.x + threadIdx.x; i < total; i += (int64_t)gridDim.x * blockDim.x) {
         const int c = (int)(i % hc);
diff --git a/tinynn-autograd_amd/csrc/tnn_head.hip b/tinynn-autograd_amd/csrc/tnn_head.hip
--- a/tinynn-autograd_amd/csrc/tnn_head.hip
+++ b/tinynn-autograd_amd/csrc/tnn_head.hip
@@ -1,6 +1,7 @@
 #include <math.h>
 #include <stdio.h>
 #include <stdlib.h>
+#include <string.h>
 
 #include "tnn_internal.h"
 #include "tnn_tile_order.h"
@@ -34,26 +35,39 @@
 struct HeadStage {
     f32x4 v[NP], yv;
 };
+struct HeadFirst {
+    const float *zpart, *y, *b;
+    int m, vec;
+};
+__device__ __forceinline__ HeadFirst head_first(const HeadMArgs& p);
+template <int C, int NP>
+__device__ __forceinline__ void head_stage_request(const HeadFirst& p, const int t, HeadStage<C, NP>& h) {
+    const int n = p.m * C;
+    if (p.vec && t < (n >> 2)) {
+#pragma unroll
+        for (int tn = 0; tn < NP; ++tn) h.v[tn] = *reinterpret_cast<const f32x4*>(p.zpart + (size_t)tn * n + 4 * t);
+        h.yv = *reinterpret_cast<const f32x4*>(p.y + 4 * t);
+    }
+}
 template <int C, int NP>
 __device__ __forceinline__ void head_stage_request(const HeadMArgs& p, const int t, HeadStage<C, NP>& h) {
-    const int n = p.m * C;
-    if (p.vec && t < (n >> 2)) {
-#pragma unroll
-        for (int tn = 0; tn < NP; ++tn) h.v[tn] = *reinterpret_cast<const f32x4*>(p.zpart + (size_t)tn * n + 4 * t);
-        h.yv = *reinterpret_cast<const f32x4*>(p.y + 4 * t);
-    }
+    head_stage_request<C, NP>(head_first(p), t, h);
+}
+template <int C, int NP>
+__device__ __forceinline__ f32x4 head_stage_bias(const HeadFirst& p, const int t) {
+    f32x4 b = {0.f, 0.f, 0.f, 0.f};
+    if (p.vec) {
+#pragma unroll
+        for (int i = 0; i < 4; ++i) b[i] = p.b[(4 * t + i) % C];
+    }
+    return b;
 }
 template <int C, int NP>
 __device__ __forceinline__ f32x4 head_stage_bias(const HeadMArgs& p, const int t) {
-    f32x4 b = {0.f, 0.f, 0.f, 0.f};
-    if (p.vec) {
-#pragma unroll
-        for (int i = 0; i < 4; ++i) b[i] = p.b[(4 * t + i) % C];
-    }
-    return b;
-}
-template <int C, int NP>
-__device__ __forceinline__ void head_stage_store(const HeadMArgs& p, const int t, const HeadStage<C, NP>& h, float* zs, float* ys,
+    return head_stage_bias<C, NP>(head_first(p), t);
+}
+template <int C, int NP, class P>
+__device__ __forceinline__ void head_stage_store(const P& p, const int t, const HeadStage<C, NP>& h, float* zs, float* ys,
                                                  const f32x4 bias4) {
     static_assert(NP == 8, "the partial-sum tree is written for 8 tiles");
     const int n = p.m * C;
@@ -74,6 +88,8 @@
         }
     }
 }
+
+__device__ __forceinline__ HeadFirst head_first(const HeadMArgs& p) { return HeadFirst{p.zpart, p.y, p.b, p.m, p.vec}; }
 
 template <int H, int C, bool PART, int CUT, bool DA, int SH = 0>
 __device__ __forceinline__ void head_block(const HeadMArgs& p, const int g) {
@@ -286,12 +302,14 @@
     int dx_wide;
 };
 
+int g_head_args_form = -1;
+
 #ifdef TNN_STEP_TRACE
 __device__ unsigned long long g_step_trace_head[1024 * 4];
 #endif
 
-template <int H, int C, int CUT = 0, int SH = 0>
-__global__ __launch_bounds__(512) void mlp_head_bwd_kernel(HeadMArgs p, HeadBwdArgs q) {
+template <int H, int C, int CUT, int SH>
+__device__ __forceinline__ void mlp_head_bwd_body(const HeadFirst& f, const HeadMArgs& p, const HeadBwdArgs& q) {
     constexpr int ROWS = 128, WS = 12, NP = H / 16, G = H / 8, TH = H / 16, PS = H + 4;
     static_assert(H == 128 && NP == 8, "one 16-deep K chunk per wave, 8 waves");
     TNN_STEP_STAMP(g_step_trace_head, 0, 0);
@@ -309,7 +327,11 @@
     const int t = threadIdx.x, lane = t & 63, wid = t >> 6;
     const int i16 = lane & 15, grp = lane >> 4;
     const int srow = t >> 2, sub = t & 3;
-    const int m = p.m;
+    const int m = f.m;
+    HeadStage<C, NP> stg;
+    head_stage_request<C, NP>(f, t, stg);
+    const f32x4 bias4 = head_stage_bias<C, NP>(f, t);
+    __builtin_amdgcn_sched_barrier(0);
     const bool slive = srow < m;
     const int sr = min(srow, m - 1);
     const int n_dw = q.n_dw;
@@ -321,9 +343,6 @@
     tnn::tile_coords(is_dw ? q.ord_dw : q.ord_dx, is_dw ? blk : blk - n_dw, tm, tn);
     const int m0 = tm * 16, n0 = tn * ((!is_dw && wide) ? 32 : 16);
 
-    HeadStage<C, NP> stg;
-    head_stage_request<C, NP>(p, t, stg);
-    const f32x4 bias4 = head_stage_bias<C, NP>(p, t);
     const int urow = (is_dw ? n0 : 16 * wid) + i16;
     const int prow0 = (is_dw ? 16 * wid : m0) + 4 * grp;
     float w2f[3], a1m[4];
@@ -348,7 +367,7 @@
     static_assert(C == 10, "the zero columns of the K = 12 product are written for 10 classes");
 
     TNN_STEP_STAMP_ACKED(g_step_trace_head, 0, 1);
-    head_stage_store<C, NP>(p, t, stg, zs, ys, bias4);
+    head_stage_store<C, NP>(f, t, stg, zs, ys, bias4);
     __syncthreads();
     float zc[3], yc[3];
 #pragma unroll
@@ -457,6 +476,16 @@
         q.db1[n0 + t] = s;
     }
     TNN_STEP_STAMP_ACKED(g_step_trace_head, 0, 3);
+}
+
+template <int H, int C, int CUT = 0, int SH = 0>
+__global__ __launch_bounds__(512) void mlp_head_bwd_kernel(HeadMArgs p, HeadBwdArgs q) {
+    mlp_head_bwd_body<H, C, CUT, SH>(head_first(p), p, q);
+}
+template <int H, int C>
+__global__ __launch_bounds__(512) void mlp_head_bwd_pre_kernel(const float* zpart, const float* y, const float* b, int m, int vec,
+                                                               HeadMArgs p, HeadBwdArgs q) {
+    mlp_head_bwd_body<H, C, 0, 0>(HeadFirst{zpart, y, b, m, vec}, p, q);
 }
 
 template <int C, int NP>
@@ -1350,7 +1379,11 @@
         TNN_LAUNCH_OK();
         return 0;
     }
-    hipLaunchKernelGGL((mlp_head_bwd_kernel<128, 10>), grid, 512, 0, tnn::stream(), p, q);
+    const char* sw = getenv("TNN_STEP_ARGS");
+    const bool forced = sw != nullptr && strncmp(sw, "struct", 6) == 0 && (sw[6] == 0 || (sw[6] == ':' && strstr(sw + 7, "head") != nullptr));
+    g_head_args_form = forced ? 0 : 1;
+    if (forced) hipLaunchKernelGGL((mlp_head_bwd_kernel<128, 10>), grid, 512, 0, tnn::stream(), p, q);
+    else hipLaunchKernelGGL((mlp_head_bwd_pre_kernel<128, 10>), grid, 512, 0, tnn::stream(), p.zpart, p.y, p.b, p.m, p.vec, p, q);
     TNN_LAUNCH_OK();
     return 0;
 }
@@ -1359,6 +1392,8 @@
 }
 
 extern "C" {
+
+__attribute__((visibility("default"))) int tnn_step_args_form_head(void) { return g_head_args_form; }
 
 #ifdef TNN_STEP_TRACE
 __attribute__((visibility("default"))) int tnn_debug_step_trace_head(unsigned long long* out, int n) {
diff --git a/tinynn-autograd_amd/csrc/tnn_tile_order.h b/tinynn-autograd_amd/csrc/tnn_tile_order.h
--- a/tinynn-autograd_amd/csrc/tnn_tile_order.h
+++ b/tinynn-autograd_amd/csrc/tnn_tile_order.h
@@ -52,4 +52,31 @@
     tn = (int)((xcd >> o.xm_shift) * o.pn + q);
 }
 
+struct PackedTileOrder {
+    uint32_t w[3];
+};
+constexpr uint32_t kPackedOrderFlagShift = 16;
+
+inline bool pack_tile_order(const TileOrder& o, PackedTileOrder& p) {
+    if (o.pm == 0 || o.pm > 65535u || o.pn > 65535u) return false;
+    if (o.magic != (uint64_t(1) << 32) / o.pm + 1) return false;
+    if (o.xcd_mask > 7u || o.xcd_shift > 3u || o.xm_mask > 7u || o.xm_shift > 3u) return false;
+    p.w[0] = o.pm | o.pn << 16;
+    p.w[1] = (uint32_t)o.magic;
+    p.w[2] = o.xcd_mask | o.xcd_shift << 3 | o.xm_mask << 5 | o.xm_shift << 8;
+    return true;
 }
+
+TNN_TILE_ORDER_HD TileOrder unpack_tile_order(const uint32_t w0, const uint32_t w1, const uint32_t w2) {
+    TileOrder o;
+    o.pm = w0 & 0xffffu;
+    o.pn = w0 >> 16;
+    o.magic = (o.pm == 1u ? uint64_t(1) << 32 : uint64_t(0)) | w1;
+    o.xcd_mask = w2 & 7u;
+    o.xcd_shift = (w2 >> 3) & 3u;
+    o.xm_mask = (w2 >> 5) & 7u;
+    o.xm_shift = (w2 >> 8) & 3u;
+    return o;
+}
+
+}
```

Measured after the change: 8.138 million samples/s (median of 6 runs). 6.9% higher.
